# voutcn/megahit

Measured on NVIDIA H100. Metric: sorted (k+1)-mer edges/sec at k=27 on 150bp reads, higher is better.
Workload: dtype u32

## Files before the change

### include/mhb.h

```cpp
#ifndef MHB_H
#define MHB_H
#include <stddef.h>
#include <stdint.h>

#ifdef __cplusplus
extern "C" {
#endif

#define MHB_OK 0
#define MHB_ERR_ARG 1
#define MHB_ERR_CUDA 2
#define MHB_ERR_IO 3
#define MHB_ERR_NOMEM 4

#define MHB_NUM_BUCKETS 65536
#define MHB_MAX_MUL 65535
#define MHB_MAX_K 255
#define MHB_SENTINEL_OFFSET 0xFFFFFFFFu

const char *mhb_last_error(void);
const char *mhb_version(void);
int mhb_device_count(void);
uint64_t mhb_launch_count(void);

uint32_t mhb_count_record_words(uint32_t k);
uint32_t mhb_words_per_edge(uint32_t k);
uint32_t mhb_s2s_record_words(uint32_t k);
uint32_t mhb_count_sort_bytes(uint32_t k, uint8_t *bytes);
uint32_t mhb_s2s_sort_bytes(uint32_t k, uint8_t *bytes);
size_t mhb_sort_workspace_bytes(uint64_t n, uint32_t words);


typedef struct {
  const uint32_t *bin;
  uint64_t bin_words;
  uint64_t n_reads;
  uint32_t fixed_len;
  const uint64_t *rec_off;
  const uint64_t *edge_off;
} mhb_dev_reads;

int mhb_count_extract(void *stream, const mhb_dev_reads *reads, uint32_t k, uint32_t *records,
                      uint64_t n_edges, uint64_t *hist256, int hist_byte);

int mhb_check_fixed_len(void *stream, const uint32_t *bin_dev, uint64_t n_reads, uint32_t fixed_len, uint64_t *flag_dev);

int mhb_count_extract_range(void *stream, const mhb_dev_reads *reads, uint32_t k, uint32_t lo, uint32_t hi, int write,
                            uint64_t *per_read, uint32_t *records, uint64_t *hist256, int hist_byte,
                            uint64_t *total_dev);

int mhb_sort_records(void *stream, uint32_t *a, uint32_t *b, uint64_t n, uint32_t words,
                     const uint8_t *bytes, uint32_t n_bytes, const uint64_t *first_hist, void *ws,
                     size_t ws_bytes, int *result_in_b);

int mhb_sort_records_relaxed(void *stream, uint32_t *a, uint32_t *b, uint64_t n, uint32_t words, const uint8_t *bytes,
                             uint32_t n_bytes, const uint64_t *first_hist, void *ws, size_t ws_bytes, int *result_in_b);

int mhb_partition_scatter(void *stream, const uint32_t *recs, uint64_t n, uint32_t words, int byte,
                          const uint8_t *owner_of_byte_dev, const uint64_t *bin_addr_dev, void *ws, size_t ws_bytes);
int mhb_partition_scatter_hist(void *stream, const uint32_t *recs, uint64_t n, uint32_t words, int byte,
                               const uint8_t *owner_of_byte_dev, const uint64_t *bin_addr_dev, void *ws, size_t ws_bytes,
                               int next_byte, uint64_t *owner_next_hist, int *hist_done);
int mhb_plan_partition(void *stream, const uint64_t *hist_all_dev, uint32_t world, uint32_t rank, uint32_t record_bytes,
                       const uint64_t *peer_base_host, uint8_t *owner_lut_dev, uint64_t *bin_addr_dev, uint64_t *plan_dev);
int mhb_compact_tip_edges(void *stream, const uint32_t *edges, const uint8_t *aux, uint64_t n_solid, uint32_t k,
                          uint32_t *tips_out, uint8_t *tip_aux_out, uint64_t capacity, uint64_t *cursor_dev);
int mhb_dev_malloc(void **ptr, size_t bytes);
int mhb_dev_free(void *ptr);
int mhb_ipc_export(const void *dev_ptr, uint8_t *handle64);
int mhb_ipc_open(const uint8_t *handle64, void **peer_ptr);
int mhb_ipc_close(void *peer_ptr);

int mhb_set_sort_cfg(int cfg);

int mhb_sort_pass_ms(int back, double *pass_ms, uint32_t max_passes, uint32_t *n_passes, uint64_t *n_records,
                     uint32_t *words);

size_t mhb_count_solid_scratch_bytes(uint64_t n);
int mhb_count_solid(void *stream, const uint32_t *sorted_records, uint64_t n, uint32_t k, int32_t m,
                    uint32_t *edges_out, uint8_t *aux_out, uint64_t capacity_edges, uint64_t *mul_hist,
                    uint64_t *n_solid_out, void *scratch, size_t scratch_bytes);

int mhb_count_hashed_supported(uint32_t k, int32_t m);
size_t mhb_count_hashed_workspace_bytes(uint64_t n, uint32_t k, int32_t m);
int mhb_count_solid_hashed(void *stream, uint32_t *recs_a, uint32_t *recs_b, uint64_t n, uint32_t k, int32_t m,
                           const uint64_t *hist_byte5, uint32_t *edges_out, uint8_t *aux_out, uint64_t capacity_edges,
                           uint64_t *mul_hist, uint64_t *n_solid_out, void *ws, size_t ws_bytes);

size_t mhb_tipset_bytes(uint64_t n_tip_edges, uint32_t k);
int mhb_tipset_build(void *stream, const uint32_t *edges, const uint8_t *aux, uint64_t n_solid, uint32_t k,
                     void *tipset, size_t tipset_bytes, uint64_t n_tip_edges);
int mhb_count_mark_mercy(void *stream, const mhb_dev_reads *reads, uint32_t k, const void *tipset,
                         size_t tipset_bytes, uint64_t n_tip_edges, uint32_t *first_0_out, uint32_t *last_0_in);
int mhb_count_tip_edges(void *stream, const uint8_t *aux, uint64_t n_solid, uint64_t *n_tip_host);

size_t mhb_mercy_candidates_scratch_bytes(uint64_t n_reads);
int mhb_mercy_candidates(void *stream, const uint32_t *first_0_out, const uint32_t *last_0_in, uint64_t n_reads,
                         uint64_t *cand_ids, uint64_t *n_cand_host, void *scratch, size_t scratch_bytes);
size_t mhb_mercy_edges_scratch_bytes(uint64_t n_cand, uint32_t max_read_len);
int mhb_mercy_edges(void *stream, const mhb_dev_reads *reads, const uint64_t *cand_ids, uint64_t n_cand,
                    uint32_t max_read_len, uint32_t k, const uint32_t *edges, uint64_t n_edges, uint32_t *mercy_out,
                    uint64_t capacity, uint64_t *n_mercy_host, void *scratch, size_t scratch_bytes);
int mhb_mercy_edges_count(void *stream, const mhb_dev_reads *reads, const uint64_t *cand_ids, uint64_t n_cand,
                          uint32_t max_read_len, uint32_t k, uint32_t n_segs, const uint32_t *const *seg_edges,
                          const uint64_t *seg_counts, const void *const *seg_luts, const uint8_t *owner_of_byte,
                          uint64_t *n_mercy_host, void *scratch, size_t scratch_bytes);
int mhb_mercy_edges_write(void *stream, const mhb_dev_reads *reads, const uint64_t *cand_ids, uint64_t n_cand,
                          uint32_t max_read_len, uint32_t k, uint32_t *mercy_out, uint64_t capacity, uint64_t n_mercy,
                          void *scratch, size_t scratch_bytes);

size_t mhb_mercy_planes_words(uint64_t n_cand, uint32_t max_read_len);
int mhb_mercy_probe_owned(void *stream, const mhb_dev_reads *reads, const uint64_t *cand_ids, uint64_t n_cand,
                          uint32_t max_read_len, uint32_t k, const uint32_t *edges, uint64_t n_edges, const void *lut,
                          const uint8_t *owner_of_byte, uint32_t me, uint32_t *planes_out);
int mhb_mercy_count_planes(void *stream, const mhb_dev_reads *reads, const uint64_t *cand_ids, uint64_t n_cand,
                           uint32_t max_read_len, uint32_t k, const uint32_t *planes, uint32_t n_src,
                           uint64_t src_stride_words, uint64_t *n_mercy_host, void *scratch, size_t scratch_bytes);

int mhb_mercy_edges_segs(void *stream, const mhb_dev_reads *reads, const uint64_t *cand_ids, uint64_t n_cand,
                         uint32_t max_read_len, uint32_t k, uint32_t n_segs, const uint32_t *const *seg_edges,
                         const uint64_t *seg_counts, const void *const *seg_luts, const uint8_t *owner_of_byte,
                         uint32_t *mercy_out, uint64_t capacity, uint64_t *n_mercy_host, void *scratch,
                         size_t scratch_bytes);
size_t mhb_edge_lut_bytes(void);
int mhb_edge_lut_build(void *stream, const uint32_t *edges, uint64_t n_edges, uint32_t k, void *lut);

typedef struct {
  const uint32_t *words;
  uint64_t n_words;
  uint64_t n_seqs;
  uint32_t fixed_len;
  const uint64_t *word_off;
  const uint32_t *len;
  const uint64_t *item_off;
  const uint16_t *mult;
  uint32_t fixed_stride;
} mhb_dev_seqs;

int mhb_s2s_extract(void *stream, const mhb_dev_seqs *seqs, uint32_t k, uint32_t *records, uint64_t n_items,
                    uint64_t *hist256, int hist_byte);

int mhb_s2s_extract_edges_pruned(void *stream, const uint32_t *edges, const uint8_t *aux, uint64_t n_edges,
                                 uint64_t n_with_aux, uint32_t k, uint32_t *records, uint64_t capacity,
                                 uint64_t *cursor_dev, uint64_t *hist256, int hist_byte);

int mhb_s2s_extract_range(void *stream, const mhb_dev_seqs *seqs, uint32_t k, uint32_t *records, uint64_t n_items,
                          uint32_t lo, uint32_t hi, uint64_t *cursor_dev, uint64_t capacity, uint64_t *hist256,
                          int hist_byte);

size_t mhb_s2s_emit_scratch_bytes(uint64_t n, uint32_t k);
int mhb_s2s_emit(void *stream, const uint32_t *sorted_records, uint64_t n, uint32_t k, uint8_t *bytes_out,
                 uint64_t capacity_bytes, uint64_t *bucket_table, uint64_t *totals, void *scratch,
                 size_t scratch_bytes);

int mhb_s2s_emit_fmt(void *stream, const uint32_t *sorted_records, uint64_t n, uint32_t k, uint8_t *bytes_out,
                     uint64_t capacity_bytes, uint64_t *bucket_table, uint64_t *totals, void *scratch,
                     size_t scratch_bytes, int label_fmt);

int mhb_set_device(int device);

typedef struct {
  uint32_t k;
  int32_t m;
  const uint32_t *bin;
  uint64_t bin_words;
  uint64_t n_reads;
  int want_mercy;
} mhb_count_args;

typedef struct {
  uint64_t n_edge_records;
  uint64_t n_solid;
  uint32_t words_per_edge;
  uint32_t *edges;
  uint64_t n_cand;
  uint64_t *cand_ids;
  uint64_t n_has_tips;
  int64_t counting[MHB_MAX_MUL + 1];
  double t_h2d_ms, t_extract_ms, t_sort_ms, t_count_ms, t_mercy_ms, t_d2h_ms, t_total_ms;
  uint32_t n_sort_passes;
  uint32_t n_rounds;
  double sort_pass_ms[64];
} mhb_count_result;

int mhb_count_host(const mhb_count_args *args, mhb_count_result *res);
int mhb_set_round_limit(uint64_t max_records_per_round);
int mhb_set_s2s_round_limit(uint64_t max_items_per_round);
int mhb_plan_rounds(const uint64_t *hist256, uint64_t max_records, uint32_t *lo_out, uint32_t *hi_out);
int mhb_plan_rounds16(const uint64_t *hist256, const uint64_t *sub_hist, uint64_t max_records, uint32_t *lo16_out,
                      uint32_t *hi16_out, uint32_t cap_out);

typedef struct {
  uint32_t k;
  const uint32_t *words;
  const uint64_t *word_off;
  const uint32_t *len;
  const uint16_t *mult;
  uint64_t n_seqs;
} mhb_s2s_args;

typedef struct {
  uint64_t n_records;
  uint64_t n_items, n_tips, n_large_mul, n_bytes;
  uint32_t words_per_tip_label;
  uint8_t *bytes;
  uint64_t bucket_table[MHB_NUM_BUCKETS * 4];
  uint64_t w_count[9];
  uint64_t ones_in_last;
  double t_total_ms, t_extract_ms, t_sort_ms, t_emit_ms;
} mhb_s2s_result;

int mhb_s2s_host(const mhb_s2s_args *args, mhb_s2s_result *res);

typedef struct {
  uint32_t k;
  int32_t m;
  const uint32_t *bin;
  uint64_t bin_words;
  uint64_t n_reads;
  int32_t need_mercy;
  int32_t want_edges;
  uint8_t *sdbg_out;
  uint64_t sdbg_out_capacity;
} mhb_build_args;

typedef struct {
  uint64_t n_edge_records, n_solid, n_cand, n_mercy, n_sort_items;
  uint32_t words_per_edge, words_per_tip_label;
  uint64_t n_items, n_tips, n_large_mul, n_bytes;
  uint8_t *bytes;
  uint64_t *bucket_table;
  uint64_t w_count[9];
  uint64_t ones_in_last;
  uint32_t *edges;
  uint64_t *cand_ids;
  int64_t *counting;
  double t_total_ms, t_h2d_ms, t_count_ms, t_mercy_ms, t_s2s_ms, t_d2h_ms;
  uint32_t n_rounds_s1, n_rounds_s2;
} mhb_build_result;

int mhb_build_host(const mhb_build_args *args, mhb_build_result *res);
// ... 112 lines not shown
```

### megahit_b200/csrc/mhb_hashcount.cu

```cuda
#include <cuda_runtime.h>
#include <stdio.h>
#include <string.h>

#include "mhb.h"
#include "mhb_common.cuh"
#include "mhb_count.cuh"

using namespace mhb;

namespace {

constexpr int kHcHist = 1024;
constexpr u64 kHcEmpty = ~0ull;
constexpr int kHcBatch = 8;
constexpr u32 kRemBits = 42;
constexpr u32 kHcHotCount = 256;
constexpr int kHcHotRound = 32;
constexpr int kHcMaxProbes = 48;
constexpr int kHcStack = 72;
constexpr u32 kHcHistDone = 1u << 31;
constexpr u32 kHcPrefetchChunk = 16384;

__device__ __forceinline__ u64 rec_key64(const uint2 r) { return ((u64)r.x << 32) | r.y; }

// ... 352 lines not shown
          s.tmp[atomicAdd(&s.cell_cur[(u32)((e << bits) >> cshift)], 1u)] = e;
        }
        __syncthreads();
        for (u32 i = tid; i < (u32)CELLS; i += THREADS) s.cell_cur[i] = 0;
        for (u32 i = tid; i < ns; i += THREADS) {
          const u64 e = s.tmp[i];
          const u32 c = (u32)((e << bits) >> cshift);
          const u32 b0 = s.cell_base[c], b1 = c + 1 < (u32)CELLS ? s.cell_base[c + 1] : ns;
          u32 r = b0;
          for (u32 j = b0; j < b1; ++j) r += s.tmp[j] < e ? 1u : 0u;
          list[base + out_cursor + r] = e;
        }
        out_cursor += ns;
      }
      if (failed) {
        for (u32 i = tid; i < (u32)CELLS; i += THREADS) s.cell_cur[i] = 0;
        if (bits + 2 > kRemBits || sp + 4 > (u32)kHcStack) {
          if (tid == 0) atomicExch(err_flag, 1u);
        } else {
          const u32 flag = (hist_done || !overflowed) ? kHcHistDone : 0u;
          if (tid == 0)
            for (int c = 3; c >= 0; --c) {
              s.st_prefix[sp + 3 - c] = (prefix << 2) | (u64)c;
              s.st_bits[sp + 3 - c] = (bits + 2) | flag;
            }
          sp += 4;
        }
        __syncthreads();
      }
      if (sp == 0) break;
      --sp;
      prefix = s.st_prefix[sp];
      bits = s.st_bits[sp] & ~kHcHistDone;
      hist_done = (s.st_bits[sp] & kHcHistDone) != 0;
    }
    if (tid == 0) slice_count[sl] = out_cursor;
  }
  __syncthreads();
  for (u32 i = tid; i < kHcHist; i += THREADS)
    if (s.cta_hist[i]) atomicAdd((unsigned long long *)&mul_hist[i], (unsigned long long)s.cta_hist[i]);
}

using HcGeomB = HcGeom<512, 12, 2>;

__global__ void k_slice_counts(const u64 *__restrict__ bounds, u32 T, u32 *__restrict__ cnt) {
  const u32 b = blockIdx.x * blockDim.x + threadIdx.x;
  if (b >= 65536u) return;
  const u64 nb = bounds[b + 1] - bounds[b];
  cnt[b] = (u32)((nb + T - 1) / T);
}

__global__ void __launch_bounds__(256)
    k_hash_gather(const u64 *__restrict__ list, const u64 *__restrict__ n_slices_dev, const u32 *__restrict__ slice_count,
                  const u64 *__restrict__ slice_dst, const u64 *__restrict__ slice_base, const u32 *__restrict__ slice_bucket,
                  u32 we, u32 *__restrict__ edges, uint8_t *__restrict__ aux, u64 capacity, const u32 *err_flag,
                  u64 *n_solid_out) {
  const u32 lane = threadIdx.x & 31;
  if (blockIdx.x == 0 && threadIdx.x == 0 && *err_flag) *n_solid_out = ~0ull;
  const u64 n_slices = *n_slices_dev;
  for (u64 sl = (u64)blockIdx.x * 8 + (threadIdx.x >> 5); sl < n_slices; sl += (u64)gridDim.x * 8) {
    const u32 cnt = slice_count[sl];
    if (!cnt) continue;
    const u64 base = slice_base[sl], off = slice_dst[sl], b = slice_bucket[sl];
    for (u32 x = lane; x < cnt; x += 32) {
      if (off + x >= capacity) break;
      const u64 ent = list[base + x];
      const u64 key = (b << 48) | ((ent >> 22) << 6);
      u32 *e = edges + (off + x) * we;
      e[0] = (u32)(key >> 32);
      e[1] = (u32)key;
      if (we == 3) e[2] = 0;
      e[we - 1] |= (u32)(ent >> 6) & 0xFFFFu;
      aux[off + x] = (uint8_t)(ent & 3u);
    }
  }
}

int scan_counts(cudaStream_t st, const u32 *in, u64 n, u64 *out, u64 *total_dev, u64 *bsum) {
  const u64 nb = (n + kScanTile - 1) / kScanTile;
  k_scan32_sums<<<(unsigned)nb, kScanThreads, 0, st>>>(in, n, bsum);
  CK_LAUNCH();
  k_scan_u64<<<1, 1024, 0, st>>>(bsum, nb, total_dev);
  CK_LAUNCH();
  k_scan32_apply<<<(unsigned)nb, kScanThreads, 0, st>>>(in, n, bsum, out);
  CK_LAUNCH();
  return MHB_OK;
}

template <class G>
static int launch_hash_count(cudaStream_t st, const uint2 *recs, const ulonglong2 *plan, const u64 *n_slices_dev, int m, u32 *misc,
                             u64 *list, u32 *slice_count, u64 *mul_hist) {
  static int bps = 0;
  const size_t smem = sizeof(HcShared<G>);
  if (!bps) {
    CK(cudaFuncSetAttribute(k_hash_count<G>, cudaFuncAttributeMaxDynamicSharedMemorySize, (int)smem));
    CK(cudaOccupancyMaxActiveBlocksPerMultiprocessor(&bps, k_hash_count<G>, G::THREADS, smem));
    if (bps < 1) return mhb_set_error(MHB_ERR_CUDA, "hash-count kernel does not fit an SM (%zu B shared memory)", smem);
    if (getenv("MHB_VERBOSE")) fprintf(stderr, "[mhb] hash count: %d threads, %d slots, %zu B smem, %d CTA/SM, slice %u\n", G::THREADS, G::SLOTS, smem, bps, G::SLICE);
  }
  k_hash_count<G><<<sm_count() * bps, G::THREADS, smem, st>>>(recs, plan, n_slices_dev, m, misc, list, slice_count, mul_hist,
                                                             misc + 1);
  CK_LAUNCH();
  return MHB_OK;
}

struct HcLayout {
  size_t sort_ws, off_bounds, off_bcnt, off_soff, off_bsum, off_misc, off_scount, off_sdst, off_sbase, off_sbucket, off_plan,
      off_list, total;
  uint64_t max_slices;
};
HcLayout hc_layout(uint64_t n, int32_t m) {
  HcLayout L;
  auto pad = [](size_t x) { return (x + 255) & ~(size_t)255; };
  L.max_slices = n / HcGeomB::SLICE + 65536 + 2;
  L.sort_ws = pad(mhb_sort_workspace_bytes(n, 2));
  size_t p = L.sort_ws;
  L.off_bounds = p;
  p += pad(65537 * 8);
  L.off_bcnt = p;
  p += pad(65537 * 4);
  L.off_soff = p;
  p += pad(65537 * 8);
  L.off_bsum = p;
  p += pad((L.max_slices / kScanTile + 4) * 8);
  L.off_misc = p;
  p += 256;
  L.off_scount = p;
  p += pad(L.max_slices * 4);
  L.off_sdst = p;
  p += pad(L.max_slices * 8);
  L.off_sbase = p;
  p += pad(L.max_slices * 8);
  L.off_sbucket = p;
  p += pad(L.max_slices * 4);
  L.off_plan = p;
  p += pad(L.max_slices * 16);
  L.off_list = p;
  p += pad((size_t)(n / (uint64_t)(m < 1 ? 1 : m) + L.max_slices + 8) * 8);
  L.total = p;
  return L;
}

}

extern "C" int mhb_count_hashed_supported(uint32_t k, int32_t m) {
  return count_record_words(k) == 2 && 2 * (k + 1) >= 24 && m >= 1 && m <= kHcHist;
}

extern "C" size_t mhb_count_hashed_workspace_bytes(uint64_t n, uint32_t k, int32_t m) {
  (void)k;
  return hc_layout(n, m).total;
}

extern "C" int mhb_count_solid_hashed(void *stream, uint32_t *recs_a, uint32_t *recs_b, uint64_t n, uint32_t k, int32_t m,
                                      const uint64_t *hist_byte5, uint32_t *edges_out, uint8_t *aux_out,
                                      uint64_t capacity_edges, uint64_t *mul_hist, uint64_t *n_solid_out, void *ws,
                                      size_t ws_bytes) {
  if (!mhb_count_hashed_supported(k, m)) return mhb_set_error(MHB_ERR_ARG, "hashed count needs 8-byte records (13 <= k <= 28) and 1 <= m <= %d", kHcHist);
  if (!mul_hist || !n_solid_out || !ws) return mhb_set_error(MHB_ERR_ARG, "bad args");
  if (n == 0) return MHB_OK;
  if (n >= (1ull << 40)) return mhb_set_error(MHB_ERR_ARG, "too many records for one hashed count call");
  const HcLayout L = hc_layout(n, m);
  if (ws_bytes < L.total) return mhb_set_error(MHB_ERR_ARG, "hashed count workspace too small (%zu < %zu)", ws_bytes, L.total);
  cudaStream_t st = (cudaStream_t)stream;
  const uint8_t bytes[3] = {5, 6, 7};
  int in_b = 0;
  if (int rc = mhb_sort_records_impl(st, recs_a, recs_b, n, 2, bytes, 3, hist_byte5, ws, L.sort_ws, &in_b, nullptr)) return rc;
  const uint2 *recs = (const uint2 *)(in_b ? recs_b : recs_a);
  char *w = (char *)ws;
  u64 *bounds = (u64 *)(w + L.off_bounds);
  u32 *bcnt = (u32 *)(w + L.off_bcnt);
  u64 *slice_off = (u64 *)(w + L.off_soff);
  u64 *bsum = (u64 *)(w + L.off_bsum);
  u32 *misc = (u32 *)(w + L.off_misc);
  u32 *slice_count = (u32 *)(w + L.off_scount);
  u64 *slice_dst = (u64 *)(w + L.off_sdst);
  u64 *slice_base = (u64 *)(w + L.off_sbase);
  u32 *slice_bucket = (u32 *)(w + L.off_sbucket);
  ulonglong2 *plan = (ulonglong2 *)(w + L.off_plan);
  u64 *list = (u64 *)(w + L.off_list);
  u64 *n_slices_dev = (u64 *)(misc + 2);
  CK(cudaMemsetAsync(misc, 0, 256, st));
  CK(cudaMemsetAsync(slice_count, 0, L.max_slices * 4, st));
  k_bucket_bounds<<<(65537 + 255) / 256, 256, 0, st>>>(recs, n, bounds);
  CK_LAUNCH();
  k_slice_counts<<<65536 / 256, 256, 0, st>>>(bounds, HcGeomB::SLICE, bcnt);
  CK_LAUNCH();
  if (int rc = scan_counts(st, bcnt, 65536, slice_off, n_slices_dev, bsum)) return rc;
  CK(cudaMemcpyAsync(slice_off + 65536, n_slices_dev, 8, cudaMemcpyDeviceToDevice, st));
  k_slice_plan<<<65536 / 256, 256, 0, st>>>(recs, bounds, slice_off, m, plan, slice_base, slice_bucket);
  CK_LAUNCH();
  if (int rc = launch_hash_count<HcGeomB>(st, recs, plan, n_slices_dev, m, misc, list, slice_count, mul_hist)) return rc;
  if (int rc = scan_counts(st, slice_count, L.max_slices, slice_dst, n_solid_out, bsum)) return rc;
  k_hash_gather<<<sm_count() * 4, 256, 0, st>>>(list, n_slices_dev, slice_count, slice_dst, slice_base, slice_bucket,
                                               words_per_edge(k), edges_out, aux_out, capacity_edges, misc + 1, n_solid_out);
  CK_LAUNCH();
  return MHB_OK;
}
```

### megahit_b200/csrc/mhb_host.cu

```cuda
#include <cuda_runtime.h>
#include <stdio.h>
#include <stdlib.h>
#include <string.h>

#include <algorithm>
#include <vector>

#include "mhb.h"
#include "mhb_bits.cuh"
#include "mhb_internal.h"

using namespace mhb;

#define CK(call)                                                                                   \
  do {                                                                                             \
    cudaError_t e_ = (call);                                                                       \
    if (e_ != cudaSuccess)                                                                         \
      return mhb_set_error(MHB_ERR_CUDA, "%s failed at %s:%d: %s", #call, __FILE__, __LINE__,      \
                           cudaGetErrorString(e_));                                                \
  } while (0)
#define CKR(call)           \
  do {                      \
    int rc_ = (call);       \
    if (rc_) return rc_;    \
// ... 8 lines not shown
    used = 0;
    if (bytes <= cap) return MHB_OK;
    if (base) cudaFree(base);
    base = nullptr;
    cap = 0;
    cudaError_t e = cudaMalloc((void **)&base, bytes);
    if (e != cudaSuccess) {
      cudaGetLastError();
      return mhb_set_error(MHB_ERR_NOMEM, "cudaMalloc of %zu bytes failed: %s", bytes, cudaGetErrorString(e));
    }
    cap = bytes;
    return MHB_OK;
  }
  template <class T>
  T *take(size_t count) {
    size_t bytes = (count * sizeof(T) + 255) & ~(size_t)255;
    char *p = base + used;
    used += bytes;
    return reinterpret_cast<T *>(p);
  }
  static size_t pad(size_t bytes) { return (bytes + 255) & ~(size_t)255; }
};
Arena g_arena;

struct Timer {
  cudaEvent_t a, b;
  cudaStream_t st;
  explicit Timer(cudaStream_t s) : st(s) {
    cudaEventCreate(&a);
    cudaEventCreate(&b);
  }
  ~Timer() {
    cudaEventDestroy(a);
    cudaEventDestroy(b);
  }
  void start() { cudaEventRecord(a, st); }
  double stop() {
    cudaEventRecord(b, st);
    cudaEventSynchronize(b);
    float ms = 0;
    cudaEventElapsedTime(&ms, a, b);
    return ms;
  }
};

struct BinIndex {
  uint32_t fixed_len = 0;
  std::vector<uint64_t> rec_off, edge_off;
  uint64_t n_edges = 0;
};

int index_bin(const uint32_t *bin, uint64_t bin_words, uint64_t n_reads, uint32_t k, BinIndex *ix, bool sampled = false) {
  ix->fixed_len = 0;
  ix->n_edges = 0;
  if (n_reads == 0) return MHB_OK;
  if (bin_words == 0) return mhb_set_error(MHB_ERR_ARG, "empty .bin image for %llu reads", (unsigned long long)n_reads);
  const uint32_t L0 = bin[0];
  const uint64_t stride = 1 + div_ceil(L0, 16);
  bool fixed = L0 > 0 && bin_words == n_reads * stride;
  if (fixed && sampled) {
    const uint64_t step = std::max<uint64_t>(1, n_reads / 1024);
    for (uint64_t r = 0; r < n_reads && fixed; r += step) fixed = bin[r * stride] == L0;
    for (uint64_t r = 0; r < std::min<uint64_t>(n_reads, 1024) && fixed; ++r) fixed = bin[r * stride] == L0;
    fixed = fixed && bin[(n_reads - 1) * stride] == L0;
  } else if (fixed) {
    int bad = 0;
#pragma omp parallel for reduction(| : bad) schedule(static)
    for (long long r = 0; r < (long long)n_reads; ++r) bad |= bin[(uint64_t)r * stride] != L0;
    fixed = !bad;
  }
  if (fixed) {
    ix->fixed_len = L0;
    ix->n_edges = L0 >= k + 1 ? n_reads * (uint64_t)(L0 - k) : 0;
    if (L0 < k + 1) ix->fixed_len = L0;
    return MHB_OK;
  }
  ix->rec_off.resize(n_reads + 1);
  ix->edge_off.resize(n_reads + 1);
  uint64_t pos = 0, e = 0;
  for (uint64_t r = 0; r < n_reads; ++r) {
    if (pos >= bin_words) return mhb_set_error(MHB_ERR_ARG, ".bin image truncated at read %llu", (unsigned long long)r);
    const uint32_t L = bin[pos];
    ix->rec_off[r] = pos;
    ix->edge_off[r] = e;
    if (L >= k + 1) e += L - k;
    pos += 1 + div_ceil(L, 16);
  }
  if (pos > bin_words) return mhb_set_error(MHB_ERR_ARG, ".bin image truncated");
  ix->rec_off[n_reads] = pos;
  ix->edge_off[n_reads] = e;
  ix->n_edges = e;
  return MHB_OK;
}

}

extern "C" int mhb_release(void) {
  if (g_arena.base) cudaFree(g_arena.base);
  g_arena = Arena();
  return MHB_OK;
}

size_t mhb_arena_bytes(void) { return g_arena.cap; }

int SdbgStitch::append(void *stream, const uint8_t *d_bytes, uint64_t cap_bytes, const uint64_t *d_table,
                       const uint64_t *d_totals) {
  cudaStream_t st = (cudaStream_t)stream;
  uint64_t rt[16];
  CK(cudaMemcpyAsync(rt, d_totals, sizeof(rt), cudaMemcpyDeviceToHost, st));
  CK(cudaMemcpyAsync(round_table.data(), d_table, round_table.size() * 8, cudaMemcpyDeviceToHost, st));
  CK(cudaStreamSynchronize(st));
  if (rt[0] > cap_bytes) return mhb_set_error(MHB_ERR_NOMEM, "internal: SdBG byte stream exceeds capacity");
  const size_t base = bytes.size();
  bytes.resize(base + rt[0]);
  if (rt[0]) CK(cudaMemcpy(bytes.data() + base, d_bytes, rt[0], cudaMemcpyDeviceToHost));
  for (size_t b = 0; b < (size_t)MHB_NUM_BUCKETS; ++b)
    if (round_table[4 * b + 1]) {
      table[4 * b + 0] = round_table[4 * b + 0] + base;
      table[4 * b + 1] = round_table[4 * b + 1];
      table[4 * b + 2] = round_table[4 * b + 2];
      table[4 * b + 3] = round_table[4 * b + 3];
    }
  for (int i = 0; i < 16; ++i) tot[i] += rt[i];
  return MHB_OK;
}


namespace {
struct CountWork {
  bool hashed;
  size_t bytes;
  size_t ws_bytes;
  int hist_byte;
};
CountWork count_work_plan(uint64_t n, uint32_t k, int32_t m) {
  static const bool force_sort = getenv("MHB_COUNT_MODE") && !strcmp(getenv("MHB_COUNT_MODE"), "sort");
  CountWork cw;
  cw.hashed = !force_sort && mhb_count_hashed_supported(k, m);
  if (cw.hashed) {
    cw.bytes = mhb_count_hashed_workspace_bytes(n, k, m);
    cw.ws_bytes = 0;
    cw.hist_byte = 5;
  } else {
    uint8_t sb[72];
    mhb_count_sort_bytes(k, sb);
    cw.ws_bytes = Arena::pad(mhb_sort_workspace_bytes(n, count_record_words(k)));
    cw.bytes = cw.ws_bytes + Arena::pad(mhb_count_solid_scratch_bytes(n));
    cw.hist_byte = sb[0];
  }
  return cw;
}
int run_count_stage(cudaStream_t st, const CountWork &cw, uint32_t *d_a, uint32_t *d_b, uint64_t n, uint32_t k, int32_t m,
                    const uint64_t *d_hist0, uint32_t *d_edges, uint8_t *d_aux, uint64_t cap_edges, uint64_t *d_mul_hist,
                    uint64_t *d_nsolid, char *work, double *pass_ms, uint32_t *n_passes) {
  const uint32_t WR = count_record_words(k);
  if (cw.hashed) {
    if (n_passes) *n_passes = n ? 2 : 0;
    CKR(mhb_count_solid_hashed(st, d_a, d_b, n, k, m, d_hist0, d_edges, d_aux, cap_edges, d_mul_hist, d_nsolid, work, cw.bytes));
    if (pass_ms && n) {
      uint32_t np = 0, w = 0;
      uint64_t nr = 0;
      CKR(mhb_sort_pass_ms(0, pass_ms, 64, &np, &nr, &w));
    }
    return MHB_OK;
  }
  uint8_t sort_bytes[72];
  const uint32_t n_sort = mhb_count_sort_bytes(k, sort_bytes);
  if (n_passes) *n_passes = n ? n_sort : 0;
  int in_b = 0;
  CKR(mhb_sort_records_impl(st, d_a, d_b, n, WR, sort_bytes, n_sort, d_hist0, work, cw.ws_bytes, &in_b, pass_ms));
  return mhb_count_solid(st, in_b ? d_b : d_a, n, k, m, d_edges, d_aux, cap_edges, d_mul_hist, d_nsolid, work + cw.ws_bytes,
                         cw.bytes - cw.ws_bytes);
}
}

namespace {
size_t round_bytes(uint64_t n, uint32_t WR, uint32_t WE, int32_t m, uint32_t k) {
  const uint64_t cap_edges = n / (uint64_t)std::max(1, m) + 1;
  return 2 * Arena::pad((size_t)n * WR * 4 + 16) + Arena::pad(count_work_plan(n, k, m).bytes) +
         Arena::pad((size_t)cap_edges * WE * 4) + Arena::pad(cap_edges);
}
}

namespace {
uint64_t g_round_limit = 0;
uint64_t g_s2s_round_limit = 0;


}

extern "C" int mhb_plan_rounds(const uint64_t *hist256, uint64_t max_records, uint32_t *lo_out, uint32_t *hi_out) {
  if (!hist256 || !lo_out || !hi_out || max_records == 0) {
    mhb_set_error(MHB_ERR_ARG, "bad round plan arguments");
    return -1;
  }
  int n = 0;
  uint32_t lo = 0;
  uint64_t acc = 0;
  for (uint32_t b = 0; b < 256; ++b) {
    if (hist256[b] > max_records) {
      mhb_set_error(MHB_ERR_NOMEM, "leading byte 0x%02x alone holds %llu records, more than one round can take (%llu)", b,
                    (unsigned long long)hist256[b], (unsigned long long)max_records);
      return -1;
    }
    if (acc + hist256[b] > max_records) {
      lo_out[n] = lo;
      hi_out[n] = b - 1;
      ++n;
      lo = b;
      acc = 0;
    }
    acc += hist256[b];
  }
  lo_out[n] = lo;
  hi_out[n] = 255;
  return n + 1;
}

extern "C" int mhb_plan_rounds16(const uint64_t *hist256, const uint64_t *sub_hist, uint64_t max_records, uint32_t *lo_out,
                                 uint32_t *hi_out, uint32_t cap_out) {
  if (!hist256 || !lo_out || !hi_out || max_records == 0 || cap_out == 0) {
    mhb_set_error(MHB_ERR_ARG, "bad round plan arguments");
    return -1;
  }
  uint32_t n = 0, lo = 0;
  uint64_t acc = 0;
  bool open = false;
  auto close_at = [&](uint32_t hi) -> bool {
    if (n >= cap_out) return false;
    lo_out[n] = lo;
    hi_out[n] = hi;
    ++n;
    return true;
  };
  auto add = [&](uint32_t a_lo, uint32_t a_hi, uint64_t cnt) -> int {
    if (cnt > max_records) {
      mhb_set_error(MHB_ERR_NOMEM, "bucket 0x%04x alone holds %llu records, more than one round can take (%llu)", a_lo,
                    (unsigned long long)cnt, (unsigned long long)max_records);
      return -1;
    }
    if (open && acc + cnt > max_records) {
      if (!close_at(a_lo - 1)) return -2;
      open = false;
    }
    if (!open) {
      lo = a_lo;
      acc = 0;
      open = true;
    }
    acc += cnt;
    (void)a_hi;
    return 0;
  };
  for (uint32_t b = 0; b < 256; ++b) {
    int rc = 0;
    if (hist256[b] > max_records) {
      if (!sub_hist) {
        mhb_set_error(MHB_ERR_NOMEM, "leading byte 0x%02x alone holds %llu records, more than one round can take (%llu)", b,
                      (unsigned long long)hist256[b], (unsigned long long)max_records);
        return -1;
      }
      for (uint32_t c = 0; c < 256 && !rc; ++c) rc = add((b << 8) | c, (b << 8) | c, sub_hist[(size_t)b * 256 + c]);
    } else {
      rc = add(b << 8, (b << 8) | 255u, hist256[b]);
    }
    if (rc == -1) return -1;
    if (rc == -2) break;
  }
  if (!open) {
    lo = 0;
    open = true;
  }
  if (lo_out && n < cap_out) {
    lo_out[n] = n ? lo : 0;
    hi_out[n] = 65535;
    return (int)n + 1;
  }
  mhb_set_error(MHB_ERR_NOMEM, "round plan needs more than %u ranges", cap_out);
  return -1;
}

extern "C" int mhb_set_round_limit(uint64_t max_records_per_round) {
  g_round_limit = max_records_per_round;
  return MHB_OK;
}
extern "C" int mhb_set_s2s_round_limit(uint64_t max_items_per_round) {
  g_s2s_round_limit = max_items_per_round;
  return MHB_OK;
}

static int count_host_rounds(const mhb_count_args *args, mhb_count_result *res, const BinIndex &ix, uint64_t max_records) {
  const uint32_t k = args->k;
  const int32_t m = args->m;
  const uint64_t n = ix.n_edges, n_reads = args->n_reads;
  const uint32_t WR = count_record_words(k), WE = words_per_edge(k);
  uint8_t sort_bytes[72];
  const uint32_t n_sort = mhb_count_sort_bytes(k, sort_bytes);
  const int top_byte = (int)(4 * WR - 1);
  cudaStream_t st = 0;
  Timer t_all(st), t(st);
  t_all.start();

  const size_t bin_bytes = (args->bin_words * 4 + 15) & ~(size_t)15;
  size_t fixed = Arena::pad(bin_bytes + 16) + Arena::pad((n_reads + 2) * 8) + Arena::pad(65536 * 8) + 2 * Arena::pad(256 * 8) +
                 Arena::pad(64) + 8192;
  if (!ix.fixed_len) fixed += 2 * Arena::pad((n_reads + 1) * 8);
  if (args->want_mercy) fixed += 2 * Arena::pad((size_t)(n_reads + 1) * 4);
  if (!max_records) {
    size_t free_b = 0, total_b = 0;
    CK(cudaMemGetInfo(&free_b, &total_b));
    const size_t avail = (size_t)((double)(free_b + g_arena.cap) * 0.92);
    if (avail <= fixed) return mhb_set_error(MHB_ERR_NOMEM, "the read library alone (%zu bytes) does not fit the device", fixed);
    uint64_t lo = 1, hi = n;
    while (lo < hi) {
      const uint64_t mid = lo + (hi - lo + 1) / 2;
      if (fixed + round_bytes(mid, WR, WE, m, k) <= avail) lo = mid;
      else hi = mid - 1;
    }
    max_records = lo;
  }
  max_records = std::min<uint64_t>(std::max<uint64_t>(max_records, 1), std::max<uint64_t>(n, 1));
  const uint64_t cap_edges = max_records / (uint64_t)std::max(1, m) + 1;
  CKR(g_arena.reserve(fixed + round_bytes(max_records, WR, WE, m, k)));

  uint32_t *d_bin = g_arena.take<uint32_t>(bin_bytes / 4 + 4);
// ... 41 lines not shown
  uint64_t h_top[256];
  CKR(mhb_count_extract_range(st, &reads, k, 0, 65535, 0, d_per_read, nullptr, d_hist_top, top_byte, d_scalars + 1));
  CK(cudaMemcpyAsync(h_top, d_hist_top, sizeof(h_top), cudaMemcpyDeviceToHost, st));
  CK(cudaStreamSynchronize(st));
  std::vector<uint64_t> h_sub;
  for (uint32_t b = 0; b < 256; ++b) {
    if (h_top[b] <= max_records) continue;
    if (WR * 4 < 2) return mhb_set_error(MHB_ERR_NOMEM, "leading byte 0x%02x exceeds a round and the record has no second byte", b);
    if (h_sub.empty()) h_sub.assign(256 * 256, 0);
    CK(cudaMemsetAsync(d_hist0, 0, 256 * 8, st));
    CKR(mhb_count_extract_range(st, &reads, k, b << 8, (b << 8) | 255u, 0, d_per_read, nullptr, d_hist0, top_byte - 1, d_scalars + 1));
    CK(cudaMemcpyAsync(h_sub.data() + (size_t)b * 256, d_hist0, 256 * 8, cudaMemcpyDeviceToHost, st));
    CK(cudaStreamSynchronize(st));
  }
  std::vector<uint32_t> r_lo(65536), r_hi(65536);
  const int n_ranges = mhb_plan_rounds16(h_top, h_sub.empty() ? nullptr : h_sub.data(), max_records, r_lo.data(), r_hi.data(), 65536);
  if (n_ranges < 0) return MHB_ERR_NOMEM;
  std::vector<std::pair<uint32_t, uint32_t>> ranges;
  for (int i = 0; i < n_ranges; ++i) ranges.push_back({r_lo[i], r_hi[i]});
  res->t_extract_ms = t.stop();

  std::vector<uint32_t> h_edges;
  std::vector<uint32_t> h_tip_edges;
  std::vector<uint8_t> h_tip_aux, h_aux;
  uint64_t n_solid_total = 0;
  for (const auto &rg : ranges) {
    t.start();
    uint64_t n_round = 0;
    CKR(mhb_count_extract_range(st, &reads, k, rg.first, rg.second, 0, d_per_read, nullptr, nullptr, 0, d_scalars + 1));
    CK(cudaMemcpyAsync(&n_round, d_scalars + 1, 8, cudaMemcpyDeviceToHost, st));
    CK(cudaMemsetAsync(d_hist0, 0, 256 * 8, st));
    CK(cudaMemsetAsync(d_scalars, 0, 8, st));
    CK(cudaStreamSynchronize(st));
    if (n_round > max_records) return mhb_set_error(MHB_ERR_NOMEM, "internal: round of %llu records exceeds its plan", (unsigned long long)n_round);
    if (n_round == 0) continue;
    CKR(mhb_count_extract_range(st, &reads, k, rg.first, rg.second, 1, d_per_read, d_a, d_hist0, cw.hist_byte, nullptr));
    res->t_extract_ms += t.stop();
    t.start();
    CKR(run_count_stage(st, cw, d_a, d_b, n_round, k, m, d_hist0, d_edges, d_aux, cap_edges, d_mul_hist, d_scalars, d_work,
                        nullptr, nullptr));
    uint64_t n_solid = 0;
    CK(cudaMemcpyAsync(&n_solid, d_scalars, 8, cudaMemcpyDeviceToHost, st));
    CK(cudaStreamSynchronize(st));
    res->t_count_ms += t.stop();
    if (n_solid > cap_edges) return mhb_set_error(MHB_ERR_NOMEM, "internal: solid edges exceed capacity");
    t.start();
    const size_t e0 = h_edges.size();
    h_edges.resize(e0 + (size_t)n_solid * WE);
    h_aux.resize(n_solid);
    if (n_solid) {
      CK(cudaMemcpyAsync(h_edges.data() + e0, d_edges, (size_t)n_solid * WE * 4, cudaMemcpyDeviceToHost, st));
      CK(cudaMemcpyAsync(h_aux.data(), d_aux, n_solid, cudaMemcpyDeviceToHost, st));
      CK(cudaStreamSynchronize(st));
    }
    if (args->want_mercy)
      for (uint64_t i = 0; i < n_solid; ++i)
        if (h_aux[i]) {
          h_tip_edges.insert(h_tip_edges.end(), h_edges.begin() + e0 + i * WE, h_edges.begin() + e0 + (i + 1) * WE);
          h_tip_aux.push_back(h_aux[i]);
        }
    n_solid_total += n_solid;
    res->t_d2h_ms += t.stop();
    ++res->n_rounds;
  }
  res->n_solid = n_solid_total;

  std::vector<uint32_t> h_first, h_last;
  if (args->want_mercy && n_reads) {
    t.start();
    const uint64_t n_tip = h_tip_aux.size();
    const size_t ts_bytes = mhb_tipset_bytes(n_tip, k);
    const size_t list_bytes = Arena::pad(h_tip_edges.size() * 4 + 16) + Arena::pad(n_tip + 16);
    char *d_tmp = nullptr;
    bool own = false;
    const size_t have = (size_t)max_records * WR * 4 * 2;
    if (ts_bytes + list_bytes + 512 <= have) d_tmp = (char *)d_a;
    else {
      CK(cudaMalloc((void **)&d_tmp, ts_bytes + list_bytes + 512));
      own = true;
    }
    uint32_t *d_tip_edges = (uint32_t *)d_tmp;
    uint8_t *d_tip_aux = (uint8_t *)(d_tmp + Arena::pad(h_tip_edges.size() * 4 + 16));
    char *d_tips = d_tmp + list_bytes;
    int rc = MHB_OK;
    if (n_tip) {
      if (cudaMemcpyAsync(d_tip_edges, h_tip_edges.data(), h_tip_edges.size() * 4, cudaMemcpyHostToDevice, st) != cudaSuccess ||
          cudaMemcpyAsync(d_tip_aux, h_tip_aux.data(), n_tip, cudaMemcpyHostToDevice, st) != cudaSuccess)
        rc = mhb_set_error(MHB_ERR_CUDA, "tip edge upload failed");
    }
    if (!rc) rc = mhb_tipset_build(st, d_tip_edges, d_tip_aux, n_tip, k, d_tips, ts_bytes, n_tip);
    if (!rc) rc = mhb_count_mark_mercy(st, &reads, k, d_tips, ts_bytes, n_tip, d_first, d_last);
    h_first.resize(n_reads);
    h_last.resize(n_reads);
    if (!rc) {
      cudaMemcpyAsync(h_first.data(), d_first, n_reads * 4, cudaMemcpyDeviceToHost, st);
      cudaMemcpyAsync(h_last.data(), d_last, n_reads * 4, cudaMemcpyDeviceToHost, st);
      if (cudaStreamSynchronize(st) != cudaSuccess) rc = mhb_set_error(MHB_ERR_CUDA, "mercy marking failed: %s", cudaGetErrorString(cudaGetLastError()));
    }
    if (own) cudaFree(d_tmp);
    if (rc) return rc;
    res->t_mercy_ms = t.stop();
  }

  res->edges = (uint32_t *)malloc(std::max<size_t>(1, h_edges.size() * 4));
  if (!res->edges) return mhb_set_error(MHB_ERR_NOMEM, "host malloc failed");
  if (!h_edges.empty()) memcpy(res->edges, h_edges.data(), h_edges.size() * 4);
  std::vector<uint64_t> h_hist(65536);
  CK(cudaMemcpy(h_hist.data(), d_mul_hist, 65536 * 8, cudaMemcpyDeviceToHost));
  for (int i = 0; i <= MHB_MAX_MUL; ++i) res->counting[i] = (int64_t)h_hist[i];
  if (args->want_mercy) {
    std::vector<uint64_t> ids;
    for (uint64_t r = 0; r < n_reads; ++r) {
      const uint32_t f = h_first[r], l = h_last[r];
      if (f != MHB_SENTINEL_OFFSET && l != MHB_SENTINEL_OFFSET) {
        ++res->n_has_tips;
        if (l > f) ids.push_back(r);
      }
    }
    res->n_cand = ids.size();
    res->cand_ids = (uint64_t *)malloc(std::max<size_t>(1, ids.size() * 8));
    if (!ids.empty()) memcpy(res->cand_ids, ids.data(), ids.size() * 8);
  }
  res->t_total_ms = t_all.stop();
  return MHB_OK;
}

extern "C" int mhb_count_host(const mhb_count_args *args, mhb_count_result *res) {
  if (!args || !res) return mhb_set_error(MHB_ERR_ARG, "null args");
  memset(res, 0, sizeof(*res));
  const uint32_t k = args->k;
  if (k < 1 || k > MHB_MAX_K) return mhb_set_error(MHB_ERR_ARG, "kmer size %u out of range", k);
  if (mhb_device_count() == 0) return mhb_set_error(MHB_ERR_CUDA, "no CUDA device: libmhb has no CPU path");
  res->words_per_edge = words_per_edge(k);

  BinIndex ix;
  CKR(index_bin(args->bin, args->bin_words, args->n_reads, k, &ix));
  const uint64_t n = ix.n_edges, n_reads = args->n_reads;
  res->n_edge_records = n;

  cudaStream_t st = 0;
  Timer t_all(st), t(st);
  t_all.start();

  const uint32_t WR = count_record_words(k), WE = words_per_edge(k);
  uint8_t sort_bytes[72];
  const uint32_t n_sort = mhb_count_sort_bytes(k, sort_bytes);
  const int32_t m = args->m;
  const uint64_t cap_edges = n / (uint64_t)std::max(1, m) + 1;

  const size_t bin_bytes = (args->bin_words * 4 + 15) & ~(size_t)15;
  const CountWork cw = count_work_plan(n, k, m);
  size_t need = Arena::pad(bin_bytes + 16) + 2 * Arena::pad((size_t)n * WR * 4 + 16) + Arena::pad(cw.bytes) +
                Arena::pad((size_t)cap_edges * WE * 4) + Arena::pad(cap_edges) +
                Arena::pad(65536 * 8) + Arena::pad(256 * 8) + 4096;
  if (!ix.fixed_len) need += 2 * Arena::pad((n_reads + 1) * 8);
  if (args->want_mercy) need += 2 * Arena::pad((size_t)(n_reads + 1) * 4);
  {
    bool rounds = g_round_limit && n > g_round_limit;
    if (!rounds && need > g_arena.cap) {
      size_t free_b = 0, total_b = 0;
      CK(cudaMemGetInfo(&free_b, &total_b));
      rounds = (double)need > 0.92 * (double)(free_b + g_arena.cap);
    }
    if (rounds) return count_host_rounds(args, res, ix, g_round_limit);
  }
  CKR(g_arena.reserve(need));

  uint32_t *d_bin = g_arena.take<uint32_t>(bin_bytes / 4 + 4);
  uint32_t *d_a = g_arena.take<uint32_t>((size_t)n * WR + 4);
  uint32_t *d_b = g_arena.take<uint32_t>((size_t)n * WR + 4);
  char *d_work = g_arena.take<char>(cw.bytes);
  uint32_t *d_edges = g_arena.take<uint32_t>((size_t)cap_edges * WE);
  uint8_t *d_aux = g_arena.take<uint8_t>(cap_edges);
  uint64_t *d_mul_hist = g_arena.take<uint64_t>(65536);
  uint64_t *d_hist0 = g_arena.take<uint64_t>(256);
  uint64_t *d_nsolid = g_arena.take<uint64_t>(8);
  uint64_t *d_rec_off = nullptr, *d_edge_off = nullptr;
  uint32_t *d_first = nullptr, *d_last = nullptr;
  if (!ix.fixed_len) {
    d_rec_off = g_arena.take<uint64_t>(n_reads + 1);
    d_edge_off = g_arena.take<uint64_t>(n_reads + 1);
  }
  if (args->want_mercy) {
    d_first = g_arena.take<uint32_t>(n_reads + 1);
    d_last = g_arena.take<uint32_t>(n_reads + 1);
  }

  t.start();
  if (args->bin_words) CK(cudaMemcpyAsync(d_bin, args->bin, args->bin_words * 4, cudaMemcpyHostToDevice, st));
  if (!ix.fixed_len && n_reads) {
    CK(cudaMemcpyAsync(d_rec_off, ix.rec_off.data(), (n_reads + 1) * 8, cudaMemcpyHostToDevice, st));
    CK(cudaMemcpyAsync(d_edge_off, ix.edge_off.data(), (n_reads + 1) * 8, cudaMemcpyHostToDevice, st));
  }
  CK(cudaMemsetAsync(d_mul_hist, 0, 65536 * 8, st));
  CK(cudaMemsetAsync(d_hist0, 0, 256 * 8, st));
  CK(cudaMemsetAsync(d_nsolid, 0, 64, st));
  res->t_h2d_ms = t.stop();

  mhb_dev_reads reads;
  reads.bin = d_bin;
  reads.bin_words = args->bin_words;
  reads.n_reads = n_reads;
  reads.fixed_len = ix.fixed_len;
  reads.rec_off = d_rec_off;
  reads.edge_off = d_edge_off;

  t.start();
  CKR(mhb_count_extract(st, &reads, k, d_a, n, d_hist0, cw.hist_byte));
  res->t_extract_ms = t.stop();

  t.start();
  res->n_rounds = 1;
  CKR(run_count_stage(st, cw, d_a, d_b, n, k, m, d_hist0, d_edges, d_aux, cap_edges, d_mul_hist, d_nsolid, d_work,
                      res->sort_pass_ms, &res->n_sort_passes));
  for (uint32_t p = 0; p < res->n_sort_passes; ++p) res->t_sort_ms += res->sort_pass_ms[p];
  uint64_t n_solid = 0;
  CK(cudaMemcpyAsync(&n_solid, d_nsolid, 8, cudaMemcpyDeviceToHost, st));
  CK(cudaStreamSynchronize(st));
  res->t_count_ms = t.stop();
  if (n_solid > cap_edges) return mhb_set_error(MHB_ERR_NOMEM, "internal: solid edges exceed capacity");
  res->n_solid = n_solid;

  std::vector<uint32_t> h_first, h_last;
  if (args->want_mercy && n_reads) {
    t.start();
    uint64_t n_tip = 0;
    CKR(mhb_count_tip_edges(st, d_aux, n_solid, &n_tip));
    const size_t ts_bytes = mhb_tipset_bytes(n_tip, k);
    char *d_tips = nullptr;
    uint32_t *d_free = d_a;
    bool own = false;
    if (ts_bytes <= (size_t)n * WR * 4) d_tips = (char *)d_free;
    else {
      CK(cudaMalloc((void **)&d_tips, ts_bytes));
      own = true;
    }
    int rc = mhb_tipset_build(st, d_edges, d_aux, n_solid, k, d_tips, ts_bytes, n_tip);
    if (!rc) rc = mhb_count_mark_mercy(st, &reads, k, d_tips, ts_bytes, n_tip, d_first, d_last);
    h_first.resize(n_reads);
    h_last.resize(n_reads);
    if (!rc) {
      cudaMemcpyAsync(h_first.data(), d_first, n_reads * 4, cudaMemcpyDeviceToHost, st);
      cudaMemcpyAsync(h_last.data(), d_last, n_reads * 4, cudaMemcpyDeviceToHost, st);
      if (cudaStreamSynchronize(st) != cudaSuccess) rc = mhb_set_error(MHB_ERR_CUDA, "mercy marking failed: %s", cudaGetErrorString(cudaGetLastError()));
    }
    if (own) cudaFree(d_tips);
    if (rc) return rc;
    res->t_mercy_ms = t.stop();
  }

  t.start();
  res->edges = (uint32_t *)malloc(std::max<size_t>(1, (size_t)n_solid * WE * 4));
  if (!res->edges) return mhb_set_error(MHB_ERR_NOMEM, "host malloc failed");
  if (n_solid) CK(cudaMemcpyAsync(res->edges, d_edges, (size_t)n_solid * WE * 4, cudaMemcpyDeviceToHost, st));
  std::vector<uint64_t> h_hist(65536);
  CK(cudaMemcpyAsync(h_hist.data(), d_mul_hist, 65536 * 8, cudaMemcpyDeviceToHost, st));
  CK(cudaStreamSynchronize(st));
  res->t_d2h_ms = t.stop();
  for (int i = 0; i <= MHB_MAX_MUL; ++i) res->counting[i] = (int64_t)h_hist[i];

  if (args->want_mercy) {
    std::vector<uint64_t> ids;
    for (uint64_t r = 0; r < n_reads; ++r) {
      const uint32_t f = h_first[r], l = h_last[r];
      if (f != MHB_SENTINEL_OFFSET && l != MHB_SENTINEL_OFFSET) {
        ++res->n_has_tips;
        if (l > f) ids.push_back(r);
      }
    }
    res->n_cand = ids.size();
    res->cand_ids = (uint64_t *)malloc(std::max<size_t>(1, ids.size() * 8));
    if (!ids.empty()) memcpy(res->cand_ids, ids.data(), ids.size() * 8);
  }
  res->t_total_ms = t_all.stop();
  return MHB_OK;
}

namespace {
size_t s2s_round_bytes(uint64_t n, uint32_t W, uint32_t k) {
  return 2 * Arena::pad((size_t)n * W * 4 + 16) + Arena::pad(mhb_sort_workspace_bytes(n, W)) +
         Arena::pad(mhb_s2s_emit_scratch_bytes(n, k)) + Arena::pad((size_t)n * (4ull + 4ull * words_per_tip_label(k)) + 16);
}
}

static int s2s_host_rounds(const mhb_s2s_args *args, mhb_s2s_result *res, const std::vector<uint64_t> &item_off,
                           uint64_t n_items, bool fixed, uint32_t L0, uint64_t n_words, uint64_t max_items) {
  const uint32_t k = args->k;
  const uint64_t ns = args->n_seqs;
  const uint32_t W = s2s_record_words(k), WPT = words_per_tip_label(k);
  uint8_t sort_bytes[72];
  const uint32_t n_sort = mhb_s2s_sort_bytes(k, sort_bytes);
  const int top_byte = (int)(4 * W - 1);
  cudaStream_t st = 0;
  Timer t_all(st), t(st);
  t_all.start();

  const size_t fixed_b = Arena::pad(n_words * 4 + 64) + Arena::pad((ns + 1) * 8) * 2 + Arena::pad((ns + 1) * 4) +
                         Arena::pad((ns + 1) * 2) + Arena::pad((size_t)MHB_NUM_BUCKETS * 4 * 8) + 2 * Arena::pad(256 * 8) +
                         Arena::pad(16 * 8) + Arena::pad(64) + 8192;
  if (!max_items) {
    size_t free_b = 0, total_b = 0;
    CK(cudaMemGetInfo(&free_b, &total_b));
    const size_t avail = (size_t)((double)(free_b + g_arena.cap) * 0.92);
    if (avail <= fixed_b) return mhb_set_error(MHB_ERR_NOMEM, "the sequences alone (%zu bytes) do not fit the device", fixed_b);
    uint64_t lo = 1, hi = n_items;
    while (lo < hi) {
      const uint64_t mid = lo + (hi - lo + 1) / 2;
      if (fixed_b + s2s_round_bytes(mid, W, k) <= avail) lo = mid;
      else hi = mid - 1;
    }
    max_items = lo;
  }
  max_items = std::min<uint64_t>(std::max<uint64_t>(max_items, 1), std::max<uint64_t>(n_items, 1));
  CKR(g_arena.reserve(fixed_b + s2s_round_bytes(max_items, W, k)));
  uint32_t *d_words = g_arena.take<uint32_t>(n_words + 16);
  uint64_t *d_word_off = g_arena.take<uint64_t>(ns + 1);
  uint64_t *d_item_off = g_arena.take<uint64_t>(ns + 1);
  uint32_t *d_len = g_arena.take<uint32_t>(ns + 1);
  uint16_t *d_mult = g_arena.take<uint16_t>(ns + 1);
  uint64_t *d_table = g_arena.take<uint64_t>((size_t)MHB_NUM_BUCKETS * 4);
  uint64_t *d_hist0 = g_arena.take<uint64_t>(256);
  uint64_t *d_hist_top = g_arena.take<uint64_t>(256);
  uint64_t *d_totals = g_arena.take<uint64_t>(16);
  uint64_t *d_cursor = g_arena.take<uint64_t>(8);
  uint32_t *d_a = g_arena.take<uint32_t>((size_t)max_items * W + 4);
  uint32_t *d_b = g_arena.take<uint32_t>((size_t)max_items * W + 4);
  const size_t ws_bytes = mhb_sort_workspace_bytes(max_items, W);
  const size_t scratch_bytes = mhb_s2s_emit_scratch_bytes(max_items, k);
  const uint64_t cap_bytes = max_items * (4ull + 4ull * WPT) + 16;
  char *d_ws = g_arena.take<char>(ws_bytes);
  char *d_scratch = g_arena.take<char>(scratch_bytes);
  uint8_t *d_bytes = g_arena.take<uint8_t>(cap_bytes);

  if (ns) {
    CK(cudaMemcpyAsync(d_words, args->words, n_words * 4, cudaMemcpyHostToDevice, st));
    CK(cudaMemcpyAsync(d_word_off, args->word_off, (ns + 1) * 8, cudaMemcpyHostToDevice, st));
    CK(cudaMemcpyAsync(d_item_off, item_off.data(), (ns + 1) * 8, cudaMemcpyHostToDevice, st));
    CK(cudaMemcpyAsync(d_len, args->len, ns * 4, cudaMemcpyHostToDevice, st));
    CK(cudaMemcpyAsync(d_mult, args->mult, ns * 2, cudaMemcpyHostToDevice, st));
  }
  CK(cudaMemsetAsync(d_hist_top, 0, 256 * 8, st));
  mhb_dev_seqs seqs;
  seqs.words = d_words;
  seqs.n_words = n_words;
  seqs.n_seqs = ns;
  seqs.fixed_len = fixed ? L0 : 0;
  seqs.word_off = d_word_off;
  seqs.len = d_len;
  seqs.item_off = d_item_off;
  seqs.mult = d_mult;
  seqs.fixed_stride = 0;

  t.start();
  uint64_t h_top[256];
  CKR(mhb_s2s_extract_range(st, &seqs, k, nullptr, n_items, 0, 65535, nullptr, 0, d_hist_top, top_byte));
  CK(cudaMemcpyAsync(h_top, d_hist_top, sizeof(h_top), cudaMemcpyDeviceToHost, st));
  CK(cudaStreamSynchronize(st));
  std::vector<uint64_t> h_sub;
  for (uint32_t b = 0; b < 256; ++b) {
    if (h_top[b] <= max_items) continue;
    if (h_sub.empty()) h_sub.assign(256 * 256, 0);
    CK(cudaMemsetAsync(d_hist0, 0, 256 * 8, st));
    CKR(mhb_s2s_extract_range(st, &seqs, k, nullptr, n_items, b << 8, (b << 8) | 255u, nullptr, 0, d_hist0, top_byte - 1));
    CK(cudaMemcpyAsync(h_sub.data() + (size_t)b * 256, d_hist0, 256 * 8, cudaMemcpyDeviceToHost, st));
    CK(cudaStreamSynchronize(st));
  }
  std::vector<uint32_t> r_lo(65536), r_hi(65536);
// ... 153 lines not shown
  mhb_count_args ca;
  memset(&ca, 0, sizeof(ca));
  ca.k = k;
  ca.m = args->m;
  ca.bin = args->bin;
  ca.bin_words = args->bin_words;
  ca.n_reads = args->n_reads;
  ca.want_mercy = args->need_mercy;
  std::vector<char> cbuf(sizeof(mhb_count_result));
  mhb_count_result *cr = reinterpret_cast<mhb_count_result *>(cbuf.data());
  CKR(mhb_count_host(&ca, cr));
  struct Owned {
    mhb_count_result *r;
    ~Owned() {
      free(r->edges);
      free(r->cand_ids);
    }
  } owned{cr};
  res->n_edge_records = cr->n_edge_records;
  res->n_solid = cr->n_solid;
  res->n_cand = cr->n_cand;
  res->words_per_edge = WE;
  res->words_per_tip_label = words_per_tip_label(k);
  res->t_count_ms = cr->t_total_ms;
  uint32_t *mercy = nullptr;
  uint64_t n_mercy = 0;
  if (args->need_mercy && cr->n_cand) {
    std::vector<uint32_t> cand;
    uint64_t r = 0;
    size_t pos = 0;
    for (uint64_t c = 0; c < cr->n_cand; ++c) {
      while (r < cr->cand_ids[c]) {
        pos += 1 + div_ceil(args->bin[pos], 16);
        ++r;
      }
      const uint32_t L = args->bin[pos], nw = div_ceil(L, 16);
      const size_t at = cand.size();
      cand.resize(at + 1 + nw, 0u);
      cand[at] = L;
      for (uint32_t i = 0; i < L; ++i) cand[at + 1 + (i >> 4)] |= base_at(&args->bin[pos + 1], L - 1 - i) << (30 - 2 * (i & 15));
    }
    uint64_t n_cr = 0;
    CKR(mhb_mercy_host(k, cr->edges, cr->n_solid, cand.data(), cand.size(), &mercy, &n_mercy, &n_cr));
  }
  struct FreeMercy {
    uint32_t *&p;
    ~FreeMercy() { free(p); }
  } fm{mercy};
  res->n_mercy = n_mercy;
  const uint64_t n_seqs = cr->n_solid + n_mercy;
  std::vector<uint32_t> words((size_t)n_seqs * NWE + 1, 0u), len(n_seqs, k + 1);
  std::vector<uint64_t> word_off(n_seqs + 1);
  std::vector<uint16_t> mult(n_seqs);
  const uint32_t tail = (k + 1) % 16;
  for (uint64_t i = 0; i < n_seqs; ++i) {
    const uint32_t *e = i < cr->n_solid ? cr->edges + i * WE : mercy + (i - cr->n_solid) * WE;
    for (uint32_t j = 0; j < NWE; ++j) words[i * NWE + j] = e[j];
    if (tail) words[i * NWE + NWE - 1] &= top_mask(2 * tail);
    word_off[i] = i * NWE;
    mult[i] = (uint16_t)(e[WE - 1] & 0xFFFFu);
  }
  word_off[n_seqs] = n_seqs * NWE;
  mhb_s2s_args sa;
  memset(&sa, 0, sizeof(sa));
  sa.k = k;
  sa.words = words.data();
  sa.word_off = word_off.data();
  sa.len = len.data();
  sa.mult = mult.data();
  sa.n_seqs = n_seqs;
  std::vector<char> sbuf(sizeof(mhb_s2s_result));
  mhb_s2s_result *sr = reinterpret_cast<mhb_s2s_result *>(sbuf.data());
  CKR(mhb_s2s_host(&sa, sr));
  res->n_sort_items = sr->n_records;
  res->n_items = sr->n_items;
  res->n_tips = sr->n_tips;
  res->n_large_mul = sr->n_large_mul;
  res->n_bytes = sr->n_bytes;
  for (int i = 0; i < 9; ++i) res->w_count[i] = sr->w_count[i];
  res->ones_in_last = sr->ones_in_last;
  res->t_s2s_ms = sr->t_total_ms;
  res->bucket_table = (uint64_t *)malloc((size_t)MHB_NUM_BUCKETS * 32);
  if (!res->bucket_table) {
    free(sr->bytes);
    return mhb_set_error(MHB_ERR_NOMEM, "host malloc failed");
  }
  memcpy(res->bucket_table, sr->bucket_table, (size_t)MHB_NUM_BUCKETS * 32);
  if (args->sdbg_out && args->sdbg_out_capacity >= sr->n_bytes) {
    if (sr->n_bytes) memcpy(args->sdbg_out, sr->bytes, sr->n_bytes);
    free(sr->bytes);
    res->bytes = args->sdbg_out;
  } else {
    res->bytes = sr->bytes;
  }
  if (args->want_edges) {
    res->counting = (int64_t *)malloc(65536 * 8);
    if (!res->counting) return mhb_set_error(MHB_ERR_NOMEM, "host malloc failed");
    memcpy(res->counting, cr->counting, 65536 * 8);
    res->edges = cr->edges;
    res->cand_ids = cr->cand_ids;
    cr->edges = nullptr;
    cr->cand_ids = nullptr;
  }
  res->t_total_ms = res->t_count_ms + res->t_s2s_ms;
  return MHB_OK;
}

extern "C" int mhb_build_host(const mhb_build_args *args, mhb_build_result *res) {
  if (!args || !res) return mhb_set_error(MHB_ERR_ARG, "null args");
  if (g_round_limit || g_s2s_round_limit) return build_host_rounds(args, res);
  const int rc = build_host_impl(args, res, false);
  if (rc == MHB_ERR_NOMEM) {
    mhb_free(res->bytes == args->sdbg_out ? nullptr : res->bytes);
    mhb_free(res->bucket_table);
    mhb_free(res->edges);
    mhb_free(res->cand_ids);
    mhb_free(res->counting);
    mhb_release();
    return build_host_rounds(args, res);
  }
  return rc;
}
static int build_host_impl(const mhb_build_args *args, mhb_build_result *res, bool full_index) {
  memset(res, 0, sizeof(*res));
  const uint32_t k = args->k;
  if (k < 9 || k > MHB_MAX_K) return mhb_set_error(MHB_ERR_ARG, "kmer size must be >= 9 and <= 255");
  if (args->need_mercy && k < 12) return mhb_set_error(MHB_ERR_ARG, "mercy edges need k >= 12");
  if (mhb_device_count() == 0) return mhb_set_error(MHB_ERR_CUDA, "no CUDA device: libmhb has no CPU path");
  const uint32_t WR = count_record_words(k), WE = words_per_edge(k), W2 = s2s_record_words(k), WPT = words_per_tip_label(k);
  res->words_per_edge = WE;
  res->words_per_tip_label = WPT;

  BinIndex ix;
  CKR(index_bin(args->bin, args->bin_words, args->n_reads, k, &ix, !full_index));
  const bool verify_fixed = !full_index && ix.fixed_len != 0;
  const uint64_t n = ix.n_edges, n_reads = args->n_reads;
  res->n_edge_records = n;
  uint32_t max_len = ix.fixed_len;
  if (!ix.fixed_len)
    for (uint64_t r = 0; r < n_reads; ++r) max_len = std::max(max_len, args->bin[ix.rec_off[r]]);

  cudaStream_t st = 0;
  Timer t_all(st), t(st);
  t_all.start();

  uint8_t cbytes[72], sbytes[72];
  const uint32_t n_csort = mhb_count_sort_bytes(k, cbytes), n_ssort = mhb_s2s_sort_bytes(k, sbytes);
  const int32_t m = args->m;
  const uint64_t cap_edges = n / (uint64_t)std::max(1, m) + 1;
  const size_t bin_bytes = (args->bin_words * 4 + 15) & ~(size_t)15;
  const CountWork cw = count_work_plan(n, k, m);
  const size_t count_work = 2 * Arena::pad((size_t)n * WR * 4 + 16) + Arena::pad(cw.bytes);
  size_t fixed = Arena::pad(bin_bytes + 16) + Arena::pad((size_t)cap_edges * WE * 4) + Arena::pad(cap_edges) +
                 Arena::pad(65536 * 8) + 2 * Arena::pad(256 * 8) + Arena::pad(64) + Arena::pad((size_t)MHB_NUM_BUCKETS * 32) +
                 Arena::pad(128) + 8192;
  if (!ix.fixed_len) fixed += 2 * Arena::pad((n_reads + 1) * 8);
  if (args->need_mercy) fixed += 2 * Arena::pad((n_reads + 1) * 4) + Arena::pad((n_reads + 1) * 8);
  CKR(g_arena.reserve(fixed + count_work));

  uint32_t *d_bin = g_arena.take<uint32_t>(bin_bytes / 4 + 4);
  uint32_t *d_edges = g_arena.take<uint32_t>((size_t)cap_edges * WE);
  uint8_t *d_aux = g_arena.take<uint8_t>(cap_edges);
  uint64_t *d_mul_hist = g_arena.take<uint64_t>(65536);
  uint64_t *d_hist0 = g_arena.take<uint64_t>(256);
  uint64_t *d_hist1 = g_arena.take<uint64_t>(256);
  uint64_t *d_nsolid = g_arena.take<uint64_t>(8);
  uint64_t *d_table = g_arena.take<uint64_t>((size_t)MHB_NUM_BUCKETS * 4);
  uint64_t *d_totals = g_arena.take<uint64_t>(16);
  uint64_t *d_rec_off = nullptr, *d_edge_off = nullptr, *d_cand = nullptr;
  uint32_t *d_first = nullptr, *d_last = nullptr;
  if (!ix.fixed_len) {
    d_rec_off = g_arena.take<uint64_t>(n_reads + 1);
    d_edge_off = g_arena.take<uint64_t>(n_reads + 1);
  }
  if (args->need_mercy) {
    d_first = g_arena.take<uint32_t>(n_reads + 1);
    d_last = g_arena.take<uint32_t>(n_reads + 1);
    d_cand = g_arena.take<uint64_t>(n_reads + 1);
  }
  char *work = g_arena.take<char>(count_work);
  size_t work_bytes = count_work;
  char *extra = nullptr;
  char *big_edges = nullptr;
  struct ExtraGuard {
    char *&p;
    ~ExtraGuard() {
      if (p) cudaFree(p);
    }
  } guard{extra}, guard2{big_edges};
  uint32_t *d_all_edges = d_edges;

  static const int h2d_chunks_env = getenv("MHB_H2D_CHUNKS") ? atoi(getenv("MHB_H2D_CHUNKS")) : 4;
  const bool chunked = h2d_chunks_env > 1 && ix.fixed_len >= k + 1 && n_reads >= (uint64_t)h2d_chunks_env * 64;
  t.start();
  CK(cudaMemsetAsync(d_mul_hist, 0, 65536 * 8, st));
  CK(cudaMemsetAsync(d_hist0, 0, 256 * 8, st));
  CK(cudaMemsetAsync(d_hist1, 0, 256 * 8, st));
  CK(cudaMemsetAsync(d_nsolid, 0, 64, st));
  if (!chunked) {
    if (args->bin_words) CK(cudaMemcpyAsync(d_bin, args->bin, args->bin_words * 4, cudaMemcpyHostToDevice, st));
    if (!ix.fixed_len && n_reads) {
      CK(cudaMemcpyAsync(d_rec_off, ix.rec_off.data(), (n_reads + 1) * 8, cudaMemcpyHostToDevice, st));
      CK(cudaMemcpyAsync(d_edge_off, ix.edge_off.data(), (n_reads + 1) * 8, cudaMemcpyHostToDevice, st));
    }
  }
  res->t_h2d_ms = t.stop();

  mhb_dev_reads reads;
  reads.bin = d_bin;
  reads.bin_words = args->bin_words;
  reads.n_reads = n_reads;
  reads.fixed_len = ix.fixed_len;
  reads.rec_off = d_rec_off;
  reads.edge_off = d_edge_off;

  t.start();
  uint32_t *c_a = (uint32_t *)work;
  uint32_t *c_b = (uint32_t *)(work + Arena::pad((size_t)n * WR * 4 + 16));
  char *c_wsp = work + 2 * Arena::pad((size_t)n * WR * 4 + 16);
  if (!chunked) {
    CKR(mhb_count_extract(st, &reads, k, c_a, n, d_hist0, cw.hist_byte));
  } else {
    static cudaStream_t copy_st = nullptr;
    static cudaEvent_t ev[64];
    static bool ev_ready = false;
    if (!ev_ready) {
      CK(cudaStreamCreateWithFlags(&copy_st, cudaStreamNonBlocking));
      for (int i = 0; i < 64; ++i) CK(cudaEventCreateWithFlags(&ev[i], cudaEventDisableTiming));
      ev_ready = true;
    }
    const int C = std::min(h2d_chunks_env, 60);
    const uint64_t stride = 1 + div_ceil(ix.fixed_len, 16);
    const uint64_t per = ((n_reads + C - 1) / C + 3) & ~(uint64_t)3;
    const uint64_t e_per_read = ix.fixed_len - k;
    cudaEvent_t start_ev = ev[63];
    CK(cudaEventRecord(start_ev, st));
    CK(cudaStreamWaitEvent(copy_st, start_ev, 0));
    int c = 0;
    for (uint64_t r0 = 0; r0 < n_reads; r0 += per, ++c) {
      const uint64_t r1 = std::min(n_reads, r0 + per);
      const uint64_t w0 = r0 * stride, w1 = r1 * stride;
      CK(cudaMemcpyAsync(d_bin + w0, args->bin + w0, (w1 - w0) * 4, cudaMemcpyHostToDevice, copy_st));
      CK(cudaEventRecord(ev[c], copy_st));
      CK(cudaStreamWaitEvent(st, ev[c], 0));
      mhb_dev_reads piece = reads;
      piece.bin = d_bin + w0;
      piece.bin_words = w1 - w0;
      piece.n_reads = r1 - r0;
      CKR(mhb_count_extract(st, &piece, k, c_a + (size_t)r0 * e_per_read * WR, (r1 - r0) * e_per_read, d_hist0, cw.hist_byte));
    }
  }
  if (verify_fixed) CKR(mhb_check_fixed_len(st, d_bin, n_reads, ix.fixed_len, d_nsolid + 1));
  CKR(run_count_stage(st, cw, c_a, c_b, n, k, m, d_hist0, d_edges, d_aux, cap_edges, d_mul_hist, d_nsolid, c_wsp, nullptr, nullptr));
  uint64_t h_scal[2] = {0, 0};
  CK(cudaMemcpyAsync(h_scal, d_nsolid, 16, cudaMemcpyDeviceToHost, st));
  CK(cudaStreamSynchronize(st));
  if (verify_fixed && h_scal[1]) return build_host_impl(args, res, true);
  const uint64_t n_solid = h_scal[0];
  if (n_solid > cap_edges) return mhb_set_error(MHB_ERR_NOMEM, "internal: solid edges exceed capacity");
  res->n_solid = n_solid;
  res->t_count_ms = t.stop();

  uint64_t n_cand = 0, n_mercy = 0;
  if (args->need_mercy && n_reads) {
    t.start();
    uint64_t n_tip = 0;
    CKR(mhb_count_tip_edges(st, d_aux, n_solid, &n_tip));
    const size_t ts_bytes = mhb_tipset_bytes(n_tip, k);
    const size_t cs_bytes = mhb_mercy_candidates_scratch_bytes(n_reads);
    auto work_area = [&](size_t bytes) -> char * {
      if (bytes <= work_bytes) return work;
      if (extra) cudaFree(extra);
      extra = nullptr;
      if (cudaMalloc((void **)&extra, bytes) != cudaSuccess) {
        cudaGetLastError();
        return nullptr;
      }
      return extra;
    };
    char *d_tips = work_area(Arena::pad(ts_bytes) + Arena::pad(cs_bytes));
    if (!d_tips) return mhb_set_error(MHB_ERR_NOMEM, "cudaMalloc for the mercy stage failed");
    char *d_cs = d_tips + Arena::pad(ts_bytes);
    CKR(mhb_tipset_build(st, d_edges, d_aux, n_solid, k, d_tips, ts_bytes, n_tip));
    CKR(mhb_count_mark_mercy(st, &reads, k, d_tips, ts_bytes, n_tip, d_first, d_last));
    CKR(mhb_mercy_candidates(st, d_first, d_last, n_reads, d_cand, &n_cand, d_cs, cs_bytes));
    if (n_cand) {
      const size_t ms_bytes = mhb_mercy_edges_scratch_bytes(n_cand, max_len);
      CK(cudaStreamSynchronize(st));
      char *d_ms = work_area(ms_bytes);
      if (!d_ms) return mhb_set_error(MHB_ERR_NOMEM, "cudaMalloc for the mercy stage failed");
      const size_t core = ms_bytes - mhb_edge_lut_bytes();
      void *lut = d_ms + core;
      CKR(mhb_edge_lut_build(st, d_edges, n_solid, k, lut));
      const uint32_t *seg_e[1] = {d_edges};
      const uint64_t seg_n[1] = {n_solid};
      const void *seg_l[1] = {lut};
      CKR(mhb_mercy_edges_count(st, &reads, d_cand, n_cand, max_len, k, 1, seg_e, seg_n, seg_l, nullptr, &n_mercy, d_ms, core));
      if (n_mercy > cap_edges - n_solid) {
        const size_t eb = Arena::pad((size_t)(n_solid + n_mercy) * WE * 4 + 16);
        if (cudaMalloc((void **)&big_edges, eb) != cudaSuccess) {
          cudaGetLastError();
          return mhb_set_error(MHB_ERR_NOMEM, "cudaMalloc of %zu bytes for solid + mercy edges failed", eb);
        }
        CK(cudaMemcpyAsync(big_edges, d_edges, (size_t)n_solid * WE * 4, cudaMemcpyDeviceToDevice, st));
        d_all_edges = (uint32_t *)big_edges;
      }
      CKR(mhb_mercy_edges_write(st, &reads, d_cand, n_cand, max_len, k, d_all_edges + (size_t)n_solid * WE, n_mercy, n_mercy,
                                d_ms, core));
    }
    res->t_mercy_ms = t.stop();
  }
  res->n_cand = n_cand;
  res->n_mercy = n_mercy;

  t.start();
  const uint64_t n_seqs = n_solid + n_mercy;
  const uint64_t n_items = n_seqs * 6;
  res->n_sort_items = n_items;
  const size_t s_ws = mhb_sort_workspace_bytes(n_items, W2), s_scr = mhb_s2s_emit_scratch_bytes(n_items, k);
  const uint64_t cap_bytes = n_items * (4ull + 4ull * WPT) + 16;
  const size_t s2s_work = 2 * Arena::pad((size_t)n_items * W2 * 4 + 16) + Arena::pad(s_ws) + Arena::pad(s_scr) + Arena::pad(cap_bytes);
  char *sw = work;
  if (s2s_work > work_bytes) {
    CK(cudaStreamSynchronize(st));
    if (extra) cudaFree(extra);
    extra = nullptr;
    cudaError_t e = cudaMalloc((void **)&extra, s2s_work);
    if (e != cudaSuccess) {
      cudaGetLastError();
      return mhb_set_error(MHB_ERR_NOMEM, "cudaMalloc of %zu bytes for the SdBG stage failed", s2s_work);
    }
    sw = extra;
  }
  uint32_t *s_a = (uint32_t *)sw;
  uint32_t *s_b = (uint32_t *)(sw + Arena::pad((size_t)n_items * W2 * 4 + 16));
  char *s_wsp = sw + 2 * Arena::pad((size_t)n_items * W2 * 4 + 16);
  char *s_scrp = s_wsp + Arena::pad(s_ws);
  uint8_t *d_bytes = (uint8_t *)(s_scrp + Arena::pad(s_scr));
  mhb_dev_seqs seqs;
  memset(&seqs, 0, sizeof(seqs));
  seqs.words = d_all_edges;
  seqs.n_words = n_seqs * WE;
  seqs.n_seqs = n_seqs;
  seqs.fixed_len = k + 1;
  seqs.fixed_stride = WE;
  static const bool no_prune = getenv("MHB_S2S_NO_PRUNE") != nullptr;
  uint64_t n_sorted = n_items;
  if (!no_prune) {
    CK(cudaMemsetAsync(d_nsolid + 4, 0, 8, st));
    CKR(mhb_s2s_extract_edges_pruned(st, d_all_edges, d_aux, n_seqs, n_solid, k, s_a, n_items, d_nsolid + 4, d_hist1, sbytes[0]));
    CK(cudaMemcpyAsync(&n_sorted, d_nsolid + 4, 8, cudaMemcpyDeviceToHost, st));
    CK(cudaStreamSynchronize(st));
    if (n_sorted > n_items) return mhb_set_error(MHB_ERR_CUDA, "internal: pruned item count exceeds 6 per edge");
    res->n_sort_items = n_sorted;
  } else {
    CKR(mhb_s2s_extract(st, &seqs, k, s_a, n_items, d_hist1, sbytes[0]));
  }
  int s_in_b = 0;
  CKR(mhb_sort_records_impl(st, s_a, s_b, n_sorted, W2, sbytes, n_ssort, d_hist1, s_wsp, s_ws, &s_in_b, nullptr));
  CKR(mhb_s2s_emit(st, s_in_b ? s_b : s_a, n_sorted, k, d_bytes, cap_bytes, d_table, d_totals, s_scrp, s_scr));
  uint64_t totals[16];
  CK(cudaMemcpyAsync(totals, d_totals, sizeof(totals), cudaMemcpyDeviceToHost, st));
  CK(cudaStreamSynchronize(st));
  res->t_s2s_ms = t.stop();
  res->n_bytes = totals[0];
  res->n_items = totals[1];
  res->n_tips = totals[2];
  res->n_large_mul = totals[3];
  for (int i = 0; i < 9; ++i) res->w_count[i] = totals[4 + i];
  res->ones_in_last = totals[13];
  if (res->n_bytes > cap_bytes) return mhb_set_error(MHB_ERR_NOMEM, "internal: SdBG byte stream exceeds capacity");

  t.start();
  res->bucket_table = (uint64_t *)malloc((size_t)MHB_NUM_BUCKETS * 32);
  if (args->sdbg_out && args->sdbg_out_capacity >= res->n_bytes) res->bytes = args->sdbg_out;
  else res->bytes = (uint8_t *)malloc(std::max<size_t>(1, res->n_bytes));
  if (!res->bucket_table || !res->bytes) return mhb_set_error(MHB_ERR_NOMEM, "host malloc failed");
  CK(cudaMemcpyAsync(res->bucket_table, d_table, (size_t)MHB_NUM_BUCKETS * 32, cudaMemcpyDeviceToHost, st));
  if (res->n_bytes) CK(cudaMemcpyAsync(res->bytes, d_bytes, res->n_bytes, cudaMemcpyDeviceToHost, st));
  if (args->want_edges) {
    res->edges = (uint32_t *)malloc(std::max<size_t>(1, (size_t)n_solid * WE * 4));
    res->cand_ids = (uint64_t *)malloc(std::max<size_t>(1, n_cand * 8));
    res->counting = (int64_t *)malloc(65536 * 8);
    if (!res->edges || !res->cand_ids || !res->counting) return mhb_set_error(MHB_ERR_NOMEM, "host malloc failed");
    if (n_solid) CK(cudaMemcpyAsync(res->edges, d_edges, (size_t)n_solid * WE * 4, cudaMemcpyDeviceToHost, st));
    if (n_cand) CK(cudaMemcpyAsync(res->cand_ids, d_cand, n_cand * 8, cudaMemcpyDeviceToHost, st));
    CK(cudaMemcpyAsync(res->counting, d_mul_hist, 65536 * 8, cudaMemcpyDeviceToHost, st));
  }
  CK(cudaStreamSynchronize(st));
  res->t_d2h_ms = t.stop();
  res->t_total_ms = t_all.stop();
  return MHB_OK;
}

extern "C" int mhb_mercy_host(uint32_t k, const uint32_t *edges, uint64_t n_edges, const uint32_t *cand_bin,
                              uint64_t cand_words, uint32_t **mercy_out, uint64_t *n_mercy_out, uint64_t *n_cand_reads_out) {
  if (!mercy_out || !n_mercy_out) return mhb_set_error(MHB_ERR_ARG, "null output");
  *mercy_out = nullptr;
  *n_mercy_out = 0;
  if (n_cand_reads_out) *n_cand_reads_out = 0;
  if (k < 12 || k > MHB_MAX_K) return mhb_set_error(MHB_ERR_ARG, "mercy edges need 12 <= k <= 255");
  if (mhb_device_count() == 0) return mhb_set_error(MHB_ERR_CUDA, "no CUDA device: libmhb has no CPU path");
  const uint32_t WE = words_per_edge(k);
  std::vector<uint32_t> bin;
  std::vector<uint64_t> rec_off, edge_off;
  bin.reserve(cand_words + 8);
// ... 132 lines not shown
```

### megahit_b200/csrc/mhb_internal.h

```cpp
#pragma once
#include <stddef.h>
#include <stdint.h>

#include <vector>

int mhb_set_error(int code, const char *fmt, ...);

int mhb_sort_records_impl(void *stream, uint32_t *a, uint32_t *b, uint64_t n, uint32_t words, const uint8_t *bytes,
                          uint32_t n_bytes, const uint64_t *first_hist, void *ws, size_t ws_bytes, int *result_in_b,
                          double *pass_ms_host);

size_t mhb_arena_bytes(void);

struct SdbgStitch {
  std::vector<uint8_t> bytes;
  std::vector<uint64_t> table = std::vector<uint64_t>((size_t)65536 * 4);
  uint64_t tot[16] = {0};
  int append(void *stream, const uint8_t *d_bytes, uint64_t cap_bytes, const uint64_t *d_table, const uint64_t *d_totals);

 private:
  std::vector<uint64_t> round_table = std::vector<uint64_t>((size_t)65536 * 4);
};
```

### megahit_b200/csrc/mhb_kernels.cuh

```cuda
#pragma once
#include <cuda_runtime.h>
#include <stdint.h>

#include "mhb_bits.cuh"

namespace mhb {

static constexpr u32 kSentinel = 4;


template <int W, int WR>
MHB_HD void make_count_record(const u32 *s, u32 nwords, u32 L, u32 k, u32 q, u32 (&rec)[WR], u32 &strand) {
  const u32 K1 = k + 1;
  u32 prev_pkg, next_pkg;
  bool st;
  if constexpr (W == 2) {
    const u32 w0 = q >> 4, sh = (q & 15) * 2;
    const u32 x0 = s[w0];
    const u32 x1 = (w0 + 1 < nwords) ? s[w0 + 1] : 0u;
    const u32 x2 = (w0 + 2 < nwords) ? s[w0 + 2] : 0u;
    const u32 pi = q + K1;
    const u32 pw = ((pi >> 4) == w0 + 1) ? x1 : x2;
    prev_pkg = (pi < L) ? ((pw >> (30 - 2 * (pi & 15))) & 3u) : kSentinel;
    const u32 nwd = (q & 15) ? x0 : (q ? s[w0 - 1] : 0u);
    next_pkg = (q > 0) ? ((nwd >> (30 - 2 * ((q - 1) & 15))) & 3u) : kSentinel;
    const u32 T = 64u - 2u * K1;
    const u64 S = ((((u64)fshl(x0, x1, sh) << 32) | fshl(x1, x2, sh)) >> T) << T;
    const u64 B = ((~S) >> T) << T;
    const u64 A = (((u64)rev2((u32)S) << 32) | rev2((u32)(S >> 32))) << T;
    st = B < A;
    const u64 key = st ? B : A;
    rec[0] = (u32)(key >> 32);
    rec[1] = (u32)key;
    if constexpr (WR == 3) rec[2] = 0u;
  } else {
    prev_pkg = (q + K1 < L) ? base_at(s, q + K1) : kSentinel;
    next_pkg = (q > 0) ? base_at(s, q - 1) : kSentinel;
    u32 S[W], A[W], B[W];
    load_sub<W>(s, nwords, q, K1, S);
    reverse_sub<W>(S, K1, A);
    complement_sub<W>(S, K1, B);
    st = less_words<W>(B, A);
#pragma unroll
    for (int j = 0; j < WR; ++j) rec[j] = j < W ? (st ? B[j] : A[j]) : 0u;
  }
  u32 p = prev_pkg, n = next_pkg;
  if (st) {
    p = next_pkg == kSentinel ? kSentinel : 3u - next_pkg;
    n = prev_pkg == kSentinel ? kSentinel : 3u - prev_pkg;
  }
  rec[WR - 1] |= (p << 3) | n;
  strand = st ? 1u : 0u;
}

template <int R>
MHB_HD void make_count_records_roll(const u32 *s, u32 nwords, u32 L, u32 k, u32 q, u64 (&rec)[R], u32 (&strand)[R]) {
  const u32 K1 = k + 1;
  const u32 T = 64u - 2u * K1;
  const u32 w0 = q >> 4, sh = (q & 15) * 2;
  const u32 x0 = s[w0];
  const u32 x1 = (w0 + 1 < nwords) ? s[w0 + 1] : 0u;
  const u32 x2 = (w0 + 2 < nwords) ? s[w0 + 2] : 0u;
  const u32 x3 = (w0 + 3 < nwords) ? s[w0 + 3] : 0u;
  u64 S = ((((u64)fshl(x0, x1, sh) << 32) | fshl(x1, x2, sh)) >> T) << T;
  u64 B = ((~S) >> T) << T;
  u64 A = (((u64)rev2((u32)S) << 32) | rev2((u32)(S >> 32))) << T;
  const u32 pi = q + K1;
  const u32 wa = (pi >> 4) - w0;
  u32 LA = fshl(wa == 1 ? x1 : x2, wa == 1 ? x2 : x3, (pi & 15) * 2);
  u32 next_pkg = (q > 0) ? (((q & 15) ? (x0 >> (32 - sh)) : s[w0 - 1]) & 3u) : kSentinel;
  const u64 lowmask = ~((1ull << T) - 1ull);
#pragma unroll
  for (int j = 0; j < R; ++j) {
    const u32 b = LA >> 30;
    const u32 prev_pkg = (pi + j < L) ? b : kSentinel;
    const bool st = B < A;
    const u64 key = st ? B : A;
    u32 p = prev_pkg, n = next_pkg;
    if (st) {
      p = next_pkg == kSentinel ? kSentinel : 3u - next_pkg;
      n = prev_pkg == kSentinel ? kSentinel : 3u - prev_pkg;
    }
    rec[j] = key | (u64)((p << 3) | n);
    strand[j] = st ? 1u : 0u;
    next_pkg = (u32)(S >> 62);
    S = (S << 2) | ((u64)b << T);
    B = (B << 2) | ((u64)(3u - b) << T);
    A = ((A >> 2) & lowmask) | ((u64)b << 62);
    LA <<= 2;
  }
}

template <int W>
MHB_HD void make_s2s_record(const u32 *s, u32 nwords, u32 L, u32 k, u32 strand, u32 offset, u32 mult,
                            u32 (&rec)[W]) {
  const u32 nc = k - ((offset + k > L) ? 1u : 0u);
  const u32 counting = (offset > 0 && offset + k <= L) ? mult : 0u;
  u32 prev;
  if (strand == 0) {
    prev = offset == 0 ? kSentinel : base_at(s, offset - 1);
    load_sub<W>(s, nwords, offset, nc, rec);
  } else {
    prev = offset == 0 ? kSentinel : 3u - base_at(s, L - offset);
    int off2 = (int)L - (int)k - (int)offset;
    if (off2 < 0) off2 = 0;
    u32 S[W], T[W];
    load_sub<W>(s, nwords, (u32)off2, nc, S);
    reverse_sub<W>(S, nc, T);
    complement_sub<W>(T, nc, rec);
  }
  rec[W - 1] |= ((nc == k) ? 1u : 0u) << 19;
  rec[W - 1] |= prev << 16;
  rec[W - 1] |= 65535u - counting;
}

#if defined(__CUDACC__)
template <int WR>
__device__ __forceinline__ void ld_rec(const u32 *base, u64 idx, u32 (&r)[WR]) {
  if constexpr (WR % 4 == 0) {
    const uint4 *p = reinterpret_cast<const uint4 *>(base + idx * WR);
#pragma unroll
    for (int j = 0; j < WR / 4; ++j) {
      const uint4 v = p[j];
      r[4 * j] = v.x;
      r[4 * j + 1] = v.y;
      r[4 * j + 2] = v.z;
      r[4 * j + 3] = v.w;
    }
  } else if constexpr (WR % 2 == 0) {
    const uint2 *p = reinterpret_cast<const uint2 *>(base + idx * WR);
#pragma unroll
    for (int j = 0; j < WR / 2; ++j) {
      const uint2 v = p[j];
      r[2 * j] = v.x;
      r[2 * j + 1] = v.y;
    }
  } else {
    const u32 *p = base + idx * WR;
#pragma unroll
    for (int j = 0; j < WR; ++j) r[j] = p[j];
  }
}
template <int WR>
__device__ __forceinline__ void st_rec(u32 *base, u64 idx, const u32 (&r)[WR]) {
  if constexpr (WR % 4 == 0) {
    uint4 *p = reinterpret_cast<uint4 *>(base + idx * WR);
#pragma unroll
    for (int j = 0; j < WR / 4; ++j) p[j] = make_uint4(r[4 * j], r[4 * j + 1], r[4 * j + 2], r[4 * j + 3]);
  } else if constexpr (WR % 2 == 0) {
    uint2 *p = reinterpret_cast<uint2 *>(base + idx * WR);
#pragma unroll
    for (int j = 0; j < WR / 2; ++j) p[j] = make_uint2(r[2 * j], r[2 * j + 1]);
  } else {
    u32 *p = base + idx * WR;
#pragma unroll
    for (int j = 0; j < WR; ++j) p[j] = r[j];
  }
}

template <int WR>
__device__ __forceinline__ u32 rec_byte(const u32 (&r)[WR], int b) {
  return (pick<WR>(r, (u32)(WR - 1 - (b >> 2))) >> (8 * (b & 3))) & 255u;
}

__device__ __forceinline__ u32 lane_id() { return threadIdx.x & 31; }
__device__ __forceinline__ u32 lanemask_lt() {
  u32 m;
  asm("mov.u32 %0, %%lanemask_lt;" : "=r"(m));
  return m;
}

__device__ __forceinline__ u32 smem_u32(const void *p) { return (u32)__cvta_generic_to_shared(p); }
__device__ __forceinline__ void mbar_init(u64 *bar, u32 count) {
  asm volatile("mbarrier.init.shared::cta.b64 [%0], %1;" ::"r"(smem_u32(bar)), "r"(count) : "memory");
}
__device__ __forceinline__ void mbar_fence_init() {
  asm volatile("fence.mbarrier_init.release.cluster;" ::: "memory");
  asm volatile("fence.proxy.async.shared::cta;" ::: "memory");
}
__device__ __forceinline__ void mbar_expect_tx(u64 *bar, u32 bytes) {
  asm volatile("mbarrier.arrive.expect_tx.shared::cta.b64 _, [%0], %1;" ::"r"(smem_u32(bar)), "r"(bytes)
               : "memory");
}
__device__ __forceinline__ void bulk_g2s(void *dst, const void *src, u32 bytes, u64 *bar) {
  asm volatile("cp.async.bulk.shared::cluster.global.mbarrier::complete_tx::bytes [%0], [%1], %2, [%3];" ::"r"(
                   smem_u32(dst)),
               "l"(src), "r"(bytes), "r"(smem_u32(bar))
               : "memory");
}
__device__ __forceinline__ bool mbar_try_wait(u64 *bar, u32 parity) {
  u32 ok;
  asm volatile(
      "{\n\t.reg .pred p;\n\tmbarrier.try_wait.parity.shared::cta.b64 p, [%1], %2;\n\tselp.u32 %0, 1, 0, p;\n\t}"
      : "=r"(ok)
      : "r"(smem_u32(bar)), "r"(parity)
      : "memory");
  return ok != 0;
}
__device__ __forceinline__ void mbar_wait(u64 *bar, u32 parity) {
  while (!mbar_try_wait(bar, parity)) {
  }
}

__device__ __forceinline__ u64 ld_relaxed(const u64 *p) {
  u64 v;
  asm volatile("ld.relaxed.gpu.global.u64 %0, [%1];" : "=l"(v) : "l"(p) : "memory");
  return v;
}
__device__ __forceinline__ void st_relaxed(u64 *p, u64 v) {
  asm volatile("st.relaxed.gpu.global.u64 [%0], %1;" ::"l"(p), "l"(v) : "memory");
}

static constexpr u64 kLbPartial = 1ull << 62, kLbInclusive = 2ull << 62, kLbStatusMask = 3ull << 62;
static constexpr u64 kLbValueMask = (1ull << 54) - 1;
__host__ __device__ inline u64 lb_epoch(u32 e) { return (u64)(e & 255u) << 54; }

template <int THREADS>
__device__ __forceinline__ u32 block_excl_scan(u32 v, u32 *s_warp , u32 &total) {
  const u32 lane = lane_id(), warp = threadIdx.x >> 5;
  u32 inc = v;
#pragma unroll
  for (int d = 1; d < 32; d <<= 1) {
    u32 t = __shfl_up_sync(0xffffffffu, inc, d);
    if (lane >= (u32)d) inc += t;
  }
  if (lane == 31) s_warp[warp] = inc;
  __syncthreads();
  if (warp == 0) {
    u32 w = lane < THREADS / 32 ? s_warp[lane] : 0u;
    u32 winc = w;
#pragma unroll
    for (int d = 1; d < 32; d <<= 1) {
      u32 t = __shfl_up_sync(0xffffffffu, winc, d);
      if (lane >= (u32)d) winc += t;
    }
    if (lane < THREADS / 32) s_warp[lane] = winc - w;
// ... 12 lines not shown
```

### megahit_b200/csrc/mhb_sortdisp.cu

```cuda
#include <cuda_runtime.h>
#include <stdio.h>
#include <stdlib.h>
#include <string.h>

#include "mhb.h"
#include "mhb_common.cuh"
#include "mhb_kernels.cuh"
#include "mhb_sort.cuh"
#include "mhb_sort3.cuh"
#include "mhb_part.cuh"

using namespace mhb;

#define MHB_V3_DEFAULT 0x180
#define MHB_V3_LIST(X) X(0x180) X(0x080) X(0x000) X(0x1080) X(0x082)
static bool v3_listed(int bits) {
#define X(B) \
  if (bits == B) return true;
  MHB_V3_LIST(X)
#undef X
  return false;
}
static int g_sort_cfg = -1;
extern "C" int mhb_set_sort_cfg(int cfg) {
  if (!((cfg >= 0 && cfg <= 3) || (cfg >= 256 && v3_listed(cfg - 256))))
    return mhb_set_error(MHB_ERR_ARG, "unknown sort configuration %d", cfg);
  g_sort_cfg = cfg;
  return MHB_OK;
}
static int sort_cfg() {
  int &cfg = g_sort_cfg;
  if (cfg < 0) {
    const char *e = getenv("MHB_SORT_CFG");
    cfg = e ? atoi(e) : 256 + MHB_V3_DEFAULT;
    if (!((cfg >= 0 && cfg <= 3) || (cfg >= 256 && v3_listed(cfg - 256)))) cfg = 256 + MHB_V3_DEFAULT;
  }
  return cfg;
}
template <int WR, int CFG>
static u64 sort_tiles_cfg(u64 n) {
  return (n + SortCfg<WR, CFG>::TILE - 1) / SortCfg<WR, CFG>::TILE;
}
template <int WR, int CFG>
static u64 sort_tiles_cfg3(u64 n) {
  return (n + SortCfg3<WR, CFG>::TILE - 1) / SortCfg3<WR, CFG>::TILE;
}
template <int WR>
static u64 sort_tiles(u64 n) {
  const int cfg = sort_cfg();
  if (cfg >= 256) {
    if constexpr (WR == 2 || WR == 3) {
#define X(B) \
  if (cfg - 256 == B) return sort_tiles_cfg3<WR, B>(n);
      MHB_V3_LIST(X)
#undef X
    }
    return sort_tiles_cfg3<WR, MHB_V3_DEFAULT>(n);
  }
  if constexpr (WR <= 3) {
    switch (cfg) {
      case 1: return sort_tiles_cfg<WR, 1>(n);
      case 2: return sort_tiles_cfg<WR, 2>(n);
      case 3: return sort_tiles_cfg<WR, 3>(n);
      default: break;
    }
  }
  return sort_tiles_cfg<WR, 0>(n);
}
static u64 sort_num_tiles(u64 n, u32 words) {
#define M(WW) \
  if (words == WW) return sort_tiles<WW>(n);
  MHB_FOR_WR(M)
#undef M
  return 0;
}
static constexpr size_t kSortHeadBytes = (size_t)(72 + 1) * 256 * 8  + 256 * 8  + 128 * 4 + 256 * 8 ;
static size_t lb_bytes(u64 tiles) { return (size_t)tiles * 256 * 8 + (size_t)((tiles + 3) / 4) * 256 * 16; }

extern "C" size_t mhb_sort_workspace_bytes(uint64_t n, uint32_t words) {
  u64 tiles = sort_num_tiles(n, words);
  if (words <= 3) tiles = (n + 256 * 8 - 1) / (256 * 8) > tiles ? (n + 256 * 8 - 1) / (256 * 8) : tiles;
#define M(WW) \
  if (words == WW && sort_tiles_cfg<WW, 0>(n) > tiles) tiles = sort_tiles_cfg<WW, 0>(n);
  MHB_FOR_WR(M)
#undef M
  return kSortHeadBytes + lb_bytes(tiles) + 256;
}

template <int WR, int CFG>
static int launch_radix_pass_cfg(cudaStream_t st, const u32 *in, u64 n, int byte_idx, const u64 *bin_base,
                                 u64 *lookback, u32 *tile_counter, u64 *next_hist, int next_byte, u32 epoch) {
  using C = SortCfg<WR, CFG>;
  static int blocks_per_sm = 0;
  if (!blocks_per_sm) {
    CK(cudaFuncSetAttribute(k_radix_pass<WR, CFG>, cudaFuncAttributeMaxDynamicSharedMemorySize, (int)C::SMEM));
    CK(cudaOccupancyMaxActiveBlocksPerMultiprocessor(&blocks_per_sm, k_radix_pass<WR, CFG>, C::THREADS, C::SMEM));
    if (blocks_per_sm < 1) return mhb_set_error(MHB_ERR_CUDA, "radix pass kernel (WR=%d) does not fit an SM", WR);
    if (getenv("MHB_VERBOSE")) fprintf(stderr, "[mhb] radix pass WR=%d cfg=%d: %d threads x %d rec, %zu B smem, %d CTA/SM\n", WR, CFG, C::THREADS, C::IPT, C::SMEM, blocks_per_sm);
  }
  const u64 tiles = sort_tiles_cfg<WR, CFG>(n);
  u64 grid = (u64)blocks_per_sm * sm_count();
  if (grid > tiles) grid = tiles;
  k_radix_pass<WR, CFG><<<(int)grid, C::THREADS, C::SMEM, st>>>(in, n, (u32)tiles, byte_idx, bin_base, lookback,
                                                                 tile_counter, next_hist, next_byte, epoch);
  CK_LAUNCH();
  return MHB_OK;
}

template <int WR, int CFG>
static int launch_radix_pass_cfg3(cudaStream_t st, const u32 *in, u64 n, int byte_idx, const u64 *bin_base,
                                  u64 *lookback, u32 *tile_counter, u64 *next_hist, int next_byte, u32 epoch) {
  using C = SortCfg3<WR, CFG>;
  static int blocks_per_sm = 0;
  if (!blocks_per_sm) {
    CK(cudaFuncSetAttribute(k_radix_pass3<WR, CFG, false, true>, cudaFuncAttributeMaxDynamicSharedMemorySize, (int)C::SMEM));
    CK(cudaFuncSetAttribute(k_radix_pass3<WR, CFG, false, false>, cudaFuncAttributeMaxDynamicSharedMemorySize, (int)C::SMEM));
    CK(cudaOccupancyMaxActiveBlocksPerMultiprocessor(&blocks_per_sm, k_radix_pass3<WR, CFG, false, true>, C::THREADS, C::SMEM));
    if (blocks_per_sm < 1) return mhb_set_error(MHB_ERR_CUDA, "radix pass v3 kernel (WR=%d) does not fit an SM", WR);
    if (getenv("MHB_VERBOSE")) fprintf(stderr, "[mhb] radix pass v3 WR=%d bits=0x%03x: %d threads x %d rec, rank %d, prefetch %d, look-back %d/%d, batch %d, early %d, %zu B smem, %d CTA/SM\n", WR, CFG, C::THREADS, C::IPT, C::RANK, (int)C::PREFETCH, C::LB1, C::LBW, (int)C::BATCH, (int)C::EARLY, C::SMEM, blocks_per_sm);
  }
  const u64 tiles = sort_tiles_cfg3<WR, CFG>(n);
  u64 grid = (u64)blocks_per_sm * sm_count();
  if (grid > tiles) grid = tiles;
  if (next_hist)
    k_radix_pass3<WR, CFG, false, true><<<(int)grid, C::THREADS, C::SMEM, st>>>(in, n, (u32)tiles, byte_idx, bin_base, lookback,
                                                                                 tile_counter, next_hist, next_byte, epoch);
  else
    k_radix_pass3<WR, CFG, false, false><<<(int)grid, C::THREADS, C::SMEM, st>>>(in, n, (u32)tiles, byte_idx, bin_base, lookback,
                                                                                  tile_counter, nullptr, 0, epoch);
  CK_LAUNCH();
  return MHB_OK;
}

template <int WR>
static int launch_part_unstable(cudaStream_t st, const u32 *in, u64 n, int byte_idx, const u64 *bin_base,
                                unsigned long long *gcursor, u32 *tile_counter, u64 *next_hist, int next_byte,
                                const uint8_t *lut) {
  using C = PartCfg<WR>;
  static int bps = 0;
  if (!bps) {
    CK(cudaFuncSetAttribute(k_part_unstable<WR, false, true>, cudaFuncAttributeMaxDynamicSharedMemorySize, (int)C::SMEM));
    CK(cudaFuncSetAttribute(k_part_unstable<WR, false, false>, cudaFuncAttributeMaxDynamicSharedMemorySize, (int)C::SMEM));
    CK(cudaFuncSetAttribute(k_part_unstable<WR, true, false>, cudaFuncAttributeMaxDynamicSharedMemorySize, (int)C::SMEM));
    CK(cudaFuncSetAttribute(k_part_unstable<WR, true, true>, cudaFuncAttributeMaxDynamicSharedMemorySize, (int)C::SMEM_OWNER_HIST));
    CK(cudaOccupancyMaxActiveBlocksPerMultiprocessor(&bps, k_part_unstable<WR, false, true>, C::THREADS, C::SMEM));
    if (bps < 1) return mhb_set_error(MHB_ERR_CUDA, "partition pass (WR=%d) does not fit an SM", WR);
    if (getenv("MHB_VERBOSE")) fprintf(stderr, "[mhb] unstable partition pass WR=%d: %d threads x %d rec, %zu B smem, %d CTA/SM\n", WR, C::THREADS, C::IPT, C::SMEM, bps);
  }
  const u64 tiles = (n + C::TILE - 1) / C::TILE;
  u64 grid = (u64)bps * sm_count();
  if (grid > tiles) grid = tiles;
  if (lut && next_hist)
    k_part_unstable<WR, true, true><<<(int)grid, C::THREADS, C::SMEM_OWNER_HIST, st>>>(in, n, (u32)tiles, byte_idx, bin_base, gcursor,
                                                                                       tile_counter, next_hist, next_byte, lut);
  else if (lut)
    k_part_unstable<WR, true, false><<<(int)grid, C::THREADS, C::SMEM, st>>>(in, n, (u32)tiles, byte_idx, bin_base, gcursor,
                                                                             tile_counter, nullptr, 0, lut);
  else if (next_hist)
    k_part_unstable<WR, false, true><<<(int)grid, C::THREADS, C::SMEM, st>>>(in, n, (u32)tiles, byte_idx, bin_base, gcursor,
                                                                             tile_counter, next_hist, next_byte, nullptr);
  else
    k_part_unstable<WR, false, false><<<(int)grid, C::THREADS, C::SMEM, st>>>(in, n, (u32)tiles, byte_idx, bin_base, gcursor,
                                                                              tile_counter, nullptr, 0, nullptr);
  CK_LAUNCH();
  return MHB_OK;
}

template <int WR>
static int launch_radix_pass(cudaStream_t st, const u32 *in, u64 n, int byte_idx, const u64 *bin_base,
                             u64 *lookback, u32 *tile_counter, u64 *next_hist, int next_byte, u32 epoch) {
  const int cfg = sort_cfg();
  if (cfg >= 256) {
    if constexpr (WR == 2 || WR == 3) {
#define X(B) \
  if (cfg - 256 == B) return launch_radix_pass_cfg3<WR, B>(st, in, n, byte_idx, bin_base, lookback, tile_counter, next_hist, next_byte, epoch);
      MHB_V3_LIST(X)
#undef X
    }
    return launch_radix_pass_cfg3<WR, MHB_V3_DEFAULT>(st, in, n, byte_idx, bin_base, lookback, tile_counter, next_hist, next_byte, epoch);
  }
  if constexpr (WR <= 3) {
    switch (cfg) {
      case 1: return launch_radix_pass_cfg<WR, 1>(st, in, n, byte_idx, bin_base, lookback, tile_counter, next_hist, next_byte, epoch);
      case 2: return launch_radix_pass_cfg<WR, 2>(st, in, n, byte_idx, bin_base, lookback, tile_counter, next_hist, next_byte, epoch);
      case 3: return launch_radix_pass_cfg<WR, 3>(st, in, n, byte_idx, bin_base, lookback, tile_counter, next_hist, next_byte, epoch);
      default: break;
    }
  }
  return launch_radix_pass_cfg<WR, 0>(st, in, n, byte_idx, bin_base, lookback, tile_counter, next_hist, next_byte, epoch);
}

#ifdef MHB_SORT_TIMELINE
extern "C" int mhb_debug_set_sort_timeline(unsigned long long *dev_buf, unsigned long long rows) {
  CK(cudaMemcpyToSymbol(g_sort_timeline, &dev_buf, sizeof(dev_buf)));
  CK(cudaMemcpyToSymbol(g_sort_timeline_rows, &rows, sizeof(rows)));
  return MHB_OK;
}
#endif

namespace {
struct SortTrace {
  cudaEvent_t ev[74];
  bool created = false;
  uint32_t n_passes = 0, words = 0;
  uint64_t n = 0;
};
SortTrace g_trace[4];
uint64_t g_trace_seq = 0;
}

int mhb_sort_records_ex(void *stream, uint32_t *a, uint32_t *b, uint64_t n, uint32_t words, const uint8_t *bytes,
                        uint32_t n_bytes, const uint64_t *first_hist, void *ws, size_t ws_bytes, int *result_in_b,
                        double *pass_ms_host, int relaxed);
int mhb_sort_records_impl(void *stream, uint32_t *a, uint32_t *b, uint64_t n, uint32_t words, const uint8_t *bytes,
                          uint32_t n_bytes, const uint64_t *first_hist, void *ws, size_t ws_bytes, int *result_in_b,
                          double *pass_ms_host) {
  return mhb_sort_records_ex(stream, a, b, n, words, bytes, n_bytes, first_hist, ws, ws_bytes, result_in_b, pass_ms_host, 1);
}
int mhb_sort_records_ex(void *stream, uint32_t *a, uint32_t *b, uint64_t n, uint32_t words, const uint8_t *bytes,
                          uint32_t n_bytes, const uint64_t *first_hist, void *ws, size_t ws_bytes, int *result_in_b,
                        double *pass_ms_host, int relaxed) {
  static const bool stable_first = getenv("MHB_SORT_STABLE_FIRST") != nullptr;
  if (stable_first) relaxed = 0;
  if (words < 1 || words > 17 || n_bytes > 72 || !result_in_b)
    return mhb_set_error(MHB_ERR_ARG, "bad sort geometry (words=%u n_bytes=%u)", words, n_bytes);
  *result_in_b = 0;
  if (n == 0 || n_bytes == 0) return MHB_OK;
  if (ws_bytes < mhb_sort_workspace_bytes(n, words)) return mhb_set_error(MHB_ERR_ARG, "sort workspace too small");
  if (n >= (1ull << 53)) return mhb_set_error(MHB_ERR_ARG, "too many records");
  cudaStream_t st = (cudaStream_t)stream;
  u64 *hist = (u64 *)ws;
  u64 *bin_base = hist + (72 + 1) * 256;
  u32 *tile_counter = (u32 *)(bin_base + 256);
  unsigned long long *gcursor = (unsigned long long *)(tile_counter + 128);
  u64 *lookback = (u64 *)((char *)ws + kSortHeadBytes);
  CK(cudaMemsetAsync(ws, 0, kSortHeadBytes + lb_bytes(sort_num_tiles(n, words)) + 256, st));
  if (first_hist) {
    CK(cudaMemcpyAsync(hist, first_hist, 256 * 8, cudaMemcpyDeviceToDevice, st));
  } else {
#define M(WW) \
  if (words == WW) k_hist_byte<WW><<<sm_count() * 4, 256, 0, st>>>(a, n, bytes[0], hist);
    MHB_FOR_WR(M)
#undef M
    CK_LAUNCH();
  }
  SortTrace &tr = g_trace[g_trace_seq++ & 3];
  if (!tr.created) {
    for (int i = 0; i < 74; ++i) CK(cudaEventCreate(&tr.ev[i]));
    tr.created = true;
  }
  tr.n_passes = n_bytes;
  tr.words = words;
  tr.n = n;
  CK(cudaEventRecord(tr.ev[0], st));
  u32 *in = a, *out = b;
  for (u32 p = 0; p < n_bytes; ++p) {
    k_hist_scan256<<<1, 256, 0, st>>>(hist + (u64)p * 256, bin_base, (u64)(uintptr_t)out, words * 4);
    CK_LAUNCH();
    u64 *next_hist = p + 1 < n_bytes ? hist + (u64)(p + 1) * 256 : nullptr;
    const int next_byte = p + 1 < n_bytes ? bytes[p + 1] : 0;
    int rc = MHB_ERR_ARG;
    if (p == 0 && relaxed && words == 2) rc = launch_part_unstable<2>(st, in, n, bytes[p], bin_base, gcursor, tile_counter + p, next_hist, next_byte, nullptr);
    else if (p == 0 && relaxed && words == 3) rc = launch_part_unstable<3>(st, in, n, bytes[p], bin_base, gcursor, tile_counter + p, next_hist, next_byte, nullptr);
    else {
#define M(WW) \
  if (words == WW) rc = launch_radix_pass<WW>(st, in, n, bytes[p], bin_base, lookback, tile_counter + p, next_hist, next_byte, p + 1);
      MHB_FOR_WR(M)
#undef M
    }
    if (rc) return rc;
    CK(cudaEventRecord(tr.ev[p + 1], st));
    u32 *t = in;
    in = out;
    out = t;
  }
  *result_in_b = (in == b) ? 1 : 0;
  if (pass_ms_host) {
    CK(cudaEventSynchronize(tr.ev[n_bytes]));
    for (u32 p = 0; p < n_bytes; ++p) {
      float ms = 0;
      CK(cudaEventElapsedTime(&ms, tr.ev[p], tr.ev[p + 1]));
      pass_ms_host[p] = ms;
    }
  }
  return MHB_OK;
}

template <int WR>
static int launch_partition_pass(cudaStream_t st, const u32 *in, u64 n, int byte_idx, const u64 *bin_addr, u64 *lookback,
                                 u32 *tile_counter, const uint8_t *lut) {
  using C = SortCfg<WR, 0>;
  static int blocks_per_sm = 0;
  if (!blocks_per_sm) {
    CK(cudaFuncSetAttribute(k_radix_pass<WR, 0, true>, cudaFuncAttributeMaxDynamicSharedMemorySize, (int)C::SMEM));
    CK(cudaOccupancyMaxActiveBlocksPerMultiprocessor(&blocks_per_sm, k_radix_pass<WR, 0, true>, C::THREADS, C::SMEM));
    if (blocks_per_sm < 1) return mhb_set_error(MHB_ERR_CUDA, "partition pass kernel (WR=%d) does not fit an SM", WR);
  }
  const u64 tiles = sort_tiles_cfg<WR, 0>(n);
  u64 grid = (u64)blocks_per_sm * sm_count();
  if (grid > tiles) grid = tiles;
  k_radix_pass<WR, 0, true><<<(int)grid, C::THREADS, C::SMEM, st>>>(in, n, (u32)tiles, byte_idx, bin_addr, lookback,
                                                                     tile_counter, nullptr, 0, 1, lut);
  CK_LAUNCH();
  return MHB_OK;
}

static int partition_scatter_impl(void *stream, const uint32_t *recs, uint64_t n, uint32_t words, int byte,
                                  const uint8_t *owner_of_byte_dev, const uint64_t *bin_addr_dev, void *ws, size_t ws_bytes,
                                  int next_byte, uint64_t *owner_next_hist, int *hist_done);
extern "C" int mhb_partition_scatter(void *stream, const uint32_t *recs, uint64_t n, uint32_t words, int byte,
                                     const uint8_t *owner_of_byte_dev, const uint64_t *bin_addr_dev, void *ws,
                                     size_t ws_bytes) {
  return partition_scatter_impl(stream, recs, n, words, byte, owner_of_byte_dev, bin_addr_dev, ws, ws_bytes, 0, nullptr, nullptr);
}
extern "C" int mhb_partition_scatter_hist(void *stream, const uint32_t *recs, uint64_t n, uint32_t words, int byte,
                                          const uint8_t *owner_of_byte_dev, const uint64_t *bin_addr_dev, void *ws,
                                          size_t ws_bytes, int next_byte, uint64_t *owner_next_hist, int *hist_done) {
  if (!owner_of_byte_dev || !owner_next_hist || !hist_done || next_byte < 0 || next_byte >= (int)(4 * words))
    return mhb_set_error(MHB_ERR_ARG, "bad owner-histogram arguments");
  return partition_scatter_impl(stream, recs, n, words, byte, owner_of_byte_dev, bin_addr_dev, ws, ws_bytes, next_byte,
                                owner_next_hist, hist_done);
}
static int partition_scatter_impl(void *stream, const uint32_t *recs, uint64_t n, uint32_t words, int byte,
                                  const uint8_t *owner_of_byte_dev, const uint64_t *bin_addr_dev, void *ws, size_t ws_bytes,
                                  int next_byte, uint64_t *owner_next_hist, int *hist_done) {
  if (hist_done) *hist_done = 0;
  if (words < 1 || words > 17 || byte < 0 || byte >= (int)(4 * words)) return mhb_set_error(MHB_ERR_ARG, "bad geometry");
  if (n == 0) return MHB_OK;
  u64 tiles = 0;
#define M(WW) \
  if (words == WW) tiles = sort_tiles_cfg<WW, 0>(n);
  MHB_FOR_WR(M)
#undef M
  const size_t need = kSortHeadBytes + (size_t)tiles * 256 * 8 + 256;
  if (ws_bytes < need) return mhb_set_error(MHB_ERR_ARG, "sort workspace too small");
  cudaStream_t st = (cudaStream_t)stream;
  u64 *hist = (u64 *)ws;
  u32 *tile_counter = (u32 *)(hist + (72 + 1) * 256 + 256);
  u64 *lookback = (u64 *)((char *)ws + kSortHeadBytes);
  CK(cudaMemsetAsync(ws, 0, need, st));
  int rc = MHB_ERR_ARG;
  static const bool stable_first = getenv("MHB_SORT_STABLE_FIRST") != nullptr;
  if (owner_of_byte_dev && !stable_first && (words == 2 || words == 3)) {
    unsigned long long *gcursor = (unsigned long long *)(tile_counter + 128);
    rc = words == 2 ? launch_part_unstable<2>(st, recs, n, byte, bin_addr_dev, gcursor, tile_counter, owner_next_hist, next_byte, owner_of_byte_dev)
                    : launch_part_unstable<3>(st, recs, n, byte, bin_addr_dev, gcursor, tile_counter, owner_next_hist, next_byte, owner_of_byte_dev);
    if (!rc && owner_next_hist && hist_done) *hist_done = 1;
  } else if (owner_of_byte_dev) {
#define M(WW) \
  if (words == WW) rc = launch_partition_pass<WW>(st, recs, n, byte, bin_addr_dev, lookback, tile_counter, owner_of_byte_dev);
    MHB_FOR_WR(M)
#undef M
  } else {
#define M(WW) \
  if (words == WW) rc = launch_radix_pass_cfg<WW, 0>(st, recs, n, byte, bin_addr_dev, lookback, tile_counter, nullptr, 0, 1);
    MHB_FOR_WR(M)
#undef M
  }
  return rc;
}

extern "C" int mhb_dev_malloc(void **ptr, size_t bytes) {
  CK(cudaMalloc(ptr, bytes));
  return MHB_OK;
}
extern "C" int mhb_dev_free(void *ptr) {
  CK(cudaFree(ptr));
  return MHB_OK;
}
extern "C" int mhb_ipc_export(const void *dev_ptr, uint8_t *handle64) {
  static_assert(sizeof(cudaIpcMemHandle_t) == 64, "handle size");
  cudaIpcMemHandle_t h;
  CK(cudaIpcGetMemHandle(&h, const_cast<void *>(dev_ptr)));
  memcpy(handle64, &h, 64);
  return MHB_OK;
}
extern "C" int mhb_ipc_open(const uint8_t *handle64, void **peer_ptr) {
  cudaIpcMemHandle_t h;
  memcpy(&h, handle64, 64);
  CK(cudaIpcOpenMemHandle(peer_ptr, h, cudaIpcMemLazyEnablePeerAccess));
  return MHB_OK;
}
extern "C" int mhb_ipc_close(void *peer_ptr) {
  CK(cudaIpcCloseMemHandle(peer_ptr));
  return MHB_OK;
}

extern "C" int mhb_sort_pass_ms(int back, double *pass_ms, uint32_t max_passes, uint32_t *n_passes, uint64_t *n_records,
                                uint32_t *words) {
  if (back < 0 || back > 3 || (uint64_t)back >= g_trace_seq) return mhb_set_error(MHB_ERR_ARG, "no such sort in the trace ring");
  SortTrace &tr = g_trace[(g_trace_seq - 1 - back) & 3];
  CK(cudaEventSynchronize(tr.ev[tr.n_passes]));
  for (u32 p = 0; p < tr.n_passes && p < max_passes; ++p) {
    float ms = 0;
    CK(cudaEventElapsedTime(&ms, tr.ev[p], tr.ev[p + 1]));
    pass_ms[p] = ms;
  }
  if (n_passes) *n_passes = tr.n_passes;
  if (n_records) *n_records = tr.n;
  if (words) *words = tr.words;
  return MHB_OK;
}

extern "C" int mhb_sort_records(void *stream, uint32_t *a, uint32_t *b, uint64_t n, uint32_t words,
                                const uint8_t *bytes, uint32_t n_bytes, const uint64_t *first_hist, void *ws,
                                size_t ws_bytes, int *result_in_b) {
  return mhb_sort_records_ex(stream, a, b, n, words, bytes, n_bytes, first_hist, ws, ws_bytes, result_in_b, nullptr, 0);
}

extern "C" int mhb_sort_records_relaxed(void *stream, uint32_t *a, uint32_t *b, uint64_t n, uint32_t words,
                                        const uint8_t *bytes, uint32_t n_bytes, const uint64_t *first_hist, void *ws,
                                        size_t ws_bytes, int *result_in_b) {
  return mhb_sort_records_ex(stream, a, b, n, words, bytes, n_bytes, first_hist, ws, ws_bytes, result_in_b, nullptr, 1);
}
```

### megahit_b200/dev.py

```python
from __future__ import annotations

import ctypes as C
import os

import numpy as np
import torch

from . import lib


def _ptr(t):
    return C.c_void_p(t.data_ptr()) if t is not None else None


def _stream():
    return C.c_void_p(torch.cuda.current_stream().cuda_stream)


def sort_records(a: torch.Tensor, b: torch.Tensor, n: int, words: int, sort_bytes, first_hist=None, ws=None, relaxed=False):
    L = lib.load()
    need = L.mhb_sort_workspace_bytes(n, words)
    if ws is None or ws.numel() < need:
        ws = torch.empty(need, dtype=torch.uint8, device=a.device)
    bytes_arr = (C.c_uint8 * len(sort_bytes))(*sort_bytes)
    in_b = C.c_int(0)
    fn = L.mhb_sort_records_relaxed if relaxed else L.mhb_sort_records
    lib._check(fn(_stream(), _ptr(a), _ptr(b), n, words, bytes_arr, len(sort_bytes), _ptr(first_hist), _ptr(ws), ws.numel(),
                  C.byref(in_b)))
    return b if in_b.value else a


class CountPlan:

    def __init__(self, n_reads: int, read_len: int, k: int, m: int, device, want_mercy: bool = True, mode: str | None = None):
        import os
        L = lib.load()
        self.L, self.k, self.m, self.n_reads, self.read_len, self.device = L, k, m, n_reads, read_len, device
        self.want_mercy = want_mercy
        mode = mode or os.environ.get("MHB_COUNT_MODE") or "auto"
        ok = bool(L.mhb_count_hashed_supported(k, m))
        if mode == "hashed" and not ok:
            raise lib.MhbError(f"hashed count is not available for k={k}, m={m}")
        self.hashed = ok and mode in ("hashed", "auto")
        self.n = n_reads * (read_len - k) if read_len >= k + 1 else 0
        self.WR, self.WE = lib.count_record_words(k), lib.words_per_edge(k)
        self.sort_bytes = lib.count_sort_bytes(k)
        n = self.n
        i32 = dict(dtype=torch.int32, device=device)
        self.a = torch.empty(n * self.WR + 4, **i32)
        self.b = torch.empty(n * self.WR + 4, **i32)
        if self.hashed:
            self.ws = torch.empty(L.mhb_count_hashed_workspace_bytes(n, k, m), dtype=torch.uint8, device=device)
            self.scratch = None
        else:
            self.ws = torch.empty(L.mhb_sort_workspace_bytes(n, self.WR), dtype=torch.uint8, device=device)
            self.scratch = torch.empty(L.mhb_count_solid_scratch_bytes(n), dtype=torch.uint8, device=device)
        self.cap_edges = n // max(1, m) + 1
        self.edges = torch.empty(self.cap_edges * self.WE, **i32)
        self.aux = torch.empty(self.cap_edges, dtype=torch.uint8, device=device)
        self.mul_hist = torch.zeros(65536, dtype=torch.int64, device=device)
        self.hist0 = torch.zeros(256, dtype=torch.int64, device=device)
        self.n_solid_dev = torch.zeros(8, dtype=torch.int64, device=device)
        self.first = torch.empty(n_reads + 1, **i32) if want_mercy else None
        self.last = torch.empty(n_reads + 1, **i32) if want_mercy else None
        self.tipset = None
        self.events = {}

    def _reads(self, bin_dev: torch.Tensor) -> lib.DevReads:
        return lib.DevReads(bin_dev.data_ptr(), bin_dev.numel(), self.n_reads, self.read_len, None, None)

    def _mark(self, name):
        ev = torch.cuda.Event(enable_timing=True)
        ev.record()
        self.events.setdefault(name, []).append(ev)

    def extract(self, bin_dev):
        self.hist0.zero_()
        lib._check(self.L.mhb_count_extract(_stream(), C.byref(self._reads(bin_dev)), self.k, _ptr(self.a), self.n,
                                            _ptr(self.hist0), 5 if self.hashed else self.sort_bytes[0]))

    def sort(self):
        if self.hashed:
            return None
        self.sorted = sort_records(self.a, self.b, self.n, self.WR, self.sort_bytes, self.hist0, self.ws, relaxed=True)
        return self.sorted

    def count(self):
        self.mul_hist.zero_()
        self.n_solid_dev.zero_()
        if self.hashed:
            lib._check(self.L.mhb_count_solid_hashed(_stream(), _ptr(self.a), _ptr(self.b), self.n, self.k, self.m,
                                                     _ptr(self.hist0), _ptr(self.edges), _ptr(self.aux), self.cap_edges,
                                                     _ptr(self.mul_hist), _ptr(self.n_solid_dev), _ptr(self.ws), self.ws.numel()))
            return
        lib._check(self.L.mhb_count_solid(_stream(), _ptr(self.sorted), self.n, self.k, self.m, _ptr(self.edges),
                                          _ptr(self.aux), self.cap_edges, _ptr(self.mul_hist), _ptr(self.n_solid_dev),
                                          _ptr(self.scratch), self.scratch.numel()))

    def mercy(self, bin_dev):
        n_solid = int(self.n_solid_dev[0].item())
        n_tip = C.c_uint64(0)
        lib._check(self.L.mhb_count_tip_edges(_stream(), _ptr(self.aux), n_solid, C.byref(n_tip)))
        need = self.L.mhb_tipset_bytes(n_tip.value, self.k)
        if self.tipset is None or self.tipset.numel() < need:
            self.tipset = torch.empty(need, dtype=torch.uint8, device=self.device)
        lib._check(self.L.mhb_tipset_build(_stream(), _ptr(self.edges), _ptr(self.aux), n_solid, self.k,
                                           _ptr(self.tipset), need, n_tip.value))
        lib._check(self.L.mhb_count_mark_mercy(_stream(), C.byref(self._reads(bin_dev)), self.k, _ptr(self.tipset),
                                               need, n_tip.value, _ptr(self.first), _ptr(self.last)))
        return n_solid, n_tip.value

    def mercy_edges(self, bin_dev: torch.Tensor, n_solid: int) -> int:
        L = self.L
        if not hasattr(self, "cand"):
            self.cand = torch.empty(self.n_reads + 1, dtype=torch.int64, device=self.device)
            self.cand_scratch = torch.empty(L.mhb_mercy_candidates_scratch_bytes(self.n_reads), dtype=torch.uint8, device=self.device)
            self.mercy_scratch = None
        nc = C.c_uint64(0)
        lib._check(L.mhb_mercy_candidates(_stream(), _ptr(self.first), _ptr(self.last), self.n_reads, _ptr(self.cand), C.byref(nc),
                                          _ptr(self.cand_scratch), self.cand_scratch.numel()))
        self.n_cand = nc.value
        if not self.n_cand:
            return 0
        need = L.mhb_mercy_edges_scratch_bytes(self.n_cand, self.read_len)
        if self.mercy_scratch is None or self.mercy_scratch.numel() < need:
            self.mercy_scratch = torch.empty(int(need * 1.2), dtype=torch.uint8, device=self.device)
        nm = C.c_uint64(0)
        lib._check(L.mhb_mercy_edges(_stream(), C.byref(self._reads(bin_dev)), _ptr(self.cand), self.n_cand, self.read_len, self.k,
                                     _ptr(self.edges), n_solid, C.c_void_p(self.edges.data_ptr() + n_solid * self.WE * 4),
                                     self.cap_edges - n_solid, C.byref(nm), _ptr(self.mercy_scratch), self.mercy_scratch.numel()))
        return nm.value

    def run(self, bin_dev: torch.Tensor, timed: bool = False):
        if timed:
            self._mark("t0")
        self.extract(bin_dev)
        if timed:
            self._mark("extract")
        self.sort()
        if timed:
            self._mark("sort")
        self.count()
        if timed:
            self._mark("count")
        if self.want_mercy:
            n_solid, _ = self.mercy(bin_dev)
        else:
            n_solid = int(self.n_solid_dev[0].item())
        if timed:
            self._mark("mercy")
        return n_solid

    def edges_host(self, n_solid: int) -> np.ndarray:
        return self.edges[: n_solid * self.WE].cpu().numpy().view(np.uint32).reshape(-1, self.WE)


class S2sPlan:

    def __init__(self, n_seqs: int, seq_len: int, k: int, device):
        L = lib.load()
        self.L, self.k, self.n_seqs, self.seq_len, self.device = L, k, n_seqs, seq_len, device
        self.W = lib.s2s_record_words(k)
        self.sort_bytes = lib.s2s_sort_bytes(k)
        self.n_items = n_seqs * 2 * (seq_len - k + 2)
        n = self.n_items
        i32 = dict(dtype=torch.int32, device=device)
        self.a = torch.empty(n * self.W + 4, **i32)
        self.b = torch.empty(n * self.W + 4, **i32)
        self.ws = torch.empty(L.mhb_sort_workspace_bytes(n, self.W), dtype=torch.uint8, device=device)
        self.scratch = torch.empty(L.mhb_s2s_emit_scratch_bytes(n, k), dtype=torch.uint8, device=device)
        wpt = (k + 15) // 16
        self.cap_bytes = n * (4 + 4 * wpt) + 16
        self.bytes = torch.empty(self.cap_bytes, dtype=torch.uint8, device=device)
        self.table = torch.zeros(65536 * 4, dtype=torch.int64, device=device)
        self.totals = torch.zeros(16, dtype=torch.int64, device=device)
        self.hist0 = torch.zeros(256, dtype=torch.int64, device=device)
        self.cursor = torch.zeros(1, dtype=torch.int64, device=device)
        self.events = []

    def run(self, words: torch.Tensor, mult: torch.Tensor | None = None, n_seqs: int | None = None, stride: int = 0,
            timed: bool = False, aux: torch.Tensor | None = None, n_aux: int = 0):
        n_seqs = self.n_seqs if n_seqs is None else n_seqs
        assert n_seqs <= self.n_seqs
        self.n_items = n_seqs * 2 * (self.seq_len - self.k + 2)
        if aux is not None and mult is None and not os.environ.get("MHB_S2S_NO_PRUNE"):
            return self._run_pruned(words, n_seqs, aux, n_aux, timed)
        seqs = lib.DevSeqs(words.data_ptr(), words.numel(), n_seqs, self.seq_len, None, None, None,
                           mult.data_ptr() if mult is not None else None, stride)
        self.hist0.zero_()
        ev = [torch.cuda.Event(enable_timing=True) for _ in range(4)] if timed else None
        if timed:
            ev[0].record()
        lib._check(self.L.mhb_s2s_extract(_stream(), C.byref(seqs), self.k, _ptr(self.a), self.n_items, _ptr(self.hist0),
                                          self.sort_bytes[0]))
        if timed:
            ev[1].record()
        srt = sort_records(self.a, self.b, self.n_items, self.W, self.sort_bytes, self.hist0, self.ws, relaxed=True)
        if timed:
            ev[2].record()
        lib._check(self.L.mhb_s2s_emit(_stream(), _ptr(srt), self.n_items, self.k, _ptr(self.bytes), self.cap_bytes,
                                       _ptr(self.table), _ptr(self.totals), _ptr(self.scratch), self.scratch.numel()))
        if timed:
            ev[3].record()
            self.events.append(ev)
        return self.totals

    def _run_pruned(self, edges: torch.Tensor, n_edges: int, aux: torch.Tensor, n_aux: int, timed: bool):
        cap = self.n_items
        self.hist0.zero_()
        self.cursor.zero_()
        ev = [torch.cuda.Event(enable_timing=True) for _ in range(4)] if timed else None
        if timed:
            ev[0].record()
        lib._check(self.L.mhb_s2s_extract_edges_pruned(_stream(), _ptr(edges), _ptr(aux), n_edges, n_aux, self.k, _ptr(self.a),
                                                       cap, _ptr(self.cursor), _ptr(self.hist0), self.sort_bytes[0]))
        self.n_items = int(self.cursor.item())
        assert self.n_items <= cap
        if timed:
            ev[1].record()
        srt = sort_records(self.a, self.b, self.n_items, self.W, self.sort_bytes, self.hist0, self.ws, relaxed=True)
        if timed:
            ev[2].record()
        lib._check(self.L.mhb_s2s_emit(_stream(), _ptr(srt), self.n_items, self.k, _ptr(self.bytes), self.cap_bytes,
                                       _ptr(self.table), _ptr(self.totals), _ptr(self.scratch), self.scratch.numel()))
        if timed:
            ev[3].record()
            self.events.append(ev)
        return self.totals
```

### megahit_b200/lib.py

```python
from __future__ import annotations

import ctypes as C
import os

import numpy as np

_HERE = os.path.dirname(os.path.abspath(__file__))
LIB_PATH = os.environ.get("MHB_LIB") or os.path.join(_HERE, "libmhb.so")
NUM_BUCKETS = 65536
SENTINEL_OFFSET = 0xFFFFFFFF

_lib = None


class MhbError(RuntimeError):
    pass


class DevReads(C.Structure):
    _fields_ = [("bin", C.c_void_p), ("bin_words", C.c_uint64), ("n_reads", C.c_uint64), ("fixed_len", C.c_uint32),
                ("rec_off", C.c_void_p), ("edge_off", C.c_void_p)]


class DevSeqs(C.Structure):
    _fields_ = [("words", C.c_void_p), ("n_words", C.c_uint64), ("n_seqs", C.c_uint64), ("fixed_len", C.c_uint32),
                ("word_off", C.c_void_p), ("len", C.c_void_p), ("item_off", C.c_void_p), ("mult", C.c_void_p),
                ("fixed_stride", C.c_uint32)]


class CountArgs(C.Structure):
    _fields_ = [("k", C.c_uint32), ("m", C.c_int32), ("bin", C.c_void_p), ("bin_words", C.c_uint64),
                ("n_reads", C.c_uint64), ("want_mercy", C.c_int)]


class CountResult(C.Structure):
    _fields_ = [("n_edge_records", C.c_uint64), ("n_solid", C.c_uint64), ("words_per_edge", C.c_uint32),
                ("edges", C.POINTER(C.c_uint32)), ("n_cand", C.c_uint64), ("cand_ids", C.POINTER(C.c_uint64)),
                ("n_has_tips", C.c_uint64), ("counting", C.c_int64 * 65536),
                ("t_h2d_ms", C.c_double), ("t_extract_ms", C.c_double), ("t_sort_ms", C.c_double),
                ("t_count_ms", C.c_double), ("t_mercy_ms", C.c_double), ("t_d2h_ms", C.c_double),
                ("t_total_ms", C.c_double), ("n_sort_passes", C.c_uint32), ("n_rounds", C.c_uint32), ("sort_pass_ms", C.c_double * 64)]


class S2sArgs(C.Structure):
    _fields_ = [("k", C.c_uint32), ("words", C.c_void_p), ("word_off", C.c_void_p), ("len", C.c_void_p),
                ("mult", C.c_void_p), ("n_seqs", C.c_uint64)]


class S2sResult(C.Structure):
    _fields_ = [("n_records", C.c_uint64), ("n_items", C.c_uint64), ("n_tips", C.c_uint64),
                ("n_large_mul", C.c_uint64), ("n_bytes", C.c_uint64), ("words_per_tip_label", C.c_uint32),
                ("bytes", C.POINTER(C.c_uint8)), ("bucket_table", C.c_uint64 * (65536 * 4)),
                ("w_count", C.c_uint64 * 9), ("ones_in_last", C.c_uint64),
                ("t_total_ms", C.c_double), ("t_extract_ms", C.c_double), ("t_sort_ms", C.c_double),
                ("t_emit_ms", C.c_double)]


class BuildArgs(C.Structure):
    _fields_ = [("k", C.c_uint32), ("m", C.c_int32), ("bin", C.c_void_p), ("bin_words", C.c_uint64),
                ("n_reads", C.c_uint64), ("need_mercy", C.c_int32), ("want_edges", C.c_int32),
                ("sdbg_out", C.c_void_p), ("sdbg_out_capacity", C.c_uint64)]


class BuildResult(C.Structure):
    _fields_ = [("n_edge_records", C.c_uint64), ("n_solid", C.c_uint64), ("n_cand", C.c_uint64), ("n_mercy", C.c_uint64),
                ("n_sort_items", C.c_uint64), ("words_per_edge", C.c_uint32), ("words_per_tip_label", C.c_uint32),
                ("n_items", C.c_uint64), ("n_tips", C.c_uint64), ("n_large_mul", C.c_uint64), ("n_bytes", C.c_uint64),
                ("bytes", C.POINTER(C.c_uint8)), ("bucket_table", C.POINTER(C.c_uint64)), ("w_count", C.c_uint64 * 9),
                ("ones_in_last", C.c_uint64), ("edges", C.POINTER(C.c_uint32)), ("cand_ids", C.POINTER(C.c_uint64)),
                ("counting", C.POINTER(C.c_int64)),
                ("t_total_ms", C.c_double), ("t_h2d_ms", C.c_double), ("t_count_ms", C.c_double),
                ("t_mercy_ms", C.c_double), ("t_s2s_ms", C.c_double), ("t_d2h_ms", C.c_double),
                ("n_rounds_s1", C.c_uint32), ("n_rounds_s2", C.c_uint32)]


class CountOpts(C.Structure):
    _fields_ = [("k", C.c_uint32), ("m", C.c_int32), ("host_mem", C.c_double), ("num_cpu_threads", C.c_int32),
                ("read_lib_file", C.c_char_p), ("output_prefix", C.c_char_p), ("mem_flag", C.c_int32)]


class Seq2SdbgOpts(C.Structure):
    _fields_ = [("host_mem", C.c_double), ("k", C.c_uint32), ("k_from", C.c_uint32), ("num_cpu_threads", C.c_int32),
                ("contig", C.c_char_p), ("bubble", C.c_char_p), ("addi_contig", C.c_char_p),
                ("local_contig", C.c_char_p), ("input_prefix", C.c_char_p), ("output_prefix", C.c_char_p),
                ("need_mercy", C.c_int32), ("mem_flag", C.c_int32)]


class Read2SdbgOpts(C.Structure):
    _fields_ = [("k", C.c_uint32), ("m", C.c_int32), ("host_mem", C.c_double), ("num_cpu_threads", C.c_int32),
                ("read_lib_file", C.c_char_p), ("output_prefix", C.c_char_p), ("mem_flag", C.c_int32),
                ("need_mercy", C.c_int32)]


class IterateArgs(C.Structure):
    _fields_ = [("k", C.c_uint32), ("step", C.c_uint32), ("contig_words", C.c_void_p), ("contig_word_off", C.c_void_p),
                ("contig_len", C.c_void_p), ("n_contigs", C.c_uint64), ("bin", C.c_void_p), ("bin_words", C.c_uint64),
                ("n_reads", C.c_uint64)]


class IterateResult(C.Structure):
    _fields_ = [("n_flanks", C.c_uint64), ("n_aligned_reads", C.c_uint64), ("n_candidates", C.c_uint64), ("n_edges", C.c_uint64),
                ("words_per_edge", C.c_uint32), ("edges", C.POINTER(C.c_uint32)), ("t_total_ms", C.c_double)]


class IterateOpts(C.Structure):
    _fields_ = [("contig_file", C.c_char_p), ("bubble_file", C.c_char_p), ("read_file", C.c_char_p),
                ("num_cpu_threads", C.c_int32), ("k", C.c_uint32), ("step", C.c_uint32), ("output_prefix", C.c_char_p)]


SYMBOLS = [
    "mhb_last_error", "mhb_version", "mhb_device_count", "mhb_launch_count", "mhb_count_record_words", "mhb_words_per_edge",
    "mhb_s2s_record_words", "mhb_count_sort_bytes", "mhb_s2s_sort_bytes", "mhb_sort_workspace_bytes",
    "mhb_count_extract", "mhb_check_fixed_len", "mhb_count_extract_range", "mhb_set_round_limit", "mhb_set_s2s_round_limit", "mhb_set_r2s_round_limit", "mhb_plan_rounds", "mhb_plan_rounds16", "mhb_sort_records", "mhb_sort_records_relaxed", "mhb_sort_pass_ms", "mhb_set_sort_cfg", "mhb_partition_scatter", "mhb_partition_scatter_hist", "mhb_plan_partition", "mhb_compact_tip_edges", "mhb_dev_malloc", "mhb_dev_free",
    "mhb_ipc_export", "mhb_ipc_open", "mhb_ipc_close", "mhb_count_solid_scratch_bytes", "mhb_count_solid", "mhb_count_hashed_supported", "mhb_count_hashed_workspace_bytes", "mhb_count_solid_hashed", "mhb_tipset_bytes",
    "mhb_tipset_build", "mhb_count_mark_mercy", "mhb_count_tip_edges", "mhb_s2s_extract", "mhb_s2s_extract_range",
    "mhb_s2s_emit_scratch_bytes", "mhb_s2s_emit", "mhb_set_device", "mhb_count_host", "mhb_s2s_host", "mhb_build_host", "mhb_free",
    "mhb_mercy_candidates_scratch_bytes", "mhb_mercy_candidates", "mhb_mercy_edges_scratch_bytes", "mhb_mercy_edges", "mhb_mercy_edges_count", "mhb_mercy_edges_write", "mhb_mercy_edges_segs", "mhb_mercy_host", "mhb_mercy_planes_words", "mhb_mercy_probe_owned", "mhb_mercy_count_planes", "mhb_edge_lut_bytes", "mhb_edge_lut_build",
    "mhb_release", "mhb_count_run", "mhb_count_run_multi", "mhb_seq2sdbg_run", "mhb_selftest_count_record", "mhb_selftest_count_records_roll", "mhb_selftest_s2s_record",
    "mhb_iterate_host", "mhb_iterate_run", "mhb_selftest_iterate", "mhb_s2s_extract_edges_pruned", "mhb_s2s_emit_fmt", "mhb_read2sdbg_host", "mhb_read2sdbg_run", "mhb_selftest_r2s_s1_record", "mhb_selftest_r2s_item",
    "mhb_selftest_kmsort", "mhb_selftest_kmsort_smem", "mhb_selftest_r2s_s1_group", "mhb_selftest_r2s_mercy_read",
]


def load():
    global _lib
    if _lib is not None:
        return _lib
    if not os.path.exists(LIB_PATH):
        raise MhbError(f"{LIB_PATH} is missing: build it with `make -C megahit_b200/csrc` "
                       "(there is no CPU fallback for the CUDA path)")
    L = C.CDLL(LIB_PATH)
    L.mhb_last_error.restype = C.c_char_p
    L.mhb_version.restype = C.c_char_p
    for f in ("mhb_count_record_words", "mhb_words_per_edge", "mhb_s2s_record_words", "mhb_count_sort_bytes",
              "mhb_s2s_sort_bytes"):
        getattr(L, f).restype = C.c_uint32
    for f in ("mhb_sort_workspace_bytes", "mhb_count_solid_scratch_bytes", "mhb_tipset_bytes",
              "mhb_s2s_emit_scratch_bytes"):
        getattr(L, f).restype = C.c_size_t
    L.mhb_sort_workspace_bytes.argtypes = [C.c_uint64, C.c_uint32]
    L.mhb_count_solid_scratch_bytes.argtypes = [C.c_uint64]
    L.mhb_tipset_bytes.argtypes = [C.c_uint64, C.c_uint32]
    L.mhb_s2s_emit_scratch_bytes.argtypes = [C.c_uint64, C.c_uint32]
    L.mhb_count_extract.argtypes = [C.c_void_p, C.POINTER(DevReads), C.c_uint32, C.c_void_p, C.c_uint64, C.c_void_p,
                                    C.c_int]
    L.mhb_sort_records.argtypes = [C.c_void_p, C.c_void_p, C.c_void_p, C.c_uint64, C.c_uint32, C.c_void_p, C.c_uint32,
                                   C.c_void_p, C.c_void_p, C.c_size_t, C.POINTER(C.c_int)]
    L.mhb_sort_records_relaxed.argtypes = L.mhb_sort_records.argtypes
    L.mhb_count_solid.argtypes = [C.c_void_p, C.c_void_p, C.c_uint64, C.c_uint32, C.c_int32, C.c_void_p, C.c_void_p,
                                  C.c_uint64, C.c_void_p, C.c_void_p, C.c_void_p, C.c_size_t]
    L.mhb_count_hashed_workspace_bytes.restype = C.c_size_t
    L.mhb_count_hashed_workspace_bytes.argtypes = [C.c_uint64, C.c_uint32, C.c_int32]
    L.mhb_count_hashed_supported.argtypes = [C.c_uint32, C.c_int32]
    L.mhb_count_solid_hashed.argtypes = [C.c_void_p, C.c_void_p, C.c_void_p, C.c_uint64, C.c_uint32, C.c_int32, C.c_void_p,
                                         C.c_void_p, C.c_void_p, C.c_uint64, C.c_void_p, C.c_void_p, C.c_void_p, C.c_size_t]
    L.mhb_tipset_build.argtypes = [C.c_void_p, C.c_void_p, C.c_void_p, C.c_uint64, C.c_uint32, C.c_void_p, C.c_size_t,
                                   C.c_uint64]
    L.mhb_count_mark_mercy.argtypes = [C.c_void_p, C.POINTER(DevReads), C.c_uint32, C.c_void_p, C.c_size_t, C.c_uint64,
                                       C.c_void_p, C.c_void_p]
    L.mhb_count_tip_edges.argtypes = [C.c_void_p, C.c_void_p, C.c_uint64, C.POINTER(C.c_uint64)]
    L.mhb_s2s_extract.argtypes = [C.c_void_p, C.POINTER(DevSeqs), C.c_uint32, C.c_void_p, C.c_uint64, C.c_void_p,
                                  C.c_int]
    L.mhb_s2s_emit.argtypes = [C.c_void_p, C.c_void_p, C.c_uint64, C.c_uint32, C.c_void_p, C.c_uint64, C.c_void_p,
                               C.c_void_p, C.c_void_p, C.c_size_t]
    L.mhb_count_host.argtypes = [C.POINTER(CountArgs), C.POINTER(CountResult)]
    L.mhb_s2s_host.argtypes = [C.POINTER(S2sArgs), C.POINTER(S2sResult)]
    L.mhb_build_host.argtypes = [C.POINTER(BuildArgs), C.POINTER(BuildResult)]
    L.mhb_mercy_candidates_scratch_bytes.restype = C.c_size_t
    L.mhb_mercy_candidates_scratch_bytes.argtypes = [C.c_uint64]
    L.mhb_mercy_edges_scratch_bytes.restype = C.c_size_t
    L.mhb_mercy_edges_scratch_bytes.argtypes = [C.c_uint64, C.c_uint32]
    L.mhb_mercy_candidates.argtypes = [C.c_void_p, C.c_void_p, C.c_void_p, C.c_uint64, C.c_void_p, C.POINTER(C.c_uint64),
                                       C.c_void_p, C.c_size_t]
    L.mhb_mercy_edges.argtypes = [C.c_void_p, C.POINTER(DevReads), C.c_void_p, C.c_uint64, C.c_uint32, C.c_uint32,
                                  C.c_void_p, C.c_uint64, C.c_void_p, C.c_uint64, C.POINTER(C.c_uint64), C.c_void_p,
                                  C.c_size_t]
    L.mhb_mercy_edges_segs.argtypes = [C.c_void_p, C.POINTER(DevReads), C.c_void_p, C.c_uint64, C.c_uint32, C.c_uint32,
                                       C.c_uint32, C.c_void_p, C.c_void_p, C.c_void_p, C.c_void_p, C.c_void_p, C.c_uint64,
                                       C.POINTER(C.c_uint64), C.c_void_p, C.c_size_t]
    L.mhb_mercy_edges_count.argtypes = [C.c_void_p, C.POINTER(DevReads), C.c_void_p, C.c_uint64, C.c_uint32, C.c_uint32,
                                        C.c_uint32, C.c_void_p, C.c_void_p, C.c_void_p, C.c_void_p, C.POINTER(C.c_uint64),
                                        C.c_void_p, C.c_size_t]
    L.mhb_mercy_edges_write.argtypes = [C.c_void_p, C.POINTER(DevReads), C.c_void_p, C.c_uint64, C.c_uint32, C.c_uint32,
                                        C.c_void_p, C.c_uint64, C.c_uint64, C.c_void_p, C.c_size_t]
    L.mhb_mercy_planes_words.restype = C.c_size_t
    L.mhb_mercy_planes_words.argtypes = [C.c_uint64, C.c_uint32]
    L.mhb_mercy_probe_owned.argtypes = [C.c_void_p, C.POINTER(DevReads), C.c_void_p, C.c_uint64, C.c_uint32, C.c_uint32,
                                        C.c_void_p, C.c_uint64, C.c_void_p, C.c_void_p, C.c_uint32, C.c_void_p]
    L.mhb_mercy_count_planes.argtypes = [C.c_void_p, C.POINTER(DevReads), C.c_void_p, C.c_uint64, C.c_uint32, C.c_uint32,
                                         C.c_void_p, C.c_uint32, C.c_uint64, C.POINTER(C.c_uint64), C.c_void_p, C.c_size_t]
    L.mhb_plan_partition.argtypes = [C.c_void_p, C.c_void_p, C.c_uint32, C.c_uint32, C.c_uint32, C.c_void_p, C.c_void_p,
                                     C.c_void_p, C.c_void_p]
    L.mhb_edge_lut_bytes.restype = C.c_size_t
    L.mhb_edge_lut_build.argtypes = [C.c_void_p, C.c_void_p, C.c_uint64, C.c_uint32, C.c_void_p]
    L.mhb_sort_pass_ms.argtypes = [C.c_int, C.c_void_p, C.c_uint32, C.POINTER(C.c_uint32), C.POINTER(C.c_uint64),
                                   C.POINTER(C.c_uint32)]
    L.mhb_set_device.argtypes = [C.c_int]
    L.mhb_partition_scatter.argtypes = [C.c_void_p, C.c_void_p, C.c_uint64, C.c_uint32, C.c_int, C.c_void_p, C.c_void_p,
                                        C.c_void_p, C.c_size_t]
    L.mhb_partition_scatter_hist.argtypes = [C.c_void_p, C.c_void_p, C.c_uint64, C.c_uint32, C.c_int, C.c_void_p, C.c_void_p,
                                             C.c_void_p, C.c_size_t, C.c_int, C.c_void_p, C.POINTER(C.c_int)]
    L.mhb_dev_malloc.argtypes = [C.POINTER(C.c_void_p), C.c_size_t]
    L.mhb_dev_free.argtypes = [C.c_void_p]
    L.mhb_ipc_export.argtypes = [C.c_void_p, C.c_void_p]
    L.mhb_ipc_open.argtypes = [C.c_void_p, C.POINTER(C.c_void_p)]
    L.mhb_ipc_close.argtypes = [C.c_void_p]
    L.mhb_free.argtypes = [C.c_void_p]
    L.mhb_count_run.argtypes = [C.POINTER(CountOpts)]
    L.mhb_seq2sdbg_run.argtypes = [C.POINTER(Seq2SdbgOpts)]
    L.mhb_selftest_count_record.argtypes = [C.c_void_p, C.c_uint32, C.c_uint32, C.c_uint32, C.c_uint32, C.c_void_p,
                                            C.POINTER(C.c_uint32)]
    L.mhb_selftest_count_records_roll.argtypes = [C.c_void_p, C.c_uint32, C.c_uint32, C.c_uint32, C.c_uint32, C.c_void_p,
                                                  C.c_void_p]
    L.mhb_selftest_s2s_record.argtypes = [C.c_void_p, C.c_uint32, C.c_uint32, C.c_uint32, C.c_uint32, C.c_uint32,
                                          C.c_uint32, C.c_void_p]
    L.mhb_s2s_emit_fmt.argtypes = L.mhb_s2s_emit.argtypes + [C.c_int]
    L.mhb_iterate_host.argtypes = [C.POINTER(IterateArgs), C.POINTER(IterateResult)]
    L.mhb_selftest_iterate.argtypes = [C.POINTER(IterateArgs), C.POINTER(IterateResult)]
    L.mhb_iterate_run.argtypes = [C.POINTER(IterateOpts)]
    L.mhb_s2s_extract_edges_pruned.argtypes = [C.c_void_p, C.c_void_p, C.c_void_p, C.c_uint64, C.c_uint64, C.c_uint32,
                                               C.c_void_p, C.c_uint64, C.c_void_p, C.c_void_p, C.c_int]
    L.mhb_read2sdbg_host.argtypes = [C.POINTER(BuildArgs), C.POINTER(BuildResult)]
    L.mhb_read2sdbg_run.argtypes = [C.POINTER(Read2SdbgOpts)]
    L.mhb_selftest_r2s_s1_record.argtypes = [C.c_void_p, C.c_uint32, C.c_uint32, C.c_uint32, C.c_uint32, C.c_uint64, C.c_void_p]
    L.mhb_selftest_r2s_item.argtypes = [C.c_void_p, C.c_uint32, C.c_uint32, C.c_uint32, C.c_uint32, C.c_uint32, C.c_uint32,
                                        C.c_void_p, C.POINTER(C.c_uint32)]
    L.mhb_selftest_kmsort.argtypes = [C.c_void_p, C.c_uint64, C.c_uint32]
    L.mhb_selftest_kmsort_smem.argtypes = [C.c_void_p, C.c_uint64, C.c_uint32, C.c_uint32, C.c_uint32]
    L.mhb_selftest_r2s_s1_group.argtypes = [C.c_void_p, C.c_uint64, C.c_uint32, C.c_int32, C.c_uint32, C.c_uint64, C.c_int,
                                            C.c_void_p, C.c_void_p, C.c_void_p, C.c_void_p, C.c_void_p]
    L.mhb_selftest_r2s_mercy_read.argtypes = [C.c_uint32, C.c_uint64, C.c_uint64, C.c_uint32, C.c_void_p, C.c_void_p, C.c_void_p,
                                              C.c_void_p, C.c_void_p, C.POINTER(C.c_uint32)]
    _lib = L
    return L


def _check(rc: int):
    if rc != 0:
        raise MhbError(f"libmhb error {rc}: {load().mhb_last_error().decode()}")


def device_count() -> int:
    return load().mhb_device_count()


def launch_count() -> int:
    L = load()
    L.mhb_launch_count.restype = C.c_uint64
    return int(L.mhb_launch_count())


def plan_rounds(hist256, max_records: int):
    L = load()
    h = np.ascontiguousarray(hist256, dtype=np.uint64)
    assert h.shape == (256,)
    lo, hi = (C.c_uint32 * 256)(), (C.c_uint32 * 256)()
    L.mhb_plan_rounds.argtypes = [C.c_void_p, C.c_uint64, C.c_void_p, C.c_void_p]
    n = L.mhb_plan_rounds(h.ctypes.data, int(max_records), lo, hi)
    if n < 0:
        raise MhbError(L.mhb_last_error().decode())
    return [(int(lo[i]), int(hi[i])) for i in range(n)]


def plan_rounds16(hist256, sub_hist, max_records: int, cap: int = 65536):
    L = load()
    h = np.ascontiguousarray(hist256, dtype=np.uint64)
    sub = None if sub_hist is None else np.ascontiguousarray(sub_hist, dtype=np.uint64).reshape(256, 256)
    lo, hi = (C.c_uint32 * cap)(), (C.c_uint32 * cap)()
    L.mhb_plan_rounds16.argtypes = [C.c_void_p, C.c_void_p, C.c_uint64, C.c_void_p, C.c_void_p, C.c_uint32]
    n = L.mhb_plan_rounds16(h.ctypes.data, sub.ctypes.data if sub is not None else None, int(max_records), lo, hi, cap)
    if n < 0:
        raise MhbError(L.mhb_last_error().decode())
    return [(int(lo[i]), int(hi[i])) for i in range(n)]


def set_round_limit(max_records: int = 0):
    L = load()
    L.mhb_set_round_limit.argtypes = [C.c_uint64]
    _check(L.mhb_set_round_limit(int(max_records)))


def set_s2s_round_limit(max_items: int = 0):
    L = load()
    L.mhb_set_s2s_round_limit.argtypes = [C.c_uint64]
    _check(L.mhb_set_s2s_round_limit(int(max_items)))


def set_r2s_round_limit(s1: int = 0, s2: int = 0):
    L = load()
    L.mhb_set_r2s_round_limit.argtypes = [C.c_uint64, C.c_uint64]
    _check(L.mhb_set_r2s_round_limit(int(s1), int(s2)))


def mercy_host(k: int, edges: np.ndarray, cand_bin: np.ndarray) -> np.ndarray:
    L = load()
    we = words_per_edge(k)
    edges = np.ascontiguousarray(edges, np.uint32).reshape(-1, we)
    cand = np.ascontiguousarray(cand_bin, np.uint32).reshape(-1)
    out, nm, nr = C.POINTER(C.c_uint32)(), C.c_uint64(), C.c_uint64()
    L.mhb_mercy_host.argtypes = [C.c_uint32, C.c_void_p, C.c_uint64, C.c_void_p, C.c_uint64, C.POINTER(C.POINTER(C.c_uint32)),
                                 C.POINTER(C.c_uint64), C.POINTER(C.c_uint64)]
    _check(L.mhb_mercy_host(k, edges.ctypes.data if len(edges) else None, len(edges), cand.ctypes.data if len(cand) else None,
                            len(cand), C.byref(out), C.byref(nm), C.byref(nr)))
    res = np.ctypeslib.as_array(out, (max(nm.value, 1) * we,))[: nm.value * we].reshape(-1, we).copy()
    L.mhb_free(out)
    return res


# ... 253 lines not shown
```

Measured before the change: 15.96 billion.

## Fuse count extraction with first radix partition pass for hashed counting

```diff
diff --git a/include/mhb.h b/include/mhb.h
--- a/include/mhb.h
+++ b/include/mhb.h
@@ -87,6 +87,14 @@
                            const uint64_t *hist_byte5, uint32_t *edges_out, uint8_t *aux_out, uint64_t capacity_edges,
                            uint64_t *mul_hist, uint64_t *n_solid_out, void *ws, size_t ws_bytes);
 
+int mhb_count_extract_hist(void *stream, const mhb_dev_reads *reads, uint32_t k, uint64_t n_edges, uint64_t *hist_byte5);
+size_t mhb_count_extract_part_workspace_bytes(void);
+int mhb_count_extract_part(void *stream, const mhb_dev_reads *reads, uint32_t k, uint32_t *records, uint64_t n_edges,
+                           const uint64_t *hist_byte5, uint64_t *hist_byte6, void *ws, size_t ws_bytes);
+int mhb_count_solid_hashed_part(void *stream, uint32_t *recs_a, uint32_t *recs_b, uint64_t n, uint32_t k, int32_t m,
+                                const uint64_t *hist_byte6, uint32_t *edges_out, uint8_t *aux_out, uint64_t capacity_edges,
+                                uint64_t *mul_hist, uint64_t *n_solid_out, void *ws, size_t ws_bytes);
+
 size_t mhb_tipset_bytes(uint64_t n_tip_edges, uint32_t k);
 int mhb_tipset_build(void *stream, const uint32_t *edges, const uint8_t *aux, uint64_t n_solid, uint32_t k,
                      void *tipset, size_t tipset_bytes, uint64_t n_tip_edges);
diff --git a/megahit_b200/csrc/mhb_countpart.cuh b/megahit_b200/csrc/mhb_countpart.cuh
--- /dev/null
+++ b/megahit_b200/csrc/mhb_countpart.cuh
@@ -0,0 +1,205 @@
+#pragma once
+#include "mhb_count.cuh"
+#include "mhb_part.cuh"
+
+namespace mhb {
+
+__device__ __forceinline__ const u32 *cx_read(const ReadsView &rv, u64 r, u32 &L) {
+  const u32 *p = rv.bin + rv.rec_start(r);
+  L = rv.fixed_len ? rv.fixed_len : p[0];
+  return p + 1;
+}
+
+__device__ __forceinline__ void cx_locate(const ReadsView &rv, u32 k, u64 e, u64 &r, u32 &q) {
+  if (rv.fixed_len) {
+    const u32 ne = rv.fixed_len - k;
+    if (e >> 32) {
+      r = e / ne;
+      q = (u32)(e - r * ne);
+    } else {
+      const u32 r32 = (u32)e / ne;
+      r = r32;
+      q = (u32)e - r32 * ne;
+    }
+  } else {
+    u64 lo = 0, hi = rv.n_reads - 1;
+    while (lo < hi) {
+      const u64 mid = (lo + hi + 1) >> 1;
+      if (rv.edge_off[mid] <= e) lo = mid;
+      else hi = mid - 1;
+    }
+    r = lo;
+    q = (u32)(e - rv.edge_off[lo]);
+  }
+}
+
+template <int R, int W, bool PREV_NEXT>
+__device__ __forceinline__ void cx_records(const ReadsView &rv, u32 k, u64 e, u64 n, u64 (&rec)[R]) {
+  u64 r;
+  u32 q, L;
+  cx_locate(rv, k, e, r, q);
+  const u32 *s = cx_read(rv, r, L);
+  u32 j0 = 0;
+  if constexpr (W == 2) {
+    u32 strand[R];
+    make_count_records_roll<R, PREV_NEXT>(s, div_ceil(L, 16), L, k, q, rec, strand);
+    j0 = L - k - q < (u32)R ? L - k - q : (u32)R;
+    q += j0;
+  }
+#pragma unroll
+  for (int j = 0; j < R; ++j) {
+    if ((u32)j < j0 || e + j >= n) continue;
+    while (q + k >= L) {
+      ++r;
+      s = cx_read(rv, r, L);
+      q = 0;
+    }
+    u32 t[2], strand;
+    make_count_record<W, 2>(s, div_ceil(L, 16), L, k, q, t, strand);
+    rec[j] = ((u64)t[0] << 32) | t[1];
+    ++q;
+  }
+}
+
+__device__ __forceinline__ void cx_prefetch_l2(const u32 *a, const u32 *b) {
+  const u64 a0 = ((u64)a + 15) & ~15ull, a1 = (u64)b & ~15ull;
+  for (u64 x = a0; x < a1; x += 16384) {
+    const u32 sz = (u32)(a1 - x < 16384 ? a1 - x : 16384);
+    asm volatile("cp.async.bulk.prefetch.L2.global [%0], %1;" ::"l"(x), "r"(sz) : "memory");
+  }
+}
+
+__device__ __forceinline__ u32 cx_byte(u64 rec, u32 byte) { return (u32)(rec >> (8 * byte)) & 255u; }
+
+static constexpr int kCxHistThreads = 256;
+static constexpr int kCxHistGroup = 8;
+
+template <int W>
+__global__ void __launch_bounds__(kCxHistThreads, 4)
+    k_count_hist5(ReadsView rv, u32 k, u64 n, unsigned long long *__restrict__ hist) {
+  __shared__ u32 s_hist[256];
+  for (int i = threadIdx.x; i < 256; i += kCxHistThreads) s_hist[i] = 0;
+  __syncthreads();
+  constexpr int R = kCxHistGroup;
+  const u64 n_groups = (n + R - 1) / R;
+  for (u64 g = (u64)blockIdx.x * kCxHistThreads + threadIdx.x; g < n_groups; g += (u64)gridDim.x * kCxHistThreads) {
+    u64 rec[R];
+    cx_records<R, W, false>(rv, k, R * g, n, rec);
+#pragma unroll
+    for (int j = 0; j < R; ++j)
+      if (R * g + j < n) red_shared_inc(&s_hist[cx_byte(rec[j], 5)]);
+  }
+  __syncthreads();
+  for (int i = threadIdx.x; i < 256; i += kCxHistThreads)
+    if (s_hist[i]) atomicAdd(&hist[i], (unsigned long long)s_hist[i]);
+}
+
+struct CxPartCfg {
+  static constexpr int THREADS = 384;
+  static constexpr int GROUP = 4;
+  static constexpr int GROUPS = 4;
+  static constexpr int IPT = GROUP * GROUPS;
+  static constexpr int TILE = THREADS * IPT;
+  static constexpr size_t SMEM = 256 * 8  + 4 * 256 * 4  + 16 * 4 + (size_t)TILE * 8;
+};
+
+template <int W>
+__global__ void __launch_bounds__(CxPartCfg::THREADS, 2)
+    k_count_extract_part(ReadsView rv, u32 k, u64 n, u32 num_tiles,
+                         const u64 *__restrict__ bin_addr ,
+                         unsigned long long *gcursor , u32 *tile_counter ,
+                         unsigned long long *next_hist ) {
+  using C = CxPartCfg;
+  constexpr int THREADS = C::THREADS, R = C::GROUP, G = C::GROUPS, IPT = C::IPT, TILE = C::TILE;
+  extern __shared__ __align__(16) unsigned char smem_raw[];
+  u64 *s_base = reinterpret_cast<u64 *>(smem_raw);
+  u32 *s_cnt = reinterpret_cast<u32 *>(s_base + 256);
+  u32 *s_off = s_cnt + 256;
+  u32 *s_cur = s_off + 256;
+  u32 *s_next = s_cur + 256;
+  u32 *s_misc = s_next + 256;
+  u32 *s_recs = s_misc + 16;
+  const u32 tid = threadIdx.x, lane = tid & 31, warp = tid >> 5;
+  for (int i = tid; i < 256; i += THREADS) {
+    s_cnt[i] = 0;
+    s_next[i] = 0;
+  }
+  if (tid == 0) s_misc[0] = atomicAdd(tile_counter, 1u);
+  __syncthreads();
+  u32 tile = s_misc[0];
+  while (tile < num_tiles) {
+    u32 next_ticket = 0;
+    if (tid == 0) next_ticket = atomicAdd(tile_counter, 1u);
+    const u64 tile_base = (u64)tile * TILE;
+    const u32 valid = tile_base + TILE <= n ? (u32)TILE : (u32)(n - tile_base);
+    u64 rec[G][R];
+#pragma unroll
+    for (int i = 0; i < G; ++i) {
+      const u32 p = R * (tid + (u32)i * THREADS);
+      if (p < valid) cx_records<R, W, true>(rv, k, tile_base + p, n, rec[i]);
+    }
+#pragma unroll
+    for (int i = 0; i < G; ++i)
+#pragma unroll
+      for (int j = 0; j < R; ++j)
+        if (R * (tid + (u32)i * THREADS) + j < valid) red_shared_inc(&s_cnt[cx_byte(rec[i][j], 5)]);
+    if (tid == 0 && rv.fixed_len && next_ticket < num_tiles) {
+      const u64 ne = rv.fixed_len - k, e0 = (u64)next_ticket * TILE;
+      const u64 e1 = e0 + TILE < n ? e0 + TILE : n;
+      cx_prefetch_l2(rv.bin + (e0 / ne) * rv.fixed_stride, rv.bin + ((e1 - 1) / ne + 1) * rv.fixed_stride);
+    }
+    __syncthreads();
+    if (tid < 256) {
+      const u32 c = s_cnt[tid];
+      const unsigned long long g = c ? atomicAdd(&gcursor[tid], (unsigned long long)c) : 0ull;
+      u32 inc = c;
+#pragma unroll
+      for (int dd = 1; dd < 32; dd <<= 1) {
+        const u32 t = __shfl_up_sync(0xffffffffu, inc, dd);
+        if (lane >= (u32)dd) inc += t;
+      }
+      if (lane == 31) s_misc[4 + warp] = inc;
+      s_off[tid] = inc - c;
+      s_base[tid] = bin_addr[tid] + g * 8ull;
+    }
+    __syncthreads();
+    if (tid < 256) {
+      u32 add = 0;
+#pragma unroll
+      for (int w = 0; w < 7; ++w) add += (warp > (u32)w) ? s_misc[4 + w] : 0u;
+      const u32 o = s_off[tid] + add;
+      s_off[tid] = o;
+      s_cur[tid] = o;
+    }
+    if (tid == 0) s_misc[0] = next_ticket;
+    __syncthreads();
+#pragma unroll
+    for (int i = 0; i < G; ++i)
+#pragma unroll
+      for (int j = 0; j < R; ++j)
+        if (R * (tid + (u32)i * THREADS) + j < valid) {
+          const u32 q[2] = {(u32)(rec[i][j] >> 32), (u32)rec[i][j]};
+          st_shared_rec<2>(s_recs, atom_shared_inc_ret(&s_cur[cx_byte(rec[i][j], 5)]), q);
+        }
+    __syncthreads();
+    const u32 next_tile = s_misc[0];
+#pragma unroll
+    for (int i = 0; i < IPT; ++i) {
+      const u32 p = (u32)i * THREADS + tid;
+      if (p < valid) {
+        u32 q[2];
+        ld_rec<2>(s_recs, p, q);
+        const u32 dd = rec_digit<2>(q, 0, 1);
+        st_global_rec<2>(s_base[dd] + (u64)(p - s_off[dd]) * 8, q);
+        red_shared_inc(&s_next[rec_digit<2>(q, 0, 2)]);
+      }
+    }
+    for (int i = tid; i < 256; i += THREADS) s_cnt[i] = 0;
+    __syncthreads();
+    tile = next_tile;
+  }
+  for (int i = tid; i < 256; i += THREADS)
+    if (s_next[i]) atomicAdd(&next_hist[i], (unsigned long long)s_next[i]);
+}
+
+}
diff --git a/megahit_b200/csrc/mhb_hashcount.cu b/megahit_b200/csrc/mhb_hashcount.cu
--- a/megahit_b200/csrc/mhb_hashcount.cu
+++ b/megahit_b200/csrc/mhb_hashcount.cu
@@ -528,20 +528,21 @@
   return hc_layout(n, m).total;
 }
 
-extern "C" int mhb_count_solid_hashed(void *stream, uint32_t *recs_a, uint32_t *recs_b, uint64_t n, uint32_t k, int32_t m,
-                                      const uint64_t *hist_byte5, uint32_t *edges_out, uint8_t *aux_out,
-                                      uint64_t capacity_edges, uint64_t *mul_hist, uint64_t *n_solid_out, void *ws,
-                                      size_t ws_bytes) {
+static int count_solid_hashed(cudaStream_t st, uint32_t *recs_a, uint32_t *recs_b, uint64_t n, uint32_t k, int32_t m,
+                              bool pre_partitioned, const uint64_t *first_hist, uint32_t *edges_out, uint8_t *aux_out,
+                              uint64_t capacity_edges, uint64_t *mul_hist, uint64_t *n_solid_out, void *ws, size_t ws_bytes) {
   if (!mhb_count_hashed_supported(k, m)) return mhb_set_error(MHB_ERR_ARG, "hashed count needs 8-byte records (13 <= k <= 28) and 1 <= m <= %d", kHcHist);
   if (!mul_hist || !n_solid_out || !ws) return mhb_set_error(MHB_ERR_ARG, "bad args");
   if (n == 0) return MHB_OK;
   if (n >= (1ull << 40)) return mhb_set_error(MHB_ERR_ARG, "too many records for one hashed count call");
   const HcLayout L = hc_layout(n, m);
   if (ws_bytes < L.total) return mhb_set_error(MHB_ERR_ARG, "hashed count workspace too small (%zu < %zu)", ws_bytes, L.total);
-  cudaStream_t st = (cudaStream_t)stream;
   const uint8_t bytes[3] = {5, 6, 7};
   int in_b = 0;
-  if (int rc = mhb_sort_records_impl(st, recs_a, recs_b, n, 2, bytes, 3, hist_byte5, ws, L.sort_ws, &in_b, nullptr)) return rc;
+  if (int rc = pre_partitioned
+                   ? mhb_sort_records_ex(st, recs_a, recs_b, n, 2, bytes + 1, 2, first_hist, ws, L.sort_ws, &in_b, nullptr, 0)
+                   : mhb_sort_records_impl(st, recs_a, recs_b, n, 2, bytes, 3, first_hist, ws, L.sort_ws, &in_b, nullptr))
+    return rc;
   const uint2 *recs = (const uint2 *)(in_b ? recs_b : recs_a);
   char *w = (char *)ws;
   u64 *bounds = (u64 *)(w + L.off_bounds);
@@ -573,3 +574,19 @@
   CK_LAUNCH();
   return MHB_OK;
 }
+
+extern "C" int mhb_count_solid_hashed(void *stream, uint32_t *recs_a, uint32_t *recs_b, uint64_t n, uint32_t k, int32_t m,
+                                      const uint64_t *hist_byte5, uint32_t *edges_out, uint8_t *aux_out,
+                                      uint64_t capacity_edges, uint64_t *mul_hist, uint64_t *n_solid_out, void *ws,
+                                      size_t ws_bytes) {
+  return count_solid_hashed((cudaStream_t)stream, recs_a, recs_b, n, k, m, false, hist_byte5, edges_out, aux_out,
+                            capacity_edges, mul_hist, n_solid_out, ws, ws_bytes);
+}
+
+extern "C" int mhb_count_solid_hashed_part(void *stream, uint32_t *recs_a, uint32_t *recs_b, uint64_t n, uint32_t k,
+                                           int32_t m, const uint64_t *hist_byte6, uint32_t *edges_out, uint8_t *aux_out,
+                                           uint64_t capacity_edges, uint64_t *mul_hist, uint64_t *n_solid_out, void *ws,
+                                           size_t ws_bytes) {
+  return count_solid_hashed((cudaStream_t)stream, recs_a, recs_b, n, k, m, true, hist_byte6, edges_out, aux_out,
+                            capacity_edges, mul_hist, n_solid_out, ws, ws_bytes);
+}
diff --git a/megahit_b200/csrc/mhb_host.cu b/megahit_b200/csrc/mhb_host.cu
--- a/megahit_b200/csrc/mhb_host.cu
+++ b/megahit_b200/csrc/mhb_host.cu
@@ -184,11 +184,12 @@
 }
 int run_count_stage(cudaStream_t st, const CountWork &cw, uint32_t *d_a, uint32_t *d_b, uint64_t n, uint32_t k, int32_t m,
                     const uint64_t *d_hist0, uint32_t *d_edges, uint8_t *d_aux, uint64_t cap_edges, uint64_t *d_mul_hist,
-                    uint64_t *d_nsolid, char *work, double *pass_ms, uint32_t *n_passes) {
+                    uint64_t *d_nsolid, char *work, double *pass_ms, uint32_t *n_passes, bool partitioned = false) {
   const uint32_t WR = count_record_words(k);
   if (cw.hashed) {
-    if (n_passes) *n_passes = n ? 2 : 0;
-    CKR(mhb_count_solid_hashed(st, d_a, d_b, n, k, m, d_hist0, d_edges, d_aux, cap_edges, d_mul_hist, d_nsolid, work, cw.bytes));
+    if (n_passes) *n_passes = n ? (partitioned ? 2 : 3) : 0;
+    CKR((partitioned ? mhb_count_solid_hashed_part : mhb_count_solid_hashed)(st, d_a, d_b, n, k, m, d_hist0, d_edges, d_aux,
+                                                                             cap_edges, d_mul_hist, d_nsolid, work, cw.bytes));
     if (pass_ms && n) {
       uint32_t np = 0, w = 0;
       uint64_t nr = 0;
@@ -203,6 +204,12 @@
   CKR(mhb_sort_records_impl(st, d_a, d_b, n, WR, sort_bytes, n_sort, d_hist0, work, cw.ws_bytes, &in_b, pass_ms));
   return mhb_count_solid(st, in_b ? d_b : d_a, n, k, m, d_edges, d_aux, cap_edges, d_mul_hist, d_nsolid, work + cw.ws_bytes,
                          cw.bytes - cw.ws_bytes);
+}
+
+int count_extract_partitioned(cudaStream_t st, const mhb_dev_reads *reads, uint32_t k, uint32_t *d_a, uint64_t n,
+                              uint64_t *d_hist, char *work, bool hist_done = false) {
+  if (!hist_done) CKR(mhb_count_extract_hist(st, reads, k, n, d_hist));
+  return mhb_count_extract_part(st, reads, k, d_a, n, d_hist, d_hist + 256, work, mhb_count_extract_part_workspace_bytes());
 }
 }
 
@@ -550,7 +557,7 @@
   const CountWork cw = count_work_plan(n, k, m);
   size_t need = Arena::pad(bin_bytes + 16) + 2 * Arena::pad((size_t)n * WR * 4 + 16) + Arena::pad(cw.bytes) +
                 Arena::pad((size_t)cap_edges * WE * 4) + Arena::pad(cap_edges) +
-                Arena::pad(65536 * 8) + Arena::pad(256 * 8) + 4096;
+                Arena::pad(65536 * 8) + Arena::pad(512 * 8) + 4096;
   if (!ix.fixed_len) need += 2 * Arena::pad((n_reads + 1) * 8);
   if (args->want_mercy) need += 2 * Arena::pad((size_t)(n_reads + 1) * 4);
   {
@@ -571,7 +578,7 @@
   uint32_t *d_edges = g_arena.take<uint32_t>((size_t)cap_edges * WE);
   uint8_t *d_aux = g_arena.take<uint8_t>(cap_edges);
   uint64_t *d_mul_hist = g_arena.take<uint64_t>(65536);
-  uint64_t *d_hist0 = g_arena.take<uint64_t>(256);
+  uint64_t *d_hist0 = g_arena.take<uint64_t>(512);
   uint64_t *d_nsolid = g_arena.take<uint64_t>(8);
   uint64_t *d_rec_off = nullptr, *d_edge_off = nullptr;
   uint32_t *d_first = nullptr, *d_last = nullptr;
@@ -591,7 +598,7 @@
     CK(cudaMemcpyAsync(d_edge_off, ix.edge_off.data(), (n_reads + 1) * 8, cudaMemcpyHostToDevice, st));
   }
   CK(cudaMemsetAsync(d_mul_hist, 0, 65536 * 8, st));
-  CK(cudaMemsetAsync(d_hist0, 0, 256 * 8, st));
+  CK(cudaMemsetAsync(d_hist0, 0, 512 * 8, st));
   CK(cudaMemsetAsync(d_nsolid, 0, 64, st));
   res->t_h2d_ms = t.stop();
 
@@ -604,13 +611,14 @@
   reads.edge_off = d_edge_off;
 
   t.start();
-  CKR(mhb_count_extract(st, &reads, k, d_a, n, d_hist0, cw.hist_byte));
+  if (cw.hashed) CKR(count_extract_partitioned(st, &reads, k, d_a, n, d_hist0, d_work));
+  else CKR(mhb_count_extract(st, &reads, k, d_a, n, d_hist0, cw.hist_byte));
   res->t_extract_ms = t.stop();
 
   t.start();
   res->n_rounds = 1;
-  CKR(run_count_stage(st, cw, d_a, d_b, n, k, m, d_hist0, d_edges, d_aux, cap_edges, d_mul_hist, d_nsolid, d_work,
-                      res->sort_pass_ms, &res->n_sort_passes));
+  CKR(run_count_stage(st, cw, d_a, d_b, n, k, m, cw.hashed ? d_hist0 + 256 : d_hist0, d_edges, d_aux, cap_edges,
+                      d_mul_hist, d_nsolid, d_work, res->sort_pass_ms, &res->n_sort_passes, cw.hashed));
   for (uint32_t p = 0; p < res->n_sort_passes; ++p) res->t_sort_ms += res->sort_pass_ms[p];
   uint64_t n_solid = 0;
   CK(cudaMemcpyAsync(&n_solid, d_nsolid, 8, cudaMemcpyDeviceToHost, st));
@@ -1070,7 +1078,7 @@
   const CountWork cw = count_work_plan(n, k, m);
   const size_t count_work = 2 * Arena::pad((size_t)n * WR * 4 + 16) + Arena::pad(cw.bytes);
   size_t fixed = Arena::pad(bin_bytes + 16) + Arena::pad((size_t)cap_edges * WE * 4) + Arena::pad(cap_edges) +
-                 Arena::pad(65536 * 8) + 2 * Arena::pad(256 * 8) + Arena::pad(64) + Arena::pad((size_t)MHB_NUM_BUCKETS * 32) +
+                 Arena::pad(65536 * 8) + Arena::pad(512 * 8) + Arena::pad(256 * 8) + Arena::pad(64) + Arena::pad((size_t)MHB_NUM_BUCKETS * 32) +
                  Arena::pad(128) + 8192;
   if (!ix.fixed_len) fixed += 2 * Arena::pad((n_reads + 1) * 8);
   if (args->need_mercy) fixed += 2 * Arena::pad((n_reads + 1) * 4) + Arena::pad((n_reads + 1) * 8);
@@ -1080,7 +1088,7 @@
   uint32_t *d_edges = g_arena.take<uint32_t>((size_t)cap_edges * WE);
   uint8_t *d_aux = g_arena.take<uint8_t>(cap_edges);
   uint64_t *d_mul_hist = g_arena.take<uint64_t>(65536);
-  uint64_t *d_hist0 = g_arena.take<uint64_t>(256);
+  uint64_t *d_hist0 = g_arena.take<uint64_t>(512);
   uint64_t *d_hist1 = g_arena.take<uint64_t>(256);
   uint64_t *d_nsolid = g_arena.take<uint64_t>(8);
   uint64_t *d_table = g_arena.take<uint64_t>((size_t)MHB_NUM_BUCKETS * 4);
@@ -1112,7 +1120,7 @@
   const bool chunked = h2d_chunks_env > 1 && ix.fixed_len >= k + 1 && n_reads >= (uint64_t)h2d_chunks_env * 64;
   t.start();
   CK(cudaMemsetAsync(d_mul_hist, 0, 65536 * 8, st));
-  CK(cudaMemsetAsync(d_hist0, 0, 256 * 8, st));
+  CK(cudaMemsetAsync(d_hist0, 0, 512 * 8, st));
   CK(cudaMemsetAsync(d_hist1, 0, 256 * 8, st));
   CK(cudaMemsetAsync(d_nsolid, 0, 64, st));
   if (!chunked) {
@@ -1137,7 +1145,8 @@
   uint32_t *c_b = (uint32_t *)(work + Arena::pad((size_t)n * WR * 4 + 16));
   char *c_wsp = work + 2 * Arena::pad((size_t)n * WR * 4 + 16);
   if (!chunked) {
-    CKR(mhb_count_extract(st, &reads, k, c_a, n, d_hist0, cw.hist_byte));
+    if (cw.hashed) CKR(count_extract_partitioned(st, &reads, k, c_a, n, d_hist0, c_wsp));
+    else CKR(mhb_count_extract(st, &reads, k, c_a, n, d_hist0, cw.hist_byte));
   } else {
     static cudaStream_t copy_st = nullptr;
     static cudaEvent_t ev[64];
@@ -1165,11 +1174,14 @@
       piece.bin = d_bin + w0;
       piece.bin_words = w1 - w0;
       piece.n_reads = r1 - r0;
-      CKR(mhb_count_extract(st, &piece, k, c_a + (size_t)r0 * e_per_read * WR, (r1 - r0) * e_per_read, d_hist0, cw.hist_byte));
-    }
+      if (cw.hashed) CKR(mhb_count_extract_hist(st, &piece, k, (r1 - r0) * e_per_read, d_hist0));
+      else CKR(mhb_count_extract(st, &piece, k, c_a + (size_t)r0 * e_per_read * WR, (r1 - r0) * e_per_read, d_hist0, cw.hist_byte));
+    }
+    if (cw.hashed) CKR(count_extract_partitioned(st, &reads, k, c_a, n, d_hist0, c_wsp, true));
   }
   if (verify_fixed) CKR(mhb_check_fixed_len(st, d_bin, n_reads, ix.fixed_len, d_nsolid + 1));
-  CKR(run_count_stage(st, cw, c_a, c_b, n, k, m, d_hist0, d_edges, d_aux, cap_edges, d_mul_hist, d_nsolid, c_wsp, nullptr, nullptr));
+  CKR(run_count_stage(st, cw, c_a, c_b, n, k, m, cw.hashed ? d_hist0 + 256 : d_hist0, d_edges, d_aux, cap_edges, d_mul_hist,
+                      d_nsolid, c_wsp, nullptr, nullptr, cw.hashed));
   uint64_t h_scal[2] = {0, 0};
   CK(cudaMemcpyAsync(h_scal, d_nsolid, 16, cudaMemcpyDeviceToHost, st));
   CK(cudaStreamSynchronize(st));
diff --git a/megahit_b200/csrc/mhb_internal.h b/megahit_b200/csrc/mhb_internal.h
--- a/megahit_b200/csrc/mhb_internal.h
+++ b/megahit_b200/csrc/mhb_internal.h
@@ -9,6 +9,9 @@
 int mhb_sort_records_impl(void *stream, uint32_t *a, uint32_t *b, uint64_t n, uint32_t words, const uint8_t *bytes,
                           uint32_t n_bytes, const uint64_t *first_hist, void *ws, size_t ws_bytes, int *result_in_b,
                           double *pass_ms_host);
+int mhb_sort_records_ex(void *stream, uint32_t *a, uint32_t *b, uint64_t n, uint32_t words, const uint8_t *bytes,
+                        uint32_t n_bytes, const uint64_t *first_hist, void *ws, size_t ws_bytes, int *result_in_b,
+                        double *pass_ms_host, int relaxed);
 
 size_t mhb_arena_bytes(void);
 
diff --git a/megahit_b200/csrc/mhb_kernels.cuh b/megahit_b200/csrc/mhb_kernels.cuh
--- a/megahit_b200/csrc/mhb_kernels.cuh
+++ b/megahit_b200/csrc/mhb_kernels.cuh
@@ -53,7 +53,7 @@
   strand = st ? 1u : 0u;
 }
 
-template <int R>
+template <int R, bool PREV_NEXT = true>
 MHB_HD void make_count_records_roll(const u32 *s, u32 nwords, u32 L, u32 k, u32 q, u64 (&rec)[R], u32 (&strand)[R]) {
   const u32 K1 = k + 1;
   const u32 T = 64u - 2u * K1;
@@ -76,12 +76,17 @@
     const u32 prev_pkg = (pi + j < L) ? b : kSentinel;
     const bool st = B < A;
     const u64 key = st ? B : A;
-    u32 p = prev_pkg, n = next_pkg;
-    if (st) {
-      p = next_pkg == kSentinel ? kSentinel : 3u - next_pkg;
-      n = prev_pkg == kSentinel ? kSentinel : 3u - prev_pkg;
-    }
-    rec[j] = key | (u64)((p << 3) | n);
+    if constexpr (PREV_NEXT) {
+      u32 p = prev_pkg, n = next_pkg;
+      if (st) {
+        p = next_pkg == kSentinel ? kSentinel : 3u - next_pkg;
+        n = prev_pkg == kSentinel ? kSentinel : 3u - prev_pkg;
+      }
+      rec[j] = key | (u64)((p << 3) | n);
+    } else {
+      (void)prev_pkg;
+      rec[j] = key;
+    }
     strand[j] = st ? 1u : 0u;
     next_pkg = (u32)(S >> 62);
     S = (S << 2) | ((u64)b << T);
diff --git a/megahit_b200/csrc/mhb_sortdisp.cu b/megahit_b200/csrc/mhb_sortdisp.cu
--- a/megahit_b200/csrc/mhb_sortdisp.cu
+++ b/megahit_b200/csrc/mhb_sortdisp.cu
@@ -9,6 +9,7 @@
 #include "mhb_sort.cuh"
 #include "mhb_sort3.cuh"
 #include "mhb_part.cuh"
+#include "mhb_countpart.cuh"
 
 using namespace mhb;
 
@@ -209,9 +210,6 @@
 uint64_t g_trace_seq = 0;
 }
 
-int mhb_sort_records_ex(void *stream, uint32_t *a, uint32_t *b, uint64_t n, uint32_t words, const uint8_t *bytes,
-                        uint32_t n_bytes, const uint64_t *first_hist, void *ws, size_t ws_bytes, int *result_in_b,
-                        double *pass_ms_host, int relaxed);
 int mhb_sort_records_impl(void *stream, uint32_t *a, uint32_t *b, uint64_t n, uint32_t words, const uint8_t *bytes,
                           uint32_t n_bytes, const uint64_t *first_hist, void *ws, size_t ws_bytes, int *result_in_b,
                           double *pass_ms_host) {
@@ -360,6 +358,75 @@
   return rc;
 }
 
+int check_reads(const mhb_dev_reads *r, uint32_t k);
+ReadsView make_reads_view(const mhb_dev_reads *r);
+
+static int check_part_args(const mhb_dev_reads *reads, uint32_t k, uint64_t n_edges) {
+  if (int rc = check_reads(reads, k)) return rc;
+  if (!mhb_count_hashed_supported(k, 1)) return mhb_set_error(MHB_ERR_ARG, "fused count extraction needs 8-byte records (13 <= k <= 28)");
+  if (n_edges >= (1ull << 40)) return mhb_set_error(MHB_ERR_ARG, "too many records for one fused extraction");
+  if (reads->fixed_len && n_edges != (reads->fixed_len > k ? reads->n_reads * (uint64_t)(reads->fixed_len - k) : 0))
+    return mhb_set_error(MHB_ERR_ARG, "n_edges does not match the fixed-length library");
+  return MHB_OK;
+}
+
+extern "C" int mhb_count_extract_hist(void *stream, const mhb_dev_reads *reads, uint32_t k, uint64_t n_edges,
+                                      uint64_t *hist_byte5) {
+  if (int rc = check_part_args(reads, k, n_edges)) return rc;
+  if (!hist_byte5) return mhb_set_error(MHB_ERR_ARG, "null histogram");
+  if (reads->n_reads == 0 || n_edges == 0) return MHB_OK;
+  cudaStream_t st = (cudaStream_t)stream;
+  const ReadsView rv = make_reads_view(reads);
+  const u64 blocks = ((n_edges + 3) / 4 + kCxHistThreads - 1) / kCxHistThreads;
+  const int grid = (int)(blocks < (u64)(sm_count() * 8) ? blocks : (u64)(sm_count() * 8));
+  unsigned long long *h = (unsigned long long *)hist_byte5;
+  if (count_key_words(k) == 2) k_count_hist5<2><<<grid, kCxHistThreads, 0, st>>>(rv, k, n_edges, h);
+  else k_count_hist5<1><<<grid, kCxHistThreads, 0, st>>>(rv, k, n_edges, h);
+  CK_LAUNCH();
+  return MHB_OK;
+}
+
+extern "C" size_t mhb_count_extract_part_workspace_bytes(void) { return 2 * 256 * 8 + 256; }
+
+template <int W>
+static int launch_count_extract_part(cudaStream_t st, const ReadsView &rv, u32 k, u64 n, const u64 *bin_addr,
+                                     unsigned long long *gcursor, u32 *tile_counter, unsigned long long *next_hist) {
+  using C = CxPartCfg;
+  static int bps = 0;
+  if (!bps) {
+    CK(cudaFuncSetAttribute(k_count_extract_part<W>, cudaFuncAttributeMaxDynamicSharedMemorySize, (int)C::SMEM));
+    CK(cudaOccupancyMaxActiveBlocksPerMultiprocessor(&bps, k_count_extract_part<W>, C::THREADS, C::SMEM));
+    if (bps < 1) return mhb_set_error(MHB_ERR_CUDA, "fused extract + partition kernel does not fit an SM");
+    if (getenv("MHB_VERBOSE")) fprintf(stderr, "[mhb] fused extract + partition W=%d: %d threads x %d rec, %zu B smem, %d CTA/SM\n", W, C::THREADS, C::IPT, C::SMEM, bps);
+  }
+  const u64 tiles = (n + C::TILE - 1) / C::TILE;
+  u64 grid = (u64)bps * sm_count();
+  if (grid > tiles) grid = tiles;
+  k_count_extract_part<W><<<(int)grid, C::THREADS, C::SMEM, st>>>(rv, k, n, (u32)tiles, bin_addr, gcursor, tile_counter, next_hist);
+  CK_LAUNCH();
+  return MHB_OK;
+}
+
+extern "C" int mhb_count_extract_part(void *stream, const mhb_dev_reads *reads, uint32_t k, uint32_t *records,
+                                      uint64_t n_edges, const uint64_t *hist_byte5, uint64_t *hist_byte6, void *ws,
+                                      size_t ws_bytes) {
+  if (int rc = check_part_args(reads, k, n_edges)) return rc;
+  if (!records || !hist_byte5 || !hist_byte6 || !ws) return mhb_set_error(MHB_ERR_ARG, "null buffer");
+  if (ws_bytes < mhb_count_extract_part_workspace_bytes()) return mhb_set_error(MHB_ERR_ARG, "fused extraction workspace too small");
+  if (reads->n_reads == 0 || n_edges == 0) return MHB_OK;
+  cudaStream_t st = (cudaStream_t)stream;
+  u64 *bin_addr = (u64 *)ws;
+  unsigned long long *gcursor = (unsigned long long *)(bin_addr + 256);
+  u32 *tile_counter = (u32 *)(gcursor + 256);
+  CK(cudaMemsetAsync(gcursor, 0, 256 * 8 + 256, st));
+  k_hist_scan256<<<1, 256, 0, st>>>(hist_byte5, bin_addr, (u64)(uintptr_t)records, 8);
+  CK_LAUNCH();
+  const ReadsView rv = make_reads_view(reads);
+  unsigned long long *h6 = (unsigned long long *)hist_byte6;
+  return count_key_words(k) == 2 ? launch_count_extract_part<2>(st, rv, k, n_edges, bin_addr, gcursor, tile_counter, h6)
+                                 : launch_count_extract_part<1>(st, rv, k, n_edges, bin_addr, gcursor, tile_counter, h6);
+}
+
 extern "C" int mhb_dev_malloc(void **ptr, size_t bytes) {
   CK(cudaMalloc(ptr, bytes));
   return MHB_OK;
diff --git a/megahit_b200/dev.py b/megahit_b200/dev.py
--- a/megahit_b200/dev.py
+++ b/megahit_b200/dev.py
@@ -59,7 +59,9 @@
         self.edges = torch.empty(self.cap_edges * self.WE, **i32)
         self.aux = torch.empty(self.cap_edges, dtype=torch.uint8, device=device)
         self.mul_hist = torch.zeros(65536, dtype=torch.int64, device=device)
-        self.hist0 = torch.zeros(256, dtype=torch.int64, device=device)
+        self.hist0 = torch.zeros(512 if self.hashed else 256, dtype=torch.int64, device=device)
+        self.part_ws = (torch.empty(L.mhb_count_extract_part_workspace_bytes(), dtype=torch.uint8, device=device)
+                        if self.hashed else None)
         self.n_solid_dev = torch.zeros(8, dtype=torch.int64, device=device)
         self.first = torch.empty(n_reads + 1, **i32) if want_mercy else None
         self.last = torch.empty(n_reads + 1, **i32) if want_mercy else None
@@ -76,8 +78,14 @@
 
     def extract(self, bin_dev):
         self.hist0.zero_()
+        if self.hashed:
+            reads = C.byref(self._reads(bin_dev))
+            lib._check(self.L.mhb_count_extract_hist(_stream(), reads, self.k, self.n, _ptr(self.hist0)))
+            lib._check(self.L.mhb_count_extract_part(_stream(), reads, self.k, _ptr(self.a), self.n, _ptr(self.hist0),
+                                                     _ptr(self.hist0[256:]), _ptr(self.part_ws), self.part_ws.numel()))
+            return
         lib._check(self.L.mhb_count_extract(_stream(), C.byref(self._reads(bin_dev)), self.k, _ptr(self.a), self.n,
-                                            _ptr(self.hist0), 5 if self.hashed else self.sort_bytes[0]))
+                                            _ptr(self.hist0), self.sort_bytes[0]))
 
     def sort(self):
         if self.hashed:
@@ -89,9 +97,10 @@
         self.mul_hist.zero_()
         self.n_solid_dev.zero_()
         if self.hashed:
-            lib._check(self.L.mhb_count_solid_hashed(_stream(), _ptr(self.a), _ptr(self.b), self.n, self.k, self.m,
-                                                     _ptr(self.hist0), _ptr(self.edges), _ptr(self.aux), self.cap_edges,
-                                                     _ptr(self.mul_hist), _ptr(self.n_solid_dev), _ptr(self.ws), self.ws.numel()))
+            lib._check(self.L.mhb_count_solid_hashed_part(_stream(), _ptr(self.a), _ptr(self.b), self.n, self.k, self.m,
+                                                          _ptr(self.hist0[256:]), _ptr(self.edges), _ptr(self.aux), self.cap_edges,
+                                                          _ptr(self.mul_hist), _ptr(self.n_solid_dev), _ptr(self.ws),
+                                                          self.ws.numel()))
             return
         lib._check(self.L.mhb_count_solid(_stream(), _ptr(self.sorted), self.n, self.k, self.m, _ptr(self.edges),
                                           _ptr(self.aux), self.cap_edges, _ptr(self.mul_hist), _ptr(self.n_solid_dev),
diff --git a/megahit_b200/lib.py b/megahit_b200/lib.py
--- a/megahit_b200/lib.py
+++ b/megahit_b200/lib.py
@@ -112,7 +112,7 @@
     "mhb_last_error", "mhb_version", "mhb_device_count", "mhb_launch_count", "mhb_count_record_words", "mhb_words_per_edge",
     "mhb_s2s_record_words", "mhb_count_sort_bytes", "mhb_s2s_sort_bytes", "mhb_sort_workspace_bytes",
     "mhb_count_extract", "mhb_check_fixed_len", "mhb_count_extract_range", "mhb_set_round_limit", "mhb_set_s2s_round_limit", "mhb_set_r2s_round_limit", "mhb_plan_rounds", "mhb_plan_rounds16", "mhb_sort_records", "mhb_sort_records_relaxed", "mhb_sort_pass_ms", "mhb_set_sort_cfg", "mhb_partition_scatter", "mhb_partition_scatter_hist", "mhb_plan_partition", "mhb_compact_tip_edges", "mhb_dev_malloc", "mhb_dev_free",
-    "mhb_ipc_export", "mhb_ipc_open", "mhb_ipc_close", "mhb_count_solid_scratch_bytes", "mhb_count_solid", "mhb_count_hashed_supported", "mhb_count_hashed_workspace_bytes", "mhb_count_solid_hashed", "mhb_tipset_bytes",
+    "mhb_ipc_export", "mhb_ipc_open", "mhb_ipc_close", "mhb_count_solid_scratch_bytes", "mhb_count_solid", "mhb_count_hashed_supported", "mhb_count_hashed_workspace_bytes", "mhb_count_solid_hashed", "mhb_count_extract_hist", "mhb_count_extract_part_workspace_bytes", "mhb_count_extract_part", "mhb_count_solid_hashed_part", "mhb_tipset_bytes",
     "mhb_tipset_build", "mhb_count_mark_mercy", "mhb_count_tip_edges", "mhb_s2s_extract", "mhb_s2s_extract_range",
     "mhb_s2s_emit_scratch_bytes", "mhb_s2s_emit", "mhb_set_device", "mhb_count_host", "mhb_s2s_host", "mhb_build_host", "mhb_free",
     "mhb_mercy_candidates_scratch_bytes", "mhb_mercy_candidates", "mhb_mercy_edges_scratch_bytes", "mhb_mercy_edges", "mhb_mercy_edges_count", "mhb_mercy_edges_write", "mhb_mercy_edges_segs", "mhb_mercy_host", "mhb_mercy_planes_words", "mhb_mercy_probe_owned", "mhb_mercy_count_planes", "mhb_edge_lut_bytes", "mhb_edge_lut_build",
@@ -154,6 +154,12 @@
     L.mhb_count_hashed_supported.argtypes = [C.c_uint32, C.c_int32]
     L.mhb_count_solid_hashed.argtypes = [C.c_void_p, C.c_void_p, C.c_void_p, C.c_uint64, C.c_uint32, C.c_int32, C.c_void_p,
                                          C.c_void_p, C.c_void_p, C.c_uint64, C.c_void_p, C.c_void_p, C.c_void_p, C.c_size_t]
+    L.mhb_count_solid_hashed_part.argtypes = L.mhb_count_solid_hashed.argtypes
+    L.mhb_count_extract_hist.argtypes = [C.c_void_p, C.POINTER(DevReads), C.c_uint32, C.c_uint64, C.c_void_p]
+    L.mhb_count_extract_part_workspace_bytes.restype = C.c_size_t
+    L.mhb_count_extract_part_workspace_bytes.argtypes = []
+    L.mhb_count_extract_part.argtypes = [C.c_void_p, C.POINTER(DevReads), C.c_uint32, C.c_void_p, C.c_uint64, C.c_void_p,
+                                         C.c_void_p, C.c_void_p, C.c_size_t]
     L.mhb_tipset_build.argtypes = [C.c_void_p, C.c_void_p, C.c_void_p, C.c_uint64, C.c_uint32, C.c_void_p, C.c_size_t,
                                    C.c_uint64]
     L.mhb_count_mark_mercy.argtypes = [C.c_void_p, C.POINTER(DevReads), C.c_uint32, C.c_void_p, C.c_size_t, C.c_uint64,
```

Result: faster. 16.26 billion (median of 6 runs) (+1.9%).
